# Jarvis73/PEMP

Measured on AMD Instinct MI355X. Metric: episodes/sec (PEMP stage-1 eval step, PASCAL-5i-shaped 1-shot, ResNet-50), higher is better.
Workload: dtype f32

## Files before the change

### include/pemp_hip.h

```cpp
#ifndef PEMP_HIP_H
#define PEMP_HIP_H

#include <stddef.h>
#include <stdint.h>

#ifdef __cplusplus
extern "C" {
#endif

#define PEMP_ABI_VERSION 2

#define PEMP_CONV_RELU 1u
#define PEMP_CONV_SHIFT_PER_IMAGE 2u
#define PEMP_CONV_STEM4 4u
#define PEMP_CONV_POOL3S2 8u
#define PEMP_CONV_OUT_SPLIT3 16u
#define PEMP_CONV_IN_SPLIT3 32u
#define PEMP_CONV_OUT_SPLIT3_ALSO 64u
#define PEMP_CONV_RES_S2 128u
#define PEMP_CONV_RES_HEVEN 512u
#define PEMP_CONV_RES_WEVEN 1024u

typedef struct pemp_conv_desc {
    int32_t N, H, W;
    int32_t Cin, ldx;
    int32_t Ho, Wo;
    int32_t Cout, ldy;
    int32_t KH, KW;
    int32_t stride, pad, dil;
    int32_t ldr;
    int32_t Kpad;
    uint32_t flags;
    int32_t tile;
} pemp_conv_desc;

const char* pemp_last_error(void);
int pemp_abi_version(void);

int pemp_conv2d_tile_shape(int id, int* bm, int* bn);

int pemp_conv2d_nhwc_f32(const pemp_conv_desc* d, const float* x, const float* w, float* y,
                         const float* scale, const float* shift, const float* residual,
                         void* stream);

int pemp_conv2d_padv_nhwc_f32(const pemp_conv_desc* d, const float* x, const float* w, float* y,
                              const float* scale, const float* shift, const float* residual,
                              const float* pad_value, void* stream);

int pemp_conv2d_hybrid_rows(const pemp_conv_desc* d);

int pemp_conv2d_group_nhwc_f32(int n, const pemp_conv_desc* d, const float* const* x, const float* const* w,
                               float* const* y, const float* const* scale, const float* const* shift,
                               const float* const* residual, const float* const* pad_value, void* stream);

int pemp_pack_split3_bf16(const float* w, void* out, int cout, int kpad, void* stream);

int pemp_conv2d_bf16_nhwc(const pemp_conv_desc* d, const void* x, const void* w, void* y, const float* scale,
                          const float* shift, const void* residual, const void* pad_value, int out_f32, void* stream);
int pemp_convert_f32_bf16(const float* x, void* y, long long n, void* stream);
int pemp_convert_bf16_f32(const void* x, float* y, long long n, void* stream);

int pemp_conv2d_dropblock_nhwc_f32(const pemp_conv_desc* d, const float* x, const float* w, float* y, const float* scale,
                                   const float* shift, const float* residual, const float* rowmask, const int* kept_count,
                                   void* ws, size_t ws_bytes, void* stream);
int pemp_bn_apply_dropblock_f32(const float* z, int ldz, const float* mean, const float* invstd, const float* gamma,
                                const float* beta, float* y, int ldy, int M, int C, const float* rowmask,
                                const int* kept_count, void* stream);

int pemp_pack_input_nhwc4_f32(const float* img, const float* prior, float* out,
                              int N, int H, int W, void* stream);

int pemp_maxpool2d_nhwc_f32(const float* x, float* y, int N, int H, int W, int C, int ldx,
                            int Ho, int Wo, int ldy, int k, int s, int p, void* stream);

int pemp_maxpool2d_idx_nhwc_f32(const float* x, float* y, uint8_t* idx, int N, int H, int W, int C,
                                int Ho, int Wo, int k, int s, int p, void* stream);
int pemp_maxpool2d_idx_bwd_nhwc_f32(const uint8_t* idx, const float* dy, float* dx, int N, int H, int W,
                                    int C, int Ho, int Wo, int k, int s, int p, void* stream);

int pemp_global_avgpool_nhwc_f32(const float* x, float* y, int N, int HW, int C, int ldx,
                                 void* stream);

int pemp_channel_affine_multi_f32(const float* x, int ldx, int M, int C, int nb,
                                  const float* const* scale, const float* const* shift,
                                  float* const* y, const int* ldy, void* stream);

size_t pemp_mpm_workspace_bytes(int B, int S, int n, int c, int p);
int pemp_mpm_protos_f32(const float* feat, int ldf, const float* mask, const float* ctr,
                        float* protos, void* ws, size_t ws_bytes,
                        int B, int S, int h, int w, int H, int W, int c, int p, void* stream);

size_t pemp_map_workspace_bytes(int B, int S, int n, int c);
int pemp_masked_avg_pool_f32(const float* feat, int ldf, const float* mask, float* protos,
                             void* ws, size_t ws_bytes, int B, int S, int h, int w, int H, int W,
                             int c, int full_res, void* stream);

int pemp_cosine_proto_max_f32(const float* qry, int ldf, const float* protos, float* pred,
                              uint8_t* resp, int B, int n, int c, int p, float dist_scalar,
                              void* stream);

int pemp_cosine_bank_max_f32(const float* qry, int ldf, const float* bank, const int32_t* index,
                             float* pred, uint8_t* resp, int N, int K, int n, int c, int p,
                             float dist_scalar, void* stream);

int pemp_argmax_masks_f32(const float* pred, float* masks, int B, int n, void* stream);

int pemp_upsample_bilinear_ac_f32(const float* pred, float* out, int B, int C, int h, int w,
                                  int Ho, int Wo, void* stream);

int pemp_upsample_nearest_u8_i64(const uint8_t* resp, int64_t* out, int B, int h, int w,
                                 int Ho, int Wo, void* stream);

size_t pemp_eval_tail_workspace_bytes(int B, int Ho, int Wo);
int pemp_eval_tail_f32(const float* pred, const int64_t* target, uint8_t* pred_out,
                       float* logits_out, double* stats, void* ws, size_t ws_bytes,
                       int B, int h, int w, int Ho, int Wo, void* stream);

size_t pemp_nway_tail_workspace_bytes(int N, int Ho, int Wo);
int pemp_nway_tail_f32(const float* pred, const int64_t* target, const int32_t* want, uint8_t* labels,
                       float* margin, double* stats, void* ws, size_t ws_bytes,
                       int N, int K, int h, int w, int Ho, int Wo, void* stream);

typedef struct pemp_tail_item {
    int32_t Ho, Wo;
    int32_t nblk;
    int32_t part_off;
    int64_t pix_off;
} pemp_tail_item;

size_t pemp_tail_ragged_workspace_bytes(pemp_tail_item* items_host, int n);
int pemp_eval_tail_ragged_f32(const float* pred, const int64_t* target, const pemp_tail_item* items_host,
                              const pemp_tail_item* items_dev, int B, int h, int w, uint8_t* pred_out,
                              double* stats, void* ws, size_t ws_bytes, void* stream);
int pemp_nway_tail_ragged_f32(const float* pred, const int64_t* target, const int32_t* want,
                              const pemp_tail_item* items_host, const pemp_tail_item* items_dev, int N, int K,
                              int h, int w, uint8_t* labels, float* margin, double* stats, void* ws,
                              size_t ws_bytes, void* stream);

int pemp_cm_reduce_f32(const float* x, int ldx, const float* mask_in, float* mask_out, float* stat,
                       int N, int Hm, int Wm, int Hx, int Wx, int C, int stride, void* stream);

int pemp_cm_linear_f32(const float* stat, const int32_t* group, const float* lin_w, const float* lin_b,
                       float* agg, float* feat, int N, int G, int C2, void* stream);
int pemp_cm_bias_f32(const float* feat, const int32_t* group, const float* wext, int ldw, const float* alpha,
                     const float* base, float* out, int N, int Cout, void* stream);
int pemp_cm_bias_bwd_f32(const float* colsum, const float* feat, const int32_t* group, const float* wext, int ldw,
                         float* dwext, int lddw, float* dfeat_img, int accumulate, int N, int Cout, void* stream);
int pemp_cm_linear_bwd_f32(const float* dfeat_img, const int32_t* group, const float* agg, const float* lin_w,
                           float* dlin_w, float* dlin_b, float* dstat, int N, int G, int C2, void* stream);

int pemp_cm_bwd_add_f32(const float* x, int ldx, const float* mask, const float* dstat, float* dx, int ldd,
                        int N, int HW, int C, void* stream);
int pemp_cm_reduce_arg_f32(const float* x, int ldx, const float* mask_in, float* mask_out, float* stat,
                           int32_t* argmax, int N, int Hm, int Wm, int Hx, int Wx, int C, int stride, void* stream);
int pemp_cm_bwd_add_arg_f32(const float* mask, const float* dstat, const int32_t* argmax, float* dx, int ldd,
                            int N, int HW, int C, void* stream);


size_t pemp_conv2d_splitk_workspace_bytes(const pemp_conv_desc* d);
int pemp_conv2d_splitk_nhwc_f32(const pemp_conv_desc* d, const float* x, const float* w, float* y, const float* scale,
                                const float* shift, const float* residual, void* ws, size_t ws_bytes, void* stream);
int pemp_conv2d_padv_splitk_nhwc_f32(const pemp_conv_desc* d, const float* x, const float* w, float* y, const float* scale,
                                     const float* shift, const float* residual, const float* pad_value, void* ws,
                                     size_t ws_bytes, void* stream);
void* pemp_uncached_alloc(size_t bytes);
int pemp_uncached_free(void* p);
int pemp_spin_us(int us, void* stream);
int pemp_splitk_reset(void* ws, void* stream);
int pemp_conv2d_stats_nhwc_f32(const pemp_conv_desc* d, const float* x, const float* w, float* y, float* stats,
                               void* ws, size_t ws_bytes, void* stream);
int pemp_conv2d_stats_rows(const pemp_conv_desc* d);
int pemp_split3_conv2d_stats_nhwc_f32(const pemp_conv_desc* d, const float* x, const void* w3, float* y, float* stats,
                                      void* stream);
int pemp_conv2d_stats_split3_rows(const pemp_conv_desc* d);
// ... 186 lines not shown
```

### pemp_amd/_lib.py

```python
import ctypes as C
import os

import torch

_HERE = os.path.dirname(os.path.abspath(__file__))
LIB_PATH = os.environ.get("PEMP_HIP_LIB", os.path.join(_HERE, "libpemp_hip.so"))

c_fp = C.c_void_p
c_int = C.c_int
c_size = C.c_size_t


class ConvDesc(C.Structure):
    _fields_ = [(n, C.c_int32) for n in
                ("N", "H", "W", "Cin", "ldx", "Ho", "Wo", "Cout", "ldy", "KH", "KW",
                 "stride", "pad", "dil", "ldr", "Kpad")] + [("flags", C.c_uint32), ("tile", C.c_int32)]


class SampleDesc(C.Structure):
    _fields_ = [("img_off", C.c_int64), ("msk_off", C.c_int64), ("img_out", C.c_int64), ("msk_out", C.c_int64)] + \
               [(n, C.c_int32) for n in ("hs", "ws", "sh", "sw", "oy", "ox", "flip", "jitter_order")] + \
               [("jitter", C.c_float * 3), ("mask_mode", C.c_int32), ("ksx", C.c_int32), ("ksy", C.c_int32),
                ("ws_off", C.c_int64)]


class TailItem(C.Structure):
    _fields_ = [(n, C.c_int32) for n in ("Ho", "Wo", "nblk", "part_off")] + [("pix_off", C.c_int64)]


CONV_RELU = 1
CONV_SHIFT_PER_IMAGE = 2
CONV_STEM4 = 4
CONV_POOL3S2 = 8
CONV_OUT_SPLIT3 = 16
CONV_IN_SPLIT3 = 32
CONV_OUT_SPLIT3_ALSO = 64
CONV_RES_S2 = 128
CONV_RES_HEVEN = 512
CONV_RES_WEVEN = 1024

SYMBOLS = {
    "pemp_last_error": (C.c_char_p, []),
    "pemp_abi_version": (c_int, []),
    "pemp_conv2d_hybrid_rows": (c_int, [C.POINTER(ConvDesc)]),
    "pemp_conv2d_tile_shape": (c_int, [c_int, C.POINTER(c_int), C.POINTER(c_int)]),
    "pemp_conv2d_nhwc_f32": (c_int, [C.POINTER(ConvDesc), c_fp, c_fp, c_fp, c_fp, c_fp, c_fp, c_fp]),
    "pemp_conv2d_padv_splitk_nhwc_f32": (c_int, [C.POINTER(ConvDesc), c_fp, c_fp, c_fp, c_fp, c_fp, c_fp, c_fp, c_fp, c_size, c_fp]),
    "pemp_conv2d_padv_nhwc_f32": (c_int, [C.POINTER(ConvDesc), c_fp, c_fp, c_fp, c_fp, c_fp, c_fp, c_fp, c_fp]),
    "pemp_conv2d_group_nhwc_f32": (c_int, [c_int, C.POINTER(ConvDesc)] + [C.POINTER(c_fp)] * 7 + [c_fp]),
    "pemp_conv2d_bf16_nhwc": (c_int, [C.POINTER(ConvDesc), c_fp, c_fp, c_fp, c_fp, c_fp, c_fp, c_fp, c_int, c_fp]),
    "pemp_pack_split3_bf16": (c_int, [c_fp, c_fp, c_int, c_int, c_fp]),
    "pemp_convert_f32_bf16": (c_int, [c_fp, c_fp, C.c_longlong, c_fp]),
    "pemp_convert_bf16_f32": (c_int, [c_fp, c_fp, C.c_longlong, c_fp]),
    "pemp_conv2d_dropblock_nhwc_f32": (c_int, [C.POINTER(ConvDesc), c_fp, c_fp, c_fp, c_fp, c_fp, c_fp, c_fp, c_fp, c_fp, c_size, c_fp]),
    "pemp_bn_apply_dropblock_f32": (c_int, [c_fp, c_int, c_fp, c_fp, c_fp, c_fp, c_fp, c_int, c_int, c_int, c_fp, c_fp, c_fp]),
    "pemp_pack_input_nhwc4_f32": (c_int, [c_fp, c_fp, c_fp, c_int, c_int, c_int, c_fp]),
    "pemp_maxpool2d_nhwc_f32": (c_int, [c_fp, c_fp] + [c_int] * 11 + [c_fp]),
    "pemp_global_avgpool_nhwc_f32": (c_int, [c_fp, c_fp, c_int, c_int, c_int, c_int, c_fp]),
    "pemp_channel_affine_multi_f32": (c_int, [c_fp, c_int, c_int, c_int, c_int,
                                              C.POINTER(c_fp), C.POINTER(c_fp), C.POINTER(c_fp),
                                              C.POINTER(c_int), c_fp]),
    "pemp_mpm_workspace_bytes": (c_size, [c_int] * 5),
    "pemp_mpm_protos_f32": (c_int, [c_fp, c_int, c_fp, c_fp, c_fp, c_fp, c_size] + [c_int] * 8 + [c_fp]),
    "pemp_map_workspace_bytes": (c_size, [c_int] * 4),
    "pemp_masked_avg_pool_f32": (c_int, [c_fp, c_int, c_fp, c_fp, c_fp, c_size] + [c_int] * 8 + [c_fp]),
    "pemp_cosine_proto_max_f32": (c_int, [c_fp, c_int, c_fp, c_fp, c_fp, c_int, c_int, c_int, c_int,
                                          C.c_float, c_fp]),
    "pemp_cosine_bank_max_f32": (c_int, [c_fp, c_int, c_fp, c_fp, c_fp, c_fp] + [c_int] * 5 + [C.c_float, c_fp]),
    "pemp_upsample_bilinear_ac_f32": (c_int, [c_fp, c_fp] + [c_int] * 6 + [c_fp]),
    "pemp_upsample_nearest_u8_i64": (c_int, [c_fp, c_fp] + [c_int] * 5 + [c_fp]),
    "pemp_eval_tail_workspace_bytes": (c_size, [c_int] * 3),
    "pemp_eval_tail_f32": (c_int, [c_fp, c_fp, c_fp, c_fp, c_fp, c_fp, c_size] + [c_int] * 5 + [c_fp]),
    "pemp_nway_tail_workspace_bytes": (c_size, [c_int] * 3),
    "pemp_nway_tail_f32": (c_int, [c_fp] * 7 + [c_size] + [c_int] * 6 + [c_fp]),
    "pemp_tail_ragged_workspace_bytes": (c_size, [C.POINTER(TailItem), c_int]),
    "pemp_eval_tail_ragged_f32": (c_int, [c_fp, c_fp, C.POINTER(TailItem), c_fp] + [c_int] * 3 + [c_fp, c_fp, c_fp, c_size, c_fp]),
    "pemp_nway_tail_ragged_f32": (c_int, [c_fp, c_fp, c_fp, C.POINTER(TailItem), c_fp] + [c_int] * 4 + [c_fp] * 4 + [c_size, c_fp]),
    "pemp_cm_reduce_f32": (c_int, [c_fp, c_int, c_fp, c_fp, c_fp] + [c_int] * 7 + [c_fp]),
    "pemp_argmax_masks_f32": (c_int, [c_fp, c_fp, c_int, c_int, c_fp]),
    "pemp_cm_reduce_arg_f32": (c_int, [c_fp, c_int, c_fp, c_fp, c_fp, c_fp] + [c_int] * 7 + [c_fp]),
    "pemp_cm_bwd_add_arg_f32": (c_int, [c_fp, c_fp, c_fp, c_fp] + [c_int] * 4 + [c_fp]),
    "pemp_cm_linear_f32": (c_int, [c_fp] * 6 + [c_int] * 3 + [c_fp]),
    "pemp_cm_bias_f32": (c_int, [c_fp, c_fp, c_fp, c_int, c_fp, c_fp, c_fp, c_int, c_int, c_fp]),
    "pemp_cm_bias_bwd_f32": (c_int, [c_fp, c_fp, c_fp, c_fp, c_int, c_fp, c_int, c_fp, c_int, c_int, c_int, c_fp]),
    "pemp_cm_linear_bwd_f32": (c_int, [c_fp] * 7 + [c_int] * 3 + [c_fp]),
    "pemp_episode_plan": (c_size, [C.POINTER(SampleDesc), c_int, c_int, c_int]),
    "pemp_episode_preprocess": (c_int, [c_fp, C.POINTER(SampleDesc), c_fp, c_int, c_int, c_int, C.POINTER(C.c_float),
                                        C.POINTER(C.c_float), c_fp, c_fp, c_fp, c_fp, c_size, c_fp]),
    "pemp_dropblock_mask_f32": (c_int, [c_fp, c_fp, c_fp, c_int, c_int, c_int, C.c_float, c_int, C.c_uint64, C.c_uint64, c_fp,
                                        c_fp]),
    "pemp_pixel_scale_f32": (c_int, [c_fp, c_int, c_fp, c_fp, c_fp, c_int, C.c_longlong, c_int, c_fp]),
    "pemp_dropout2d_mask_f32": (c_int, [c_fp, c_fp, c_int, c_int, C.c_float, C.c_uint64, C.c_uint64, c_fp, c_fp]),
    "pemp_channel_scale_f32": (c_int, [c_fp, c_int, c_fp, c_fp, c_int, c_int, c_int, c_int, c_fp]),
    "pemp_cm_bwd_add_f32": (c_int, [c_fp, c_int, c_fp, c_fp, c_fp, c_int, c_int, c_int, c_int, c_fp]),
    "pemp_conv2d_splitk_workspace_bytes": (c_size, [C.POINTER(ConvDesc)]),
    "pemp_conv2d_splitk_nhwc_f32": (c_int, [C.POINTER(ConvDesc), c_fp, c_fp, c_fp, c_fp, c_fp, c_fp, c_fp, c_size, c_fp]),
    "pemp_uncached_alloc": (c_fp, [c_size]),
    "pemp_uncached_free": (c_int, [c_fp]),
    "pemp_splitk_reset": (c_int, [c_fp, c_fp]),
    "pemp_spin_us": (c_int, [c_int, c_fp]),
    "pemp_conv2d_stats_nhwc_f32": (c_int, [C.POINTER(ConvDesc), c_fp, c_fp, c_fp, c_fp, c_fp, c_size, c_fp]),
    "pemp_conv2d_stats_rows": (c_int, [C.POINTER(ConvDesc)]),
    "pemp_split3_conv2d_stats_nhwc_f32": (c_int, [C.POINTER(ConvDesc), c_fp, c_fp, c_fp, c_fp, c_fp]),
    "pemp_conv2d_stats_split3_rows": (c_int, [C.POINTER(ConvDesc)]),
    "pemp_bn_stats_partials_f32": (c_int, [c_fp, c_int, c_int, c_int, C.c_float, C.c_float, c_fp, c_fp, c_fp, c_fp, c_fp]),
    "pemp_bn_fwd_partials_f32": (c_int, [c_fp, c_int, c_fp, c_int, c_int, c_int, C.c_float, C.c_float, c_fp, c_fp, c_fp, c_int,
                                         c_fp, c_int, c_int, c_fp, c_fp, c_fp, c_fp, c_fp, c_fp]),
    "pemp_conv2d_bnbwd_nhwc_f32": (c_int, [C.POINTER(ConvDesc), c_fp, c_fp, c_fp, c_fp, c_fp, c_fp, c_int, c_fp, c_fp, c_fp, c_fp,
                                           c_size, c_fp]),
    "pemp_bn_bwd_partials_f32": (c_int, [c_fp, c_int, c_fp, c_int, c_fp, c_fp, c_fp, c_fp, c_int, c_fp, c_int, c_fp, c_fp, c_int,
                                         c_int, c_fp]),
    "pemp_bn_apply_mask_f32": (c_int, [c_fp, c_int, c_fp, c_fp, c_fp, c_fp, c_fp, c_int, c_fp, c_int, c_int, c_int,
                                       c_int, c_fp, c_fp]),
    "pemp_conv2d_wgrad_workspace_bytes": (c_size, [C.POINTER(ConvDesc)]),
    "pemp_conv2d_wgrad_nhwc_f32": (c_int, [C.POINTER(ConvDesc), c_fp, c_fp, c_fp, c_int, c_fp, c_size, c_fp]),
    "pemp_colsum_workspace_bytes": (c_size, [c_int, c_int]),
    "pemp_bn_stats_f32": (c_int, [c_fp, c_int, c_int, c_int, C.c_float, C.c_float, c_fp, c_fp, c_fp, c_fp,
                                  c_fp, c_size, c_fp]),
    "pemp_bn_apply_f32": (c_int, [c_fp, c_int, c_fp, c_fp, c_fp, c_fp, c_fp, c_int, c_fp, c_int, c_int, c_int,
                                  c_int, c_fp]),
    "pemp_bn_bwd_f32": (c_int, [c_fp, c_int, c_fp, c_int, c_fp, c_int, c_fp, c_fp, c_fp, c_fp, c_int, c_fp, c_int,
                                c_fp, c_fp, c_int, c_int, c_int, c_fp, c_size, c_fp]),
    "pemp_bn_bwd_mask_f32": (c_int, [c_fp, c_int, c_fp, c_int, c_fp, c_fp, c_int, c_fp, c_fp, c_fp, c_fp, c_int, c_fp, c_int,
                                     c_fp, c_fp, c_int, c_int, c_int, c_fp, c_size, c_fp]),
    "pemp_relu_bias_bwd_f32": (c_int, [c_fp, c_int, c_fp, c_int, c_fp, c_int, c_fp, c_int, c_fp, c_int, c_int,
                                       c_int, c_fp, c_size, c_fp]),
    "pemp_maxpool2d_bwd_nhwc_f32": (c_int, [c_fp, c_fp, c_fp] + [c_int] * 9 + [c_fp]),
    "pemp_maxpool2d_idx_nhwc_f32": (c_int, [c_fp, c_fp, c_fp] + [c_int] * 9 + [c_fp]),
    "pemp_maxpool2d_idx_bwd_nhwc_f32": (c_int, [c_fp, c_fp, c_fp] + [c_int] * 9 + [c_fp]),
    "pemp_scatter_strided_nhwc_f32": (c_int, [c_fp, c_fp] + [c_int] * 7 + [c_fp]),
    "pemp_gap_bwd_add_nhwc_f32": (c_int, [c_fp, c_fp, c_int, c_int, c_int, c_int, c_fp]),
    "pemp_head_bwd_workspace_bytes": (c_size, [c_int] * 5),
    "pemp_head_bwd_f32": (c_int, [c_fp, c_fp, c_int, c_fp, c_fp, c_fp, c_fp, c_fp, c_fp, c_fp, c_fp, c_fp, c_fp, c_int,
                                  c_fp, c_fp, c_size] + [c_int] * 11 + [C.c_float, c_fp]),
    "pemp_head_bwd_dlogits_f32": (c_int, [c_fp, c_fp, c_int, c_fp, c_fp, c_fp, c_fp, c_fp, c_fp, c_fp, c_int,
                                          c_fp, c_fp, c_size] + [c_int] * 11 + [C.c_float, c_fp]),
    "pemp_eval_tail_weighted_f32": (c_int, [c_fp, c_fp, c_fp, c_fp, c_fp, c_fp, c_fp, c_size] + [c_int] * 5 + [c_fp]),
    "pemp_cedt_workspace_bytes": (c_size, [c_int] * 3),
    "pemp_cedt_weight_f32": (c_int, [c_fp, c_fp, c_fp, c_size, c_int, c_int, c_int, C.c_float, c_fp]),
    "pemp_sgd_workspace_bytes": (c_size, []),
    "pemp_sgd_clip_step_f32": (c_int, [c_fp, c_fp, c_fp, C.c_longlong, C.c_float, C.c_float, C.c_float,
                                       C.c_float, c_int, C.c_float, c_int, c_fp, c_fp, c_size, c_fp]),
    "pemp_dgrad_mirror_f32": (c_int, [c_fp, c_fp, c_fp, c_int, c_int, c_fp]),
    "pemp_adam_clip_step_f32": (c_int, [c_fp, c_fp, c_fp, c_fp, C.c_longlong, C.c_float] + [C.c_double] * 5 + [C.c_longlong, C.c_float, c_fp, c_fp,
                                                                                                  c_size, c_fp]),
    "pemp_prior_mask_workspace_bytes": (c_size, [c_int] * 3),
    "pemp_prior_mask_f32": (c_int, [c_fp, c_int, c_fp, c_int, c_fp, c_fp, c_fp, c_size] + [c_int] * 4 + [c_fp]),
    "pemp_prior_bank_pack_f32": (c_int, [c_fp, c_int, c_fp, c_fp, c_fp, c_fp] + [c_int] * 4 + [c_fp]),
    "pemp_prior_bank_workspace_bytes": (c_size, [c_int] * 3),
    "pemp_prior_bank_f32": (c_int, [c_fp, c_int, c_fp, c_fp, c_fp, c_fp, c_fp, c_fp, c_size] + [c_int] * 6 + [c_fp]),
    "pemp_bank_gather_rows_f32": (c_int, [c_fp, c_fp, c_fp, c_int, c_int, c_int, c_fp]),
    "pemp_adaptive_avgpool_nhwc_f32": (c_int, [c_fp, c_int, c_fp] + [c_int] * 7 + [c_fp]),
    "pemp_resize_bilinear_ac_nhwc_f32": (c_int, [c_fp, C.c_longlong, c_int, c_int, c_fp, C.c_longlong, c_int, c_int] + [c_int] * 7
                                         + [c_fp]),
    "pemp_weighted_gap_f32": (c_int, [c_fp, c_int, c_fp, c_fp] + [c_int] * 5 + [c_fp]),
    "pemp_scale_add_nhwc_f32": (c_int, [c_fp, c_int, c_fp, c_fp, c_int, c_fp, c_int, C.c_longlong, c_int, c_fp]),
    "pemp_canet_support_vector_f32": (c_int, [c_fp, c_int, c_fp, c_fp] + [c_int] * 7 + [c_fp]),
    "pemp_canet_zterm_f32": (c_int, [c_fp, c_fp, c_fp, c_fp] + [c_int] * 7 + [c_fp]),
    "pemp_canet_block_input_f32": (c_int, [c_fp, c_int, c_fp, c_fp, c_int, c_fp] + [c_int] * 5 + [c_fp]),
    "pemp_canet_history_update_f32": (c_int, [c_fp, c_fp, c_fp, c_int, c_fp, c_int, c_int, c_fp]),
    "pemp_canet_zterm_bwd_workspace_bytes": (c_size, [c_int] * 4),
    "pemp_canet_zterm_bwd_f32": (c_int, [c_fp, c_int, c_fp, c_int, c_fp, c_fp, c_fp, c_fp, c_fp, c_size] + [c_int] * 6 + [c_fp]),
    "pemp_canet_support_vector_bwd_f32": (c_int, [c_fp, c_fp, c_fp] + [c_int] * 8 + [c_fp]),
    "pemp_canet_cls_bwd_workspace_bytes": (c_size, [c_int] * 2),
    "pemp_canet_cls_bwd_f32": (c_int, [c_fp, c_fp, c_int, c_fp, c_fp, c_int, c_fp, c_fp, c_fp, c_size] + [c_int] * 3 + [c_fp]),
    "pemp_upsample_ce_bwd_f32": (c_int, [c_fp] * 6 + [c_int] * 5 + [c_fp]),
    "pemp_weighted_gap_bwd_f32": (c_int, [c_fp, c_fp, c_fp] + [c_int] * 6 + [c_fp]),
    "pemp_adaptive_avgpool_bwd_multi_nhwc_f32": (c_int, [c_int, C.POINTER(c_fp)] + [C.POINTER(c_int)] * 3 + [c_fp] + [c_int] * 5
                                                 + [c_fp]),
    "pemp_resize_bilinear_ac_bwd_nhwc_f32": (c_int, [c_fp, C.c_longlong, c_int, c_int] * 3 + [c_int] * 6 + [c_fp]),
    "pemp_pfenet_merge_support_bwd_workspace_bytes": (c_size, [c_int] * 3),
    "pemp_pfenet_merge_support_bwd_f32": (c_int, [c_int, C.POINTER(c_fp)] + [C.POINTER(c_int)] * 3 + [C.POINTER(c_fp)] * 2
                                          + [c_int, c_fp, c_fp, c_fp, c_size] + [c_int] * 3 + [c_fp]),
    "pemp_rpmms_em_f32": (c_int, [c_fp, c_int, c_fp, c_fp, c_fp, c_fp] + [c_int] * 5 + [c_fp]),
    "pemp_rpmms_prob_map_f32": (c_int, [c_fp, c_int, c_fp, c_fp, c_int, C.c_longlong, c_int, c_int, c_int, c_fp]),
    "pemp_rpmms_proto_sum_f32": (c_int, [c_fp, c_fp, c_fp, c_int, c_fp, c_fp, c_fp, c_int, C.c_longlong] + [c_int] * 5 + [c_fp]),
    "pemp_rpmms_proto_taps_f32": (c_int, [c_fp, c_fp, c_fp, c_int, c_int, c_fp]),
    "pemp_rpmms_bank_l56_f32": (c_int, [c_fp, c_int, c_fp, c_int, c_fp, c_fp, c_fp, c_fp, c_fp, c_int, C.c_longlong] + [c_int] * 6 + [c_fp]),
    "pemp_rpmms_proto_sum_train_f32": (c_int, [c_fp, c_fp, c_fp, c_int, c_fp, c_fp, c_fp, c_fp, c_int, C.c_longlong] + [c_int] * 5 + [c_fp]),
    "pemp_rpmms_proto_sum_bwd_work_floats": (c_size, [c_int] * 4),
    "pemp_rpmms_proto_sum_bwd_f32": (c_int, [c_fp, c_int, C.c_longlong, c_fp, c_int, c_fp, c_fp, c_fp, c_fp, c_fp, c_int, c_fp, c_fp, c_int,
                                             c_fp, c_fp, c_size] + [c_int] * 5 + [c_fp]),
    "pemp_rpmms_history_bwd_f32": (c_int, [c_fp, c_int, c_fp, c_fp, c_int, c_int, c_fp]),
}

ABI_VERSION = 2
_lib = None


class PempHipError(RuntimeError):
    pass

# ... 26 lines not shown
```

### pemp_amd/build.py

```python
import hashlib
import os
import subprocess
from concurrent.futures import ThreadPoolExecutor

HERE = os.path.dirname(os.path.abspath(__file__))
CSRC = os.path.join(HERE, "csrc")
OBJ = os.path.join(HERE, "_obj")
OUT = os.path.join(HERE, "libpemp_hip.so")
SOURCES = ("conv_igemm.hip", "conv_dma.hip", "conv_dma2.hip", "conv_panel.hip", "conv_row3.hip", "conv_ring.hip", "conv_stem_pool.hip", "conv_wgrad.hip", "train_ops.hip", "pool_misc.hip", "head.hip", "head_bwd.hip", "cedt.hip",
           "episode_io.hip", "dropout.hip", "cm_linear.hip", "pfenet.hip", "pfenet_bwd.hip", "canet.hip", "canet_bwd.hip", "rpmms.hip", "rpmms_bwd.hip")
FLAGS = ["-O3", "--offload-arch=gfx950", "-std=c++17", "-fPIC"]


def _headers():
    return [os.path.join(CSRC, f) for f in sorted(os.listdir(CSRC)) if f.endswith((".h", ".inc"))] + \
           [os.path.join(HERE, "..", "include", "pemp_hip.h")]


def csrc_digest():
    h = hashlib.sha1()
    for f in sorted(os.listdir(CSRC)):
        with open(os.path.join(CSRC, f), "rb") as fh:
            h.update(f.encode() + b"\0" + fh.read())
    with open(os.path.join(HERE, "..", "include", "pemp_hip.h"), "rb") as fh:
        h.update(fh.read())
    return h.hexdigest()[:12]


CONV_ENGINE = ("common.h", "conv_common.h", "conv_tiles.h", "conv_igemm.hip", "conv_dma.hip", "conv_dma2.hip", "conv_panel.hip", "conv_row3.hip", "conv_ring.hip", "conv_stem_pool.hip")


def conv_digest():
    h = hashlib.sha1()
    for f in CONV_ENGINE:
        with open(os.path.join(CSRC, f), "rb") as fh:
            h.update(f.encode() + b"\0" + fh.read())
    return h.hexdigest()[:12]


def needs_build():
    if not os.path.exists(OUT):
        return True
    t = os.path.getmtime(OUT)
    deps = [os.path.join(CSRC, f) for f in os.listdir(CSRC)] + [os.path.join(HERE, "..", "include", "pemp_hip.h")]
    return any(os.path.getmtime(d) > t for d in deps)


def _stamp(src, flags):
    h = hashlib.sha1(" ".join(flags).encode())
    for f in [src] + _headers():
        with open(f, "rb") as fh:
            h.update(fh.read())
    return h.hexdigest()


def _compile(hipcc, name, flags, force, verbose):
    src = os.path.join(CSRC, name)
    obj = os.path.join(OBJ, name.replace(".hip", ".o"))
    stamp_file = obj + ".stamp"
    stamp = _stamp(src, flags)
    if not force and os.path.exists(obj) and os.path.exists(stamp_file) and open(stamp_file).read() == stamp:
        return obj
    cmd = [hipcc] + flags + ["-c", src, "-o", obj]
    if verbose:
        print(" ".join(cmd), flush=True)
    subprocess.run(cmd, check=True)
    with open(stamp_file, "w") as f:
        f.write(stamp)
    return obj


def build(force=False, verbose=False, extra_flags=(), out=None):
    out = out or OUT
    if not force and out == OUT and not needs_build():
        return OUT
    hipcc = os.environ.get("HIPCC", "/opt/rocm/bin/hipcc")
    os.makedirs(OBJ, exist_ok=True)
    flags = FLAGS + list(extra_flags)
    jobs = max(1, min(len(SOURCES), int(os.environ.get("PEMP_BUILD_JOBS", str(min(os.cpu_count() or 1, 8))))))
    with ThreadPoolExecutor(jobs) as ex:
        objs = list(ex.map(lambda n: _compile(hipcc, n, flags, force, verbose), SOURCES))
    tmp = out + f".tmp{os.getpid()}"
    cmd = [hipcc, "--offload-arch=gfx950", "-shared", "-fPIC", "-o", tmp] + objs
    if verbose:
        print(" ".join(cmd), flush=True)
    subprocess.run(cmd, check=True)
    os.replace(tmp, out)
    return out


if __name__ == "__main__":
    print(build(force=True, verbose=True))
```

### pemp_amd/csrc/conv_common.h

```cpp
#pragma once
#include "common.h"

namespace pemp {

typedef __attribute__((ext_vector_type(16))) float f32x16;
typedef __attribute__((ext_vector_type(4))) float v4f;
typedef __attribute__((ext_vector_type(8))) __bf16 bf16x8;
typedef __attribute__((ext_vector_type(2))) unsigned int u32x2;

#define PEMP_CONV_BF16_IO 0x100u

__device__ __forceinline__ v4f load_quad(const float* base, size_t off, unsigned bf16) {
    if (!bf16) return *(const v4f*)(base + off);
    const u32x2 r = *(const u32x2*)((const unsigned short*)base + off);
    return v4f{__builtin_bit_cast(float, r.x << 16), __builtin_bit_cast(float, r.x & 0xFFFF0000u),
               __builtin_bit_cast(float, r.y << 16), __builtin_bit_cast(float, r.y & 0xFFFF0000u)};
}

__device__ __forceinline__ unsigned int bf16_bits(float f) {
    const unsigned int u = __builtin_bit_cast(unsigned int, f);
    if ((u & 0x7FFFFFFFu) > 0x7F800000u) return (u >> 16) | 0x40u;
    return (u + 0x7FFFu + ((u >> 16) & 1u)) >> 16;
}

// ... 217 lines not shown
                    if constexpr (DB) {
                        const float k = a.rowmask[m];
                        o.x = __fdiv_rn(__fmul_rn(__fmul_rn(o.x, k), db_numel), db_sum);
                        o.y = __fdiv_rn(__fmul_rn(__fmul_rn(o.y, k), db_numel), db_sum);
                        o.z = __fdiv_rn(__fmul_rn(__fmul_rn(o.z, k), db_numel), db_sum);
                        o.w = __fdiv_rn(__fmul_rn(__fmul_rn(o.w, k), db_numel), db_sum);
                    }
                    if constexpr (EPI == 2) {
                        const uint32_t b = mw[i] >> c4;
                        o.x = (b & 1u) ? o.x : 0.f;
                        o.y = (b & 2u) ? o.y : 0.f;
                        o.z = (b & 4u) ? o.z : 0.f;
                        o.w = (b & 8u) ? o.w : 0.f;
                    }
                    store_quad(a.y, (size_t)m * a.ldy + n, o, a.flags & PEMP_CONV_BF16_IO);
                    if constexpr (EPI == 1) {
                        s1 += o;
                        s2 += o * o;
                    }
                    if constexpr (EPI == 2) {
                        s1 += o;
                        s2 += o * ((zt[i] - bmu) * bis);
                    }
                }
            }
            if constexpr (EPI != 0) {
                t1 += s1;
                t2 += s2;
            }
            if constexpr (OS3 == 2) {
                static_assert(EPI == 0 && !DB && !PRE, "the second, pre-split output: plain epilogue");
                v4f sc8[2], sh8[2];
                conv_split3_affine(a, n_base + ni * 32 + (lane & 3) * 8, sc8, sh8);
                conv_store_split3_to(a, (unsigned short*)a.res, S, m_base + mi * 32, n_base + ni * 32, lane, sc8, sh8);
            }
            asm volatile("s_waitcnt lgkmcnt(0)" ::: "memory");
        }
        if constexpr (EPI != 0) {
            *(v4f*)(R + ((ni * 2 + 0) * 8 + rr) * 32 + c4) = t1;
            *(v4f*)(R + ((ni * 2 + 1) * 8 + rr) * 32 + c4) = t2;
        }
    }
}

template <int BN, int WGM, int NW, int TN>
__device__ __forceinline__ void conv_stats_store(const ConvArgs& a, const float* Rall, int bm, int n0, int tid) {
    constexpr int WGN = NW / WGM, WN = BN / WGN;
    if (tid < 2 * BN) {
        const int st = tid / BN, col = tid - st * BN;
        const int wni = col / WN, ni = (col - wni * WN) >> 5, c = col & 31;
        float s = 0.f;
#pragma unroll
        for (int wmi = 0; wmi < WGM; ++wmi)
#pragma unroll
            for (int g = 0; g < 8; ++g) s += Rall[((((wmi * WGN + wni) * TN + ni) * 2 + st) * 8 + g) * 32 + c];
        a.stats[((size_t)bm * 2 + st) * a.Cout + n0 + col] = s;
    }
}

template <int TM, int TN, bool DB = false, int OS3 = 0>
__device__ __forceinline__ void conv_epilogue_lds(const ConvArgs& a, f32x16 (&acc)[TM][TN], float* S, int m_base,
                                                  int n_base, int lane) {
    const v4f none[1] = {{0.f, 0.f, 0.f, 0.f}};
    static_assert(TM * TN * 4 != 1, "tile");
    conv_epilogue_lds_pre<TM, TN, 1, 0, DB, OS3>(a, acc, S, m_base, n_base, lane, none);
}

__device__ __forceinline__ void conv_patch_store_f32(const ConvArgs& a, const float* S, int m_base, int n32, int lane, const v4f& sc,
                                                     const v4f& sh, bool per_img, const v4f* res, unsigned bf16) {
    const bool relu = a.flags & PEMP_CONV_RELU;
    const int rr = lane >> 3, c4 = (lane & 7) * 4, n = n32 + c4;
#pragma unroll
    for (int i = 0; i < 4; ++i) {
        const int row = rr + 8 * i;
        const int m = m_base + row;
        const v4f v = *(const v4f*)(S + row * 32 + c4);
        if (m < a.M) {
            v4f add = sh;
            if (per_img) add += *(const v4f*)(a.shift + (size_t)(m / a.HoWo) * a.Cout + n);
            if (res && a.res) add += res[i];
            store_quad(a.y, (size_t)m * a.ldy + n, conv_affine_quad(v, sc, add, relu), bf16);
        }
    }
}

template <int TM, int TN, bool PLAIN = false>
__device__ __forceinline__ void conv_epilogue_s3p(const ConvArgs& a, f32x16 (&acc)[TM][TN], float* S, int m_base, int n_base,
                                                  int lane, const v4f* pre, const v4f (&scv)[TN], const v4f (&shv)[TN]) {
    const bool per_img = !PLAIN && (a.flags & PEMP_CONV_SHIFT_PER_IMAGE);
    const int lr = lane & 31, lh = lane >> 5;
#pragma unroll
    for (int ni = 0; ni < TN; ++ni) {
#pragma unroll
        for (int mi = 0; mi < TM; ++mi) {
            PEMP_CONV_PATCH_PUT(S, acc[mi][ni], lr, lh);
            asm volatile("s_waitcnt lgkmcnt(0)" ::: "memory");
            conv_patch_store_f32(a, S, m_base + mi * 32, n_base + ni * 32, lane, scv[ni], shv[ni], per_img,
                                 PLAIN ? nullptr : pre + (mi * TN + ni) * 4, PLAIN ? 0u : a.flags & PEMP_CONV_BF16_IO);
            asm volatile("s_waitcnt lgkmcnt(0)" ::: "memory");
        }
    }
}

template <int TN>
__device__ __forceinline__ void conv_epilogue_r16(const ConvArgs& a, v4f (&acc)[TN], float* S, int m_base, int n_base, int lane) {
    constexpr int WN = TN * 16, LD = WN + 4, QPR = WN / 4;
    static_assert(16 * LD * 4 <= 4096 && (16 * QPR) % 64 == 0, "R16 epilogue patch");
    const bool relu = a.flags & PEMP_CONV_RELU;
    const bool per_img = a.flags & PEMP_CONV_SHIFT_PER_IMAGE;
    const int r16 = lane & 15, g = lane >> 4;
#pragma unroll
    for (int ni = 0; ni < TN; ++ni)
#pragma unroll
        for (int e = 0; e < 4; ++e) S[(4 * g + e) * LD + ni * 16 + r16] = acc[ni][e];
    asm volatile("s_waitcnt lgkmcnt(0)" ::: "memory");
    const int c4 = (lane % QPR) * 4, n = n_base + c4;
    v4f sc = {1.f, 1.f, 1.f, 1.f}, sh = {0.f, 0.f, 0.f, 0.f};
    if (a.scale) sc = *(const v4f*)(a.scale + n);
    if (a.shift && !per_img) sh = *(const v4f*)(a.shift + n);
#pragma unroll
    for (int i = 0; i < 16 * QPR / 64; ++i) {
        const int row = (lane + 64 * i) / QPR;
        const int m = m_base + row;
        const v4f v = *(const v4f*)(S + row * LD + c4);
        if (m < a.M) {
            v4f add = sh;
            if (per_img) add += *(const v4f*)(a.shift + (size_t)(m / a.HoWo) * a.Cout + n);
            if (a.res) add += load_quad(a.res, (size_t)m * a.ldr + n, a.flags & PEMP_CONV_BF16_IO);
            store_quad(a.y, (size_t)m * a.ldy + n, conv_affine_quad(v, sc, add, relu), a.flags & PEMP_CONV_BF16_IO);
        }
    }
}

int launch_conv_dma(int shape, const ConvArgs& a, hipStream_t st);
bool conv_dma2_supported(const ConvArgs& a);
int launch_conv_dma2(int shape, const ConvArgs& a, hipStream_t st);
int launch_conv_dma2_group(int shape, ConvGroupArgs& g, hipStream_t st);
int launch_conv_dma2_hybrid(const ConvArgs& a, hipStream_t st);
int conv_dma2_hybrid_rows(int M, int Cout);
int launch_conv_dma2_bf16(int shape, const ConvArgs& a, hipStream_t st);
int launch_conv_dma2_db(int shape, ConvArgs a, void* ws, size_t ws_bytes, bool split, hipStream_t st);
struct SplitKPlan { int full, split, pieces; size_t ws_bytes; };
SplitKPlan conv_dma2_splitk_plan(int shape, const ConvArgs& a);
int launch_conv_dma2_splitk(int shape, ConvArgs a, void* ws, size_t ws_bytes, hipStream_t st);
int launch_conv_dma2_split3(int shape, ConvArgs a, void* ws, size_t ws_bytes, bool split, hipStream_t st);
int launch_conv_dma2_group_split3(int shape, ConvGroupArgs& g, hipStream_t st);
int launch_conv_dma2_split3_stats(int shape, const ConvArgs& a, hipStream_t st);
bool conv_dma2_split3_stats_shape(int shape);
int launch_conv_dma2_split3_persist(int shape, const ConvArgs& a, hipStream_t st);
bool conv_dma2_persist_out_split3(int shape);
int launch_conv_dma2_split3_pre(int shape, bool persistent, const ConvArgs& a, hipStream_t st);
bool conv_panel_supported(const ConvArgs& a);
int launch_conv_panel(int shape, const ConvArgs& a, hipStream_t st);
bool conv_row3_supported(const ConvArgs& a);
int launch_conv_row3(bool persistent, const ConvArgs& a, hipStream_t st);
bool conv_ring_supported(const ConvArgs& a);
int launch_conv_ring(const ConvArgs& a, hipStream_t st);
int conv_dma2_simds();
int pack_split3(const float* w, void* out, int cout, int kpad, hipStream_t st);
int launch_conv_stem_pool(const ConvArgs& a, hipStream_t st);
int conv_stem_pool_out(int i);

template <class Kern> int allow_lds(Kern kern, size_t lds);
template <class Kern>
int persistent_grid(Kern kern, int threads, size_t lds, long long tiles, int& occ_cache, const char* what, int& grid_out) {
    if (!occ_cache) {
        const int rc = allow_lds(kern, lds);
        if (rc) return rc;
        int v = 0;
        hipError_t e = hipOccupancyMaxActiveBlocksPerMultiprocessor(&v, (const void*)kern, threads, lds);
        if (e != hipSuccess || v <= 0) {
            set_error("%s: occupancy query failed (%s, %d blocks)", what, hipGetErrorString(e), v);
            return -1;
        }
        occ_cache = v;
    }
    long long grid = (long long)occ_cache * (conv_dma2_simds() / 4);
    if (grid < 8) grid = 8;
    if (grid > tiles) grid = tiles;
    grid_out = (int)grid;
    return 0;
}

}
```

### pemp_amd/csrc/conv_igemm.hip

```cpp
#include "conv_tiles.h"

namespace pemp {


template <int BM, int BN, int WGM, bool STEM>
__global__ __launch_bounds__(256) void conv_igemm_kernel(ConvArgs a) {
    constexpr int WGN = 4 / WGM;
    constexpr int WM = BM / WGM, WN = BN / WGN;
    constexpr int TM = WM / 32, TN = WN / 32;
    constexpr int AL = BM / 32, BL = BN / 32;
    static_assert(TM >= 1 && TN >= 1, "wave tile");

    extern __shared__ __attribute__((aligned(16))) v4f smem[];
    v4f* As = smem;
    v4f* Bs = smem + 2 * 8 * BM;

    const int tid = threadIdx.x;
    const int lane = tid & 63;
    const int wave = tid >> 6;
    const int wm0 = (wave / WGN) * WM;
    const int wn0 = (wave % WGN) * WN;
    const int lr = lane & 31, lh = lane >> 5;

    const int ntn = a.Cout / BN;
// ... 71 lines not shown
            _Pragma("unroll") for (int i = 0; i < AL; ++i) ra[i] = *(const v4f*)pa[i];              \
        }                                                                                            \
        _Pragma("unroll") for (int i = 0; i < BL; ++i) rb[i] = *(const v4f*)pb[i];                   \
    } while (0)

#define PEMP_ADVANCE()                                                                               \
    do {                                                                                             \
        if constexpr (STEM) {                                                                        \
            _Pragma("unroll") for (int i = 0; i < BL; ++i) pb[i] += 32;                              \
        } else if (a.ntaps > 1) {                                                                    \
                                   \
            if (++cur_tap == a.ntaps) {                                                              \
                cur_tap = 0;                                                                         \
                ++cur_cb;                                                                            \
            }                                                                                        \
            PEMP_SET_TAP(cur_tap, cur_cb);                                                           \
            const int koff = cur_tap * a.Cin + cur_cb * 32;                                          \
            _Pragma("unroll") for (int i = 0; i < BL; ++i) pb[i] = wrow[i] + koff;                   \
        } else {                                                                                     \
            _Pragma("unroll") for (int i = 0; i < BL; ++i) pb[i] += 32;                              \
            _Pragma("unroll") for (int i = 0; i < AL; ++i) pa[i] += 32;                              \
        }                                                                                            \
    } while (0)

#define PEMP_LSTORE(buf_)                                                                            \
    do {                                                                                             \
        v4f* Ab_ = As + (buf_) * 8 * BM + q * BM;                                                 \
        v4f* Bb_ = Bs + (buf_) * 8 * BN + q * BN;                                                 \
        _Pragma("unroll") for (int i = 0; i < AL; ++i) {                                             \
            v4f v = ra[i];                                                                        \
            if (!((okmask >> i) & 1u)) v = v4f{0.f, 0.f, 0.f, 0.f};                          \
            Ab_[(r + 32 * i) ^ q] = v;                                                               \
        }                                                                                            \
        _Pragma("unroll") for (int i = 0; i < BL; ++i) Bb_[(r + 32 * i) ^ q] = rb[i];                \
    } while (0)

    f32x16 acc[TM][TN];
#pragma unroll
    for (int mi = 0; mi < TM; ++mi)
#pragma unroll
        for (int ni = 0; ni < TN; ++ni)
#pragma unroll
            for (int e = 0; e < 16; ++e) acc[mi][ni][e] = 0.f;

    if constexpr (!STEM) PEMP_SET_TAP(0, 0);
    PEMP_GLOAD(0);
    PEMP_LSTORE(0);
    __syncthreads();

    const int arow = wm0 + lr, brow = wn0 + lr;
#ifndef PEMP_ABLATE
#define PEMP_ABLATE 0
#endif
    for (int kt = 0; kt < a.nk; ++kt) {
        const int buf = (PEMP_ABLATE >= 2) ? 0 : (kt & 1);
        if (PEMP_ABLATE < 1 && kt + 1 < a.nk) {
            PEMP_ADVANCE();
            PEMP_GLOAD(kt + 1);
        }
        __builtin_amdgcn_sched_barrier(0);

        const v4f* Ab = As + buf * 8 * BM;
        const v4f* Bb = Bs + buf * 8 * BN;
        v4f af[2][TM], bf[2][TN];
#pragma unroll
        for (int mi = 0; mi < TM; ++mi) af[0][mi] = Ab[lh * BM + ((arow + mi * 32) ^ lh)];
#pragma unroll
        for (int ni = 0; ni < TN; ++ni) bf[0][ni] = Bb[lh * BN + ((brow + ni * 32) ^ lh)];
#pragma unroll
        for (int j = 0; j < 4; ++j) {
            if (j < 3) {
                const int qq = 2 * (j + 1) + lh;
#pragma unroll
                for (int mi = 0; mi < TM; ++mi) af[(j + 1) & 1][mi] = Ab[qq * BM + ((arow + mi * 32) ^ qq)];
#pragma unroll
                for (int ni = 0; ni < TN; ++ni) bf[(j + 1) & 1][ni] = Bb[qq * BN + ((brow + ni * 32) ^ qq)];
            }
            __builtin_amdgcn_sched_barrier(0);
#pragma unroll
            for (int mi = 0; mi < TM; ++mi)
#pragma unroll
                for (int ni = 0; ni < TN; ++ni) {
                    const v4f av = af[j & 1][mi], bv = bf[j & 1][ni];
                    acc[mi][ni] = __builtin_amdgcn_mfma_f32_32x32x2f32(av.x, bv.x, acc[mi][ni], 0, 0, 0);
                    acc[mi][ni] = __builtin_amdgcn_mfma_f32_32x32x2f32(av.y, bv.y, acc[mi][ni], 0, 0, 0);
                    acc[mi][ni] = __builtin_amdgcn_mfma_f32_32x32x2f32(av.z, bv.z, acc[mi][ni], 0, 0, 0);
                    acc[mi][ni] = __builtin_amdgcn_mfma_f32_32x32x2f32(av.w, bv.w, acc[mi][ni], 0, 0, 0);
                }
        }
        __builtin_amdgcn_sched_barrier(0);
        if (PEMP_ABLATE < 2) {
            PEMP_LSTORE(buf ^ 1);
            __syncthreads();
        }
    }
#undef PEMP_GLOAD
#undef PEMP_ADVANCE
#undef PEMP_SET_TAP
#undef PEMP_LSTORE

    conv_epilogue_lds<TM, TN>(a, acc, (float*)smem + wave * 1024, m0 + wm0, n0 + wn0, lane);
}

static int launch_conv(int shape, const ConvArgs& a, hipStream_t st) {
    return with_tile<FamIgemm>(shape, [&](auto t) {
        using T = decltype(t);
        auto kern = (a.flags & PEMP_CONV_STEM4) ? conv_igemm_kernel<T::BM, T::BN, T::WGM, true> : conv_igemm_kernel<T::BM, T::BN, T::WGM, false>;
        return launch_with_lds(kern, tile_grid<T>(a), 256, tile_lds<T>(), st, a, "conv_igemm");
    });
}

}

using namespace pemp;

extern "C" int pemp_conv2d_nhwc_f32(const pemp_conv_desc* d, const float* x, const float* w, float* y,
                                    const float* scale, const float* shift, const float* residual,
                                    void* stream) {
    return pemp_conv2d_padv_nhwc_f32(d, x, w, y, scale, shift, residual, nullptr, stream);
}

static int conv2d_impl(const pemp_conv_desc* d, const float* x, const float* w, float* y, const float* scale, const float* shift,
                       const float* residual, const float* pad_value, void* ws, size_t ws_bytes, void* stream);

extern "C" int pemp_conv2d_padv_nhwc_f32(const pemp_conv_desc* d, const float* x, const float* w, float* y,
                                         const float* scale, const float* shift, const float* residual,
                                         const float* pad_value, void* stream) {
    PEMP_REQUIRE(!d || !decode_tile(d->tile).splitk,
                 "conv2d: the split-K tile ids 31..37 / 51..56 need pemp_conv2d_splitk_nhwc_f32 (workspace)");
    return conv2d_impl(d, x, w, y, scale, shift, residual, pad_value, nullptr, 0, stream);
}

extern "C" int pemp_conv2d_splitk_nhwc_f32(const pemp_conv_desc* d, const float* x, const float* w, float* y,
                                           const float* scale, const float* shift, const float* residual, void* ws,
                                           size_t ws_bytes, void* stream) {
    return conv2d_impl(d, x, w, y, scale, shift, residual, nullptr, ws, ws_bytes, stream);
}

extern "C" int pemp_conv2d_padv_splitk_nhwc_f32(const pemp_conv_desc* d, const float* x, const float* w, float* y,
                                                const float* scale, const float* shift, const float* residual,
                                                const float* pad_value, void* ws, size_t ws_bytes, void* stream) {
    PEMP_REQUIRE(pad_value, "conv2d_padv_splitk: pad_value is null");
    return conv2d_impl(d, x, w, y, scale, shift, residual, pad_value, ws, ws_bytes, stream);
}

static int conv_fill(const pemp_conv_desc* d, const float* x, const float* w, float* y, const float* scale, const float* shift,
                     const float* residual, const float* pad_value, ConvArgs& a, bool any_taps = false, bool pooled = false) {
    PEMP_REQUIRE(d && x && w && y, "conv2d: null pointer");
    PEMP_REQUIRE(pooled || !(d->flags & (PEMP_CONV_OUT_SPLIT3 | PEMP_CONV_IN_SPLIT3 | PEMP_CONV_OUT_SPLIT3_ALSO)),
                 "conv2d: pre-split activations belong to pemp_conv2d_nhwc_f32 / _padv_ (no grouped / dropblock / statistics / bf16 form)");
    PEMP_REQUIRE(pooled || !(d->flags & PEMP_CONV_POOL3S2), "conv2d: PEMP_CONV_POOL3S2 belongs to pemp_conv2d_nhwc_f32 (no grouped / dropblock / statistics / bf16 form)");
    PEMP_REQUIRE(pooled || !(d->flags & (PEMP_CONV_RES_S2 | PEMP_CONV_RES_HEVEN | PEMP_CONV_RES_WEVEN)),
                 "conv2d: PEMP_CONV_RES_S2 belongs to pemp_conv2d_nhwc_f32 (no grouped / dropblock / statistics / bf16 form)");
    PEMP_REQUIRE(!pad_value || (!(d->flags & PEMP_CONV_STEM4) && (any_taps || d->KH * d->KW > 1) && ((uintptr_t)pad_value & 15) == 0),
                 "conv2d: pad_value needs a multi-tap non-stem conv and a 16-byte aligned [Cin] vector");
    PEMP_REQUIRE(d->N > 0 && d->H > 0 && d->W > 0 && d->Cin > 0 && d->Cout > 0, "conv2d: bad dims");
    PEMP_REQUIRE(d->KH > 0 && d->KW > 0 && d->stride > 0 && d->dil > 0 && d->pad >= 0, "conv2d: bad kernel geometry");
    const int ho = (d->H + 2 * d->pad - d->dil * (d->KH - 1) - 1) / d->stride + 1;
    const int wo = (d->W + 2 * d->pad - d->dil * (d->KW - 1) - 1) / d->stride + 1;
    PEMP_REQUIRE(ho == d->Ho && wo == d->Wo, "conv2d: Ho/Wo (%d,%d) do not match geometry (%d,%d)", d->Ho, d->Wo, ho, wo);
    PEMP_REQUIRE(d->Cout % 64 == 0, "conv2d: Cout=%d must be a multiple of 64", d->Cout);
    PEMP_REQUIRE(d->ldy >= d->Cout && d->ldy % 4 == 0 && ((uintptr_t)y & 15) == 0, "conv2d: ldy must be >= Cout and a multiple of 4, y 16-byte aligned");
    PEMP_REQUIRE(!scale || ((uintptr_t)scale & 15) == 0, "conv2d: scale must be 16-byte aligned");
    PEMP_REQUIRE(!shift || ((uintptr_t)shift & 15) == 0, "conv2d: shift must be 16-byte aligned");
    PEMP_REQUIRE(((uintptr_t)x & 15) == 0 && ((uintptr_t)w & 15) == 0, "conv2d: x/w must be 16-byte aligned");
    const bool stem = d->flags & PEMP_CONV_STEM4;
    const int ntaps = d->KH * d->KW;
    if (stem) {
        PEMP_REQUIRE(d->Cin == 4 && d->ldx == 4, "conv2d: STEM4 needs NHWC4 input (Cin=ldx=4)");
        PEMP_REQUIRE(d->Kpad % 32 == 0 && d->Kpad >= ntaps * 4, "conv2d: STEM4 Kpad=%d too small / not x32", d->Kpad);
    } else {
        PEMP_REQUIRE(d->Cin % 32 == 0, "conv2d: Cin=%d must be a multiple of 32 (or use STEM4)", d->Cin);
        PEMP_REQUIRE(d->ldx >= d->Cin && d->ldx % 4 == 0, "conv2d: ldx=%d must be >= Cin and a multiple of 4", d->ldx);
        PEMP_REQUIRE(d->Kpad == ntaps * d->Cin, "conv2d: Kpad=%d must equal KH*KW*Cin=%d", d->Kpad, ntaps * d->Cin);
    }
    const long long in_elems = (long long)d->N * d->H * d->W * d->ldx;
    const long long out_elems = (long long)d->N * d->Ho * d->Wo * (long long)(d->ldy > d->ldr ? d->ldy : d->ldr);
    PEMP_REQUIRE(in_elems < (1ll << 31) && out_elems < (1ll << 31), "conv2d: tensor too large for 32-bit indexing");

    a.x = x; a.w = w; a.y = y; a.scale = scale; a.shift = shift; a.res = residual; a.padv = pad_value; a.stats = nullptr; a.bz = nullptr;
    a.bmask = nullptr; a.bmean = nullptr; a.binvstd = nullptr; a.ldbz = 0;
    a.rowmask = nullptr; a.rowcnt = nullptr;
    a.N = d->N; a.H = d->H; a.W = d->W; a.Cin = d->Cin; a.ldx = d->ldx; a.Ho = d->Ho; a.Wo = d->Wo;
    a.Cout = d->Cout; a.ldy = d->ldy; a.KH = d->KH; a.KW = d->KW; a.stride = d->stride; a.pad = d->pad;
    a.dil = d->dil; a.ldr = d->ldr; a.Kpad = d->Kpad; a.flags = d->flags;
    a.HoWo = d->Ho * d->Wo;
    a.M = d->N * a.HoWo;
    a.ntaps = ntaps;
    a.cin_steps = stem ? 1 : d->Cin / 32;
    a.nk = d->Kpad / 32;
    if (residual && !(d->flags & PEMP_CONV_OUT_SPLIT3_ALSO)) PEMP_REQUIRE(d->ldr >= d->Cout && d->ldr % 4 == 0 && ((uintptr_t)residual & 15) == 0, "conv2d: ldr must be >= Cout and x4, residual 16-byte aligned");
    a.sk_ws = nullptr; a.sk_cnt = nullptr; a.sk_full = 0; a.sk_S = 1;
    a.bm_first = 0;
    return 0;
}

static int conv2d_impl(const pemp_conv_desc* d, const float* x, const float* w, float* y, const float* scale, const float* shift,
                       const float* residual, const float* pad_value, void* ws, size_t ws_bytes, void* stream) {
    ConvArgs a;
    const int rc = conv_fill(d, x, w, y, scale, shift, residual, pad_value, a, false, true);
    if (rc) return rc;
    const bool stem = d->flags & PEMP_CONV_STEM4;
    int tile = d->tile;
    if (tile == 0) {
        tile = 3;
    }
    TileId t = decode_tile(tile);
    if (t.ring) {
        PEMP_REQUIRE(!ws && !pad_value && conv_ring_supported(a),
                     "conv2d: tile %d unsupported: needs a 1x1 conv without padding on fp32 activations with Kpad == Cin >= 128 and Cout %% 128 == 0, the "
                     "fp32 output or PEMP_CONV_OUT_SPLIT3 (ldy == Cout); no residual, PEMP_CONV_OUT_SPLIT3_ALSO, PEMP_CONV_IN_SPLIT3, PEMP_CONV_RES_S2, "
                     "padding value, stem, split-K or workspace; operands < 2 GiB", tile);
        return launch_conv_ring(a, (hipStream_t)stream);
    }
    const bool out_split3 = d->flags & PEMP_CONV_OUT_SPLIT3;
    if (out_split3)
        PEMP_REQUIRE(t.family == TILE_SPLIT3 && !t.splitk && !t.panel && !ws && !stem && !residual && a.Cout % 32 == 0 && a.ldy == a.Cout,
                     "conv2d: PEMP_CONV_OUT_SPLIT3 needs an unsplit split3 tile id (41..44, 46, 47, 49, 146, 149), ldy == Cout, no residual / workspace");
    const bool also_split3 = d->flags & PEMP_CONV_OUT_SPLIT3_ALSO;
    if (also_split3) {
        PEMP_REQUIRE(t.presplit && !out_split3 && !ws && !stem && a.Cout % 32 == 0,
                     "conv2d: PEMP_CONV_OUT_SPLIT3_ALSO needs tile id 146 / 149, no PEMP_CONV_OUT_SPLIT3 / split-K / workspace / stem");
        PEMP_REQUIRE(residual && ((uintptr_t)residual & 15) == 0,
                     "conv2d: PEMP_CONV_OUT_SPLIT3_ALSO takes the pre-split tensor (16-byte aligned) in the residual argument; a residual is never read");
        const char *y0 = (const char*)y, *y1 = y0 + ((size_t)(a.M - 1) * a.ldy + a.Cout) * 4;
        const char *s0 = (const char*)residual, *s1 = s0 + (size_t)a.M * a.Cout * 6;
        PEMP_REQUIRE(y1 <= s0 || s1 <= y0, "conv2d: PEMP_CONV_OUT_SPLIT3_ALSO: y and the pre-split tensor overlap");
    }
    const bool res_s2 = d->flags & PEMP_CONV_RES_S2;
    PEMP_REQUIRE(res_s2 || !(d->flags & (PEMP_CONV_RES_HEVEN | PEMP_CONV_RES_WEVEN)), "conv2d: PEMP_CONV_RES_HEVEN / _WEVEN come with PEMP_CONV_RES_S2");
    if (res_s2) {
        PEMP_REQUIRE(residual && !out_split3 && !also_split3 && !(d->flags & PEMP_CONV_IN_SPLIT3) && !ws && !stem && !pad_value,
                     "conv2d: PEMP_CONV_RES_S2 needs a residual, no pre-split operands / PEMP_CONV_OUT_SPLIT3_ALSO / split-K / workspace / stem / padding value");
        PEMP_REQUIRE(t.family == TILE_SPLIT3 && t.exists && !t.splitk && !t.persistent && !t.presplit &&
                         (t.panel ? (a.nk == 2 || (a.nk == 4 && t.shape == 2)) : t.shape == 3),
                     "conv2d: PEMP_CONV_RES_S2 needs tile id 43, 72 with Kpad 64 or 128, or 71 with Kpad 64 (tile %d, Kpad %d: the persistent, split-K, "
                     "pre-split and fp32-chain ids have no strided-residual form)", tile, a.Kpad);
        a.Hr = 2 * a.Ho - 1 + ((d->flags & PEMP_CONV_RES_HEVEN) ? 1 : 0);
        a.Wr = 2 * a.Wo - 1 + ((d->flags & PEMP_CONV_RES_WEVEN) ? 1 : 0);
        PEMP_REQUIRE((long long)a.N * a.Hr * a.Wr * a.ldr < (1ll << 31), "conv2d: PEMP_CONV_RES_S2: residual too large for 32-bit indexing");
    }
    if (d->flags & PEMP_CONV_POOL3S2) {
        PEMP_REQUIRE(stem && t.family == TILE_SPLIT3 && !t.splitk && !t.panel && !residual && !pad_value,
                     "conv2d: PEMP_CONV_POOL3S2 needs PEMP_CONV_STEM4 with split3 weights (a tile id 41..49), no residual, no padding value");
        return launch_conv_stem_pool(a, (hipStream_t)stream);
    }
    PEMP_REQUIRE(tile != 33 && tile != 53, "conv2d: no split-K variant of the 64 x 64 tile");
    PEMP_REQUIRE(tile != 45 && tile != 55, "conv2d: no split3 form of the 128 x 64 8-wave tile");
    PEMP_REQUIRE(tile != 48, "conv2d: no persistent split3 form of the 128 x 128 4-wave tile");
    PEMP_REQUIRE(t.exists, "conv2d: unknown tile id %d", tile);
    hipStream_t st = (hipStream_t)stream;
    PEMP_REQUIRE(t.presplit == ((d->flags & PEMP_CONV_IN_SPLIT3) != 0), "conv2d: tile ids 146 / 149 and PEMP_CONV_IN_SPLIT3 come together (tile %d)", tile);
    if (t.presplit) {
        PEMP_REQUIRE(!stem && !ws && a.ntaps > 1 && a.ntaps <= 16 && a.ldx == a.Cin && !(d->flags & PEMP_CONV_SHIFT_PER_IMAGE),
                     "conv2d: tile %d takes convs of 2..16 taps with ldx == Cin, no per-image shift, no workspace", tile);
        PEMP_REQUIRE(conv_dma2_supported(a) && (long long)a.Cout * a.Kpad * 6 < (1ll << 31),
                     "conv2d: tile %d needs <= 32 taps and operands < 2 GiB (a padding value behind the activations)", tile);
        PEMP_REQUIRE_COUT("conv2d", t.shape, a.Cout);
        if (t.row3) {
            PEMP_REQUIRE(conv_row3_supported(a),
                         "conv2d: tile %d unsupported: needs a 3x3 / stride 1 / pad == dil conv, the plain fp32 output without residual / padding value, "
                         "and a stage of at most 288 rows (256 + 2 d + d ceil((255 + 2 d) / W))", tile);
            return launch_conv_row3(t.persistent, a, st);
        }
        return launch_conv_dma2_split3_pre(t.shape, t.persistent, a, st);
    }
    if (t.family == TILE_SPLIT3) {
        PEMP_REQUIRE(!stem && conv_dma2_supported(a) && (long long)a.Cout * a.Kpad * 6 < (1ll << 31),
                     "conv2d: split3 tile %d needs a geometry of the buffer-addressed kernels (no stem, <= 32 taps, operands < 2 GiB)", tile);
        PEMP_REQUIRE_COUT("conv2d", t.shape, a.Cout);
        if (t.panel) {
            PEMP_REQUIRE(!ws && conv_panel_supported(a),
                         "conv2d: tile %d needs a 1x1 conv without padding, Kpad <= 256, no padding value / per-image shift / workspace, operands < 2 GiB", tile);
            return launch_conv_panel(t.shape, a, st);
        }
        if (t.persistent && (!out_split3 || conv_dma2_persist_out_split3(t.shape))) return launch_conv_dma2_split3_persist(t.shape, a, st);
        return launch_conv_dma2_split3(t.shape, a, ws, ws_bytes, t.splitk, st);
    }
    if (t.family == TILE_DMA2 && t.splitk) {
        if (conv_dma2_supported(a)) {
            PEMP_REQUIRE_COUT("conv2d", t.shape, a.Cout);
            return launch_conv_dma2_splitk(t.shape, a, ws, ws_bytes, st);
        }
        t.splitk = false;
    }
    if (t.family == TILE_DMA2 && t.shape == 9) {
        if (conv_dma2_supported(a)) {
            const int rc2 = launch_conv_dma2_hybrid(a, st);
            if (rc2 != -2) return rc2;
        }
        t.shape = 3;
    }
    if (t.family == TILE_DMA2) {
        if (conv_dma2_supported(a)) {
            PEMP_REQUIRE_COUT("conv2d", t.shape, a.Cout);
            return launch_conv_dma2(t.shape, a, st);
        }
        t.family = TILE_DMA;
        if (t.shape == 8) t.shape = 3;
    }
    if (t.family == TILE_DMA) {
        PEMP_REQUIRE_COUT("conv2d", t.shape, a.Cout);
        return launch_conv_dma(t.shape, a, st);
    }
    PEMP_REQUIRE(t.shape != 1 || a.Cout % 128 == 0, "conv2d: tile 128x128 needs Cout %% 128 == 0");
    return launch_conv(t.shape, a, st);
}


extern "C" int pemp_conv2d_group_nhwc_f32(int n, const pemp_conv_desc* d, const float* const* x, const float* const* w,
                                          float* const* y, const float* const* scale, const float* const* shift,
                                          const float* const* residual, const float* const* pad_value, void* stream) {
    PEMP_REQUIRE(n >= 1 && n <= CONV_GROUP_MAX && d && x && w && y, "conv2d_group: 1..%d member convs", CONV_GROUP_MAX);
    ConvGroupArgs g;
    g.n = n;
    const int tile = d[0].tile;
    const TileId t = decode_tile(tile);
    const bool s3 = t.family == TILE_SPLIT3 && t.exists && !t.splitk && !t.persistent && !t.panel && !t.presplit;
    PEMP_REQUIRE((t.family == TILE_DMA2 && !t.splitk && t.shape <= 8) || s3, "conv2d_group: tile must be one of the buffer-addressed variants 21..28 or 41..44, 46, got %d", tile);
    for (int i = 0; i < n; ++i) {
        PEMP_REQUIRE(d[i].tile == tile, "conv2d_group: every member must name the same tile variant");
        PEMP_REQUIRE(!pad_value || (pad_value[i] != nullptr) == (pad_value[0] != nullptr), "conv2d_group: pad_value for every member or for none");
        const int rc = conv_fill(&d[i], x[i], w[i], y[i], scale ? scale[i] : nullptr, shift ? shift[i] : nullptr,
                                 residual ? residual[i] : nullptr, pad_value ? pad_value[i] : nullptr, g.a[i], true);
        if (rc) return rc;
        PEMP_REQUIRE(conv_dma2_supported(g.a[i]), "conv2d_group: member %d lies outside the buffer-addressed kernels (stem / > 32 taps / 2 GiB operands / padding vector not behind the activations)", i);
        PEMP_REQUIRE_COUT("conv2d_group", t.shape, g.a[i].Cout);
        PEMP_REQUIRE(!s3 || (long long)g.a[i].Cout * g.a[i].Kpad * 6 < (1ll << 31), "conv2d_group: split3 weights of 2 GiB or more");
    }
    auto clash = [](const float* pa, long long rows_a, int ld_a, int c_a, const float* pb, long long rows_b, int ld_b, int c_b) {
        if (!pa || !pb) return false;
        const char *a0 = (const char*)pa, *a1 = a0 + ((rows_a - 1) * ld_a + c_a) * 4;
        const char *b0 = (const char*)pb, *b1 = b0 + ((rows_b - 1) * ld_b + c_b) * 4;
        if (a1 <= b0 || b1 <= a0) return false;
        if (ld_a != ld_b) return true;
        const long long delta = (b0 - a0) / 4, r = ((delta % ld_a) + ld_a) % ld_a;
        return !(r >= c_a && r + c_b <= ld_a);
    };
    for (int i = 0; i < n; ++i) {
        const long long Mi = (long long)g.a[i].N * g.a[i].Ho * g.a[i].Wo;
        for (int j = 0; j < n; ++j) {
            if (j == i) continue;
            const long long Mj = (long long)g.a[j].N * g.a[j].Ho * g.a[j].Wo, Pj = (long long)g.a[j].N * g.a[j].H * g.a[j].W;
            PEMP_REQUIRE(j > i || !clash(g.a[i].y, Mi, g.a[i].ldy, g.a[i].Cout, g.a[j].y, Mj, g.a[j].ldy, g.a[j].Cout),
                         "conv2d_group: members %d and %d write the same output", i, j);
            PEMP_REQUIRE(!clash(g.a[i].y, Mi, g.a[i].ldy, g.a[i].Cout, g.a[j].x, Pj, g.a[j].ldx, g.a[j].Cin),
                         "conv2d_group: member %d writes what member %d reads as its input", i, j);
            PEMP_REQUIRE(!clash(g.a[i].y, Mi, g.a[i].ldy, g.a[i].Cout, g.a[j].res, Mj, g.a[j].ldr, g.a[j].Cout),
                         "conv2d_group: member %d writes what member %d reads as its residual", i, j);
        }
    }
    for (int i = n; i < CONV_GROUP_MAX; ++i) g.a[i] = g.a[0];
    return s3 ? launch_conv_dma2_group_split3(t.shape, g, (hipStream_t)stream) : launch_conv_dma2_group(t.shape, g, (hipStream_t)stream);
}

extern "C" int pemp_pack_split3_bf16(const float* w, void* out, int cout, int kpad, void* stream) {
    PEMP_REQUIRE(w && out && cout > 0 && kpad > 0 && kpad % 32 == 0, "pack_split3: null pointer or Kpad not a multiple of 32");
    PEMP_REQUIRE((((uintptr_t)w | (uintptr_t)out) & 15) == 0, "pack_split3: pointers must be 16-byte aligned");
    return pack_split3(w, out, cout, kpad, (hipStream_t)stream);
}


extern "C" int pemp_conv2d_dropblock_nhwc_f32(const pemp_conv_desc* d, const float* x, const float* w, float* y, const float* scale,
                                              const float* shift, const float* residual, const float* rowmask, const int* kept_count,
                                              void* ws, size_t ws_bytes, void* stream) {
    PEMP_REQUIRE(rowmask && kept_count, "conv2d_dropblock: null mask / count");
    ConvArgs a;
    const int rc = conv_fill(d, x, w, y, scale, shift, residual, nullptr, a);
    if (rc) return rc;
    const TileId t = decode_tile(d->tile);
    PEMP_REQUIRE(t.family == TILE_DMA2 && t.exists && t.shape <= 7,
                 "conv2d_dropblock: tile must be 21..27 or 31..37 (no 33), got %d", d->tile);
    PEMP_REQUIRE(conv_dma2_supported(a), "conv2d_dropblock: geometry / operand size outside the buffer-addressed kernels");
    a.rowmask = rowmask;
    a.rowcnt = kept_count;
    PEMP_REQUIRE_COUT("conv2d_dropblock", t.shape, a.Cout);
    return launch_conv_dma2_db(t.shape, a, ws, ws_bytes, t.splitk, (hipStream_t)stream);
}


extern "C" int pemp_conv2d_bf16_nhwc(const pemp_conv_desc* d, const void* x, const void* w, void* y, const float* scale,
                                     const float* shift, const void* residual, const void* pad_value, int out_f32, void* stream) {
    PEMP_REQUIRE(d && x && w && y, "conv2d_bf16: null pointer");
    PEMP_REQUIRE(!(d->flags & (PEMP_CONV_STEM4 | PEMP_CONV_BF16_IO | PEMP_CONV_POOL3S2 | PEMP_CONV_OUT_SPLIT3_ALSO)), "conv2d_bf16: no stem variant; unknown flags");
    PEMP_REQUIRE(d->Cin % 64 == 0 && d->ldx % 8 == 0 && d->ldx >= d->Cin && d->Kpad == d->KH * d->KW * d->Cin,
                 "conv2d_bf16: Cin must be a multiple of 64, ldx of 8 (bf16 elements), Kpad = KH*KW*Cin");
    PEMP_REQUIRE(!residual || !out_f32, "conv2d_bf16: a residual comes with a bf16 output");
    const TileId t = decode_tile(d->tile == 0 ? 24 : d->tile);
    PEMP_REQUIRE(t.family == TILE_DMA2 && !t.splitk && t.shape <= 7, "conv2d_bf16: tile must be 0 or 21..27");
    pemp_conv_desc h = *d;
    h.Cin = d->Cin / 2;
    h.ldx = d->ldx / 2;
    h.Kpad = d->Kpad / 2;
    ConvArgs a;
    const int rc = conv_fill(&h, (const float*)x, (const float*)w, (float*)y, scale, shift, (const float*)residual,
                             (const float*)pad_value, a);
    if (rc) return rc;
    if (!out_f32) a.flags |= PEMP_CONV_BF16_IO;
    PEMP_REQUIRE(conv_dma2_supported(a), "conv2d_bf16: geometry / operand size outside the buffer-addressed kernels");
    PEMP_REQUIRE_COUT("conv2d_bf16", t.shape, a.Cout);
    return launch_conv_dma2_bf16(t.shape, a, (hipStream_t)stream);
}


static TileId stats_tile(const pemp_conv_desc* d) { return decode_tile(d->tile == 0 ? 23 : d->tile); }

static int conv_stats_fill(const char* what, const pemp_conv_desc* d, ConvArgs& a) {
    PEMP_REQUIRE(!(d->flags & (PEMP_CONV_STEM4 | PEMP_CONV_RELU | PEMP_CONV_SHIFT_PER_IMAGE | PEMP_CONV_POOL3S2 | PEMP_CONV_OUT_SPLIT3 | PEMP_CONV_IN_SPLIT3 | PEMP_CONV_OUT_SPLIT3_ALSO | PEMP_CONV_RES_S2 | PEMP_CONV_RES_HEVEN | PEMP_CONV_RES_WEVEN)), "%s: plain conv only (no stem / ReLU / per-image shift)", what);
    PEMP_REQUIRE(d->N > 0 && d->H > 0 && d->W > 0 && d->Cin > 0 && d->Cout > 0 && d->KH > 0 && d->KW > 0 && d->stride > 0 && d->dil > 0 && d->pad >= 0,
                 "%s: bad geometry", what);
    const int ho = (d->H + 2 * d->pad - d->dil * (d->KH - 1) - 1) / d->stride + 1;
    const int wo = (d->W + 2 * d->pad - d->dil * (d->KW - 1) - 1) / d->stride + 1;
    PEMP_REQUIRE(ho == d->Ho && wo == d->Wo, "%s: Ho/Wo do not match geometry", what);
    PEMP_REQUIRE(d->Cout % 64 == 0 && d->Cin % 32 == 0 && d->ldx >= d->Cin && d->ldx % 4 == 0 && d->ldy >= d->Cout && d->ldy % 4 == 0,
                 "%s: Cout %% 64, Cin %% 32, strides %% 4", what);
    PEMP_REQUIRE(d->Kpad == d->KH * d->KW * d->Cin, "%s: Kpad must equal KH*KW*Cin", what);
    a.scale = nullptr; a.shift = nullptr; a.padv = nullptr; a.rowmask = nullptr; a.rowcnt = nullptr;
    a.N = d->N; a.H = d->H; a.W = d->W; a.Cin = d->Cin; a.ldx = d->ldx; a.Ho = d->Ho; a.Wo = d->Wo;
    a.Cout = d->Cout; a.ldy = d->ldy; a.KH = d->KH; a.KW = d->KW; a.stride = d->stride; a.pad = d->pad;
    a.dil = d->dil; a.ldr = d->ldr; a.Kpad = d->Kpad; a.flags = d->flags;
    a.HoWo = d->Ho * d->Wo;
    a.M = d->N * a.HoWo;
    a.ntaps = d->KH * d->KW;
    a.cin_steps = d->Cin / 32;
    a.nk = d->Kpad / 32;
    a.sk_ws = nullptr; a.sk_cnt = nullptr; a.sk_full = 0; a.sk_S = 1;
    a.bm_first = 0;
    if (!conv_dma2_supported(a)) {
        set_error("%s: geometry / operand size outside the buffer-addressed kernels", what);
        return -2;
    }
    const TileId t = stats_tile(d);
    PEMP_REQUIRE(t.family == TILE_DMA2 && t.exists && t.shape <= 7, "%s: tile must be 0, 21..27 or 31..37 (no 33)", what);
    PEMP_REQUIRE_COUT(what, t.shape, a.Cout);
    return 0;
}

static int conv_stats_common(const char* what, const pemp_conv_desc* d, ConvArgs& a, void* ws, size_t ws_bytes, hipStream_t st) {
    const int rc = conv_stats_fill(what, d, a);
    if (rc) return rc;
    const TileId t = stats_tile(d);
    return t.splitk ? launch_conv_dma2_splitk(t.shape, a, ws, ws_bytes, st) : launch_conv_dma2(t.shape, a, st);
}

extern "C" int pemp_conv2d_hybrid_rows(const pemp_conv_desc* d) {
    if (!d || d->N <= 0 || d->Ho <= 0 || d->Wo <= 0 || d->Cout <= 0) return 0;
    return conv_dma2_hybrid_rows(d->N * d->Ho * d->Wo, d->Cout);
}

extern "C" int pemp_conv2d_tile_shape(int id, int* bm, int* bn) {
    const TileId t = decode_tile(id);
    if (!t.exists) return 0;
    if (bm) *bm = kTileShapes[t.shape].bm;
    if (bn) *bn = kTileShapes[t.shape].bn;
    return 1;
}

extern "C" int pemp_conv2d_stats_rows(const pemp_conv_desc* d) {
    if (!d || d->N <= 0 || d->Ho <= 0 || d->Wo <= 0) return 0;
    const TileId t = stats_tile(d);
    if (t.family != TILE_DMA2 || t.shape > 7) return 0;
    return cdiv(d->N * d->Ho * d->Wo, kTileShapes[t.shape].bm);
}

extern "C" size_t pemp_conv2d_splitk_workspace_bytes(const pemp_conv_desc* d) {
    const TileId t = decode_tile(d ? d->tile : 0);
    if (!t.splitk || !t.exists || d->N <= 0 || d->Ho <= 0 || d->Wo <= 0 || d->Cout <= 0 || d->Kpad < 32) return 0;
    ConvArgs a;
    a.M = d->N * d->Ho * d->Wo;
    a.Cout = d->Cout;
    a.nk = d->Kpad / 32;
    return conv_dma2_splitk_plan(t.shape, a).ws_bytes;
}

extern "C" int pemp_conv2d_stats_nhwc_f32(const pemp_conv_desc* d, const float* x, const float* w, float* y, float* stats,
                                          void* ws, size_t ws_bytes, void* stream) {
    PEMP_REQUIRE(d && x && w && y && stats, "conv2d_stats: null pointer");
    PEMP_REQUIRE((((uintptr_t)x | (uintptr_t)w | (uintptr_t)y | (uintptr_t)stats) & 15) == 0, "conv2d_stats: pointers must be 16-byte aligned");
    ConvArgs a;
    a.x = x; a.w = w; a.y = y; a.res = nullptr; a.stats = stats;
    a.bmask = nullptr; a.bz = nullptr; a.bmean = nullptr; a.binvstd = nullptr; a.ldbz = 0;
    return conv_stats_common("conv2d_stats", d, a, ws, ws_bytes, (hipStream_t)stream);
}

static int stats_split3_shape(const pemp_conv_desc* d) {
    const int id = d->tile == 0 ? 43 : d->tile;
    const TileId t = decode_tile(id);
    if (id < 41 || id > 46 || t.family != TILE_SPLIT3 || !t.exists || t.persistent || t.splitk || t.panel || t.presplit) return 0;
    return conv_dma2_split3_stats_shape(t.shape) ? t.shape : 0;
}

extern "C" int pemp_conv2d_stats_split3_rows(const pemp_conv_desc* d) {
    if (!d || d->N <= 0 || d->Ho <= 0 || d->Wo <= 0) return 0;
    const int shape = stats_split3_shape(d);
    return shape ? cdiv(d->N * d->Ho * d->Wo, kTileShapes[shape].bm) : 0;
}

extern "C" int pemp_split3_conv2d_stats_nhwc_f32(const pemp_conv_desc* d, const float* x, const void* w3, float* y, float* stats, void* stream) {
    PEMP_REQUIRE(d && x && w3 && y && stats, "conv2d_stats_split3: null pointer");
    PEMP_REQUIRE((((uintptr_t)x | (uintptr_t)w3 | (uintptr_t)y | (uintptr_t)stats) & 15) == 0, "conv2d_stats_split3: pointers must be 16-byte aligned");
    const int shape = stats_split3_shape(d);
    PEMP_REQUIRE(shape, "conv2d_stats_split3: tile %d has no split3 statistics form (0 or an unsplit id of 41..46 that pemp_conv2d_stats_split3_rows answers for)", d->tile);
    PEMP_REQUIRE(d->flags == 0, "conv2d_stats_split3: plain conv only (no flags: stem / ReLU / per-image shift / pre-split operands)");
    PEMP_REQUIRE(d->Cout > 0 && d->Cout >= kTileShapes[shape].bn, "conv2d_stats_split3: Cout=%d below the tile's %d columns", d->Cout, kTileShapes[shape].bn);
    ConvArgs a;
    a.x = x; a.w = (const float*)w3; a.y = y; a.res = nullptr; a.stats = stats;
    a.bmask = nullptr; a.bz = nullptr; a.bmean = nullptr; a.binvstd = nullptr; a.ldbz = 0;
    pemp_conv_desc f = *d;
    f.tile = 20 + shape;
    const int rc = conv_stats_fill("conv2d_stats_split3", &f, a);
    if (rc) return rc;
    if ((long long)a.Cout * a.Kpad * 6 >= (1ll << 31)) {
        set_error("conv2d_stats_split3: split3 weights of 2 GiB or more");
        return -2;
    }
    return launch_conv_dma2_split3_stats(shape, a, (hipStream_t)stream);
}

extern "C" int pemp_conv2d_bnbwd_nhwc_f32(const pemp_conv_desc* d, const float* x, const float* w, float* y, const float* residual,
                                          const uint32_t* mask, const float* z, int ldz, const float* mean, const float* invstd,
                                          float* stats, void* ws, size_t ws_bytes, void* stream) {
    PEMP_REQUIRE(d && x && w && y && z && mean && invstd && stats, "conv2d_bnbwd: null pointer");
    PEMP_REQUIRE((((uintptr_t)x | (uintptr_t)w | (uintptr_t)y | (uintptr_t)stats | (uintptr_t)z | (uintptr_t)residual | (uintptr_t)mean |
                   (uintptr_t)invstd) & 15) == 0 && ((uintptr_t)mask & 3) == 0, "conv2d_bnbwd: pointers must be 16-byte aligned");
    PEMP_REQUIRE(ldz >= d->Cout && ldz % 4 == 0 && (!residual || (d->ldr >= d->Cout && d->ldr % 4 == 0)), "conv2d_bnbwd: ldz / ldr");
    ConvArgs a;
    a.x = x; a.w = w; a.y = y; a.res = residual; a.stats = stats;
    a.bmask = mask; a.bz = z; a.bmean = mean; a.binvstd = invstd; a.ldbz = ldz;
    return conv_stats_common("conv2d_bnbwd", d, a, ws, ws_bytes, (hipStream_t)stream);
}
```

### pemp_amd/csrc/conv_panel.hip

```cpp
#include "conv_tiles.h"

namespace pemp {

typedef __attribute__((address_space(3))) void* lptr_t;
typedef __attribute__((ext_vector_type(4))) unsigned int v4u;

template <int NK> constexpr bool panel_early() { return NK >= 4; }
template <int NK, int BN> constexpr bool panel_two_blocks() { return BN == 64 && NK <= 4; }
template <int NK, int BN> constexpr int panel_stages() {
    if (!panel_early<NK>()) return 3;
    if (NK == 4) return 5;
    return BN == 64 ? 8 : 6;
}
template <int NK, int NS, int BL, int NST>
constexpr int panel_behind(int kt) {
    int c = 0;
    for (int u = kt + 1 - NS; u <= kt - 1; ++u) {
        const int ku = ((u % NK) + NK) % NK;
        if (u > kt + 1 - NS) c += BL;
        if (ku == NK - 1) c += NST;
    }
    return c;
}
template <int NK, int NS, int BL, int NST>
constexpr int panel_behind_max() {
    int m = 0;
    for (int kt = 0; kt < NK; ++kt) m = panel_behind<NK, NS, BL, NST>(kt) > m ? panel_behind<NK, NS, BL, NST>(kt) : m;
    return m;
}
template <int NK, int NS, int BL, int NST, int KT = 0>
__device__ __forceinline__ void panel_wait(int kt) {
    if constexpr (KT < NK) {
        if (kt == KT) asm volatile("s_waitcnt vmcnt(%0) lgkmcnt(0)" ::"n"(panel_behind<NK, NS, BL, NST>(KT)) : "memory");
        else panel_wait<NK, NS, BL, NST, KT + 1>(kt);
    }
}

template <int NK, int BN, int NW, bool RS2 = false>
__device__ __forceinline__ void conv_panel_body(const ConvArgs& a) {
#if defined(__HIP_DEVICE_COMPILE__)
    constexpr int TN = BN / 32;
    constexpr int SQ = BN * 12;
    static_assert(SQ % (NW * 64) == 0, "whole DMA rounds");
    constexpr int BL = SQ / (NW * 64);
    constexpr int NST = TN * 4;
    constexpr int NS = panel_stages<NK, BN>();
    constexpr bool EARLY = panel_early<NK>();
    static_assert(panel_behind_max<NK, NS, BL, NST>() <= 63, "vmcnt range");
    static_assert(NK >= 4 || (panel_behind<NK, NS, BL, NST>(0) == BL + (NK == 1 ? 2 : 1) * NST && panel_behind<NK, NS, BL, NST>(NK - 1) == BL + (NK == 1 ? 2 : NK == 2 ? 1 : 0) * NST),
                  "the short-K counts");

    extern __shared__ __attribute__((aligned(16))) v4f smem[];
    v4f* Bs = smem;
    const int tid = threadIdx.x;
    const int lane = tid & 63;
    const int wave = __builtin_amdgcn_readfirstlane(tid >> 6);
    float* patch = (float*)(smem + NS * SQ) + wave * 1024;
    const int lr = lane & 31, lh = lane >> 5;
    const int m_wave = ((int)blockIdx.x * NW + wave) * 32;
    const int ntn = a.Cout / BN;
    const int T = ntn * NK;

    const __amdgpu_buffer_rsrc_t rx = __builtin_amdgcn_make_buffer_rsrc((void*)a.x, 0, 0x80000000u, 0x00020000);
    const __amdgpu_buffer_rsrc_t rw = __builtin_amdgcn_make_buffer_rsrc((void*)a.w, 0, 0x80000000u, 0x00020000);
    const __amdgpu_buffer_rsrc_t ry = __builtin_amdgcn_make_buffer_rsrc((void*)a.y, 0, 0x80000000u, 0x00020000);
    const __amdgpu_buffer_rsrc_t rr = __builtin_amdgcn_make_buffer_rsrc((void*)(a.res ? a.res : a.y), 0, 0x80000000u, 0x00020000);

    unsigned b_voff[BL];
#pragma unroll
    for (int i = 0; i < BL; ++i) {
        const int q = i * NW * 64 + tid, row = q / 12, pos = q - row * 12;
        const int src = PEMP_SPLIT3_SWZ(row, pos);
        b_voff[i] = (unsigned)(row * a.Kpad * 6 + src * 16);
    }
    const int tile_bytes = BN * a.Kpad * 6;
#define PEMP_PANEL_DMA_SETUP(buf_, t_, n_, kt_)                                                                   \
    v4f* const Bd_ = Bs + (buf_) * SQ + wave * 64;                                                                \
    const int so_ = __builtin_amdgcn_readfirstlane((t_) < T ? (n_) * tile_bytes + (kt_) * 192 : 0);              \
    const bool in_ = (t_) < T
#define PEMP_PANEL_DMA_ONE(i_) \
    __builtin_amdgcn_raw_ptr_buffer_load_lds(rw, (lptr_t)(Bd_ + (i_) * NW * 64), 16, in_ ? b_voff[i_] : 0x80000000u, so_, 0, 0)
#define PEMP_PANEL_DMA(buf_, t_, n_, kt_)                                                                         \
    do {                                                                                                          \
        PEMP_PANEL_DMA_SETUP(buf_, t_, n_, kt_);                                                                  \
        _Pragma("unroll") for (int i = 0; i < BL; ++i) PEMP_PANEL_DMA_ONE(i);                                     \
    } while (0)

#pragma unroll
    for (int t = 0; t < NS; ++t) PEMP_PANEL_DMA(t, t, t / NK, t % NK);

    bf16x8 ah[2 * NK], am[2 * NK], al[2 * NK];
    {
        const int m = m_wave + lr;
        const bool ok = m < a.M;
        const int mm = ok ? m : 0;
        const int img = mm / a.HoWo;
        const int rem = mm - img * a.HoWo;
        const int ho = rem / a.Wo;
        const int wo = rem - ho * a.Wo;
        const unsigned off = ok ? (unsigned)(((img * a.H + ho * a.stride) * a.W + wo * a.stride) * a.ldx + 8 * lh) * 4u : 0x80000000u;
        v4f x0[2 * NK], x1[2 * NK];
#pragma unroll
        for (int s = 0; s < 2 * NK; ++s) {
            x0[s] = __builtin_bit_cast(v4f, __builtin_amdgcn_raw_buffer_load_b128(rx, off + s * 64, 0, 0));
            x1[s] = __builtin_bit_cast(v4f, __builtin_amdgcn_raw_buffer_load_b128(rx, off + s * 64 + 16, 0, 0));
        }
#pragma unroll
        for (int s = 0; s < 2 * NK; ++s) split3_bf16(x0[s], x1[s], ah[s], am[s], al[s]);
    }
    asm volatile("s_waitcnt vmcnt(0)" ::: "memory");
    __builtin_amdgcn_s_barrier();
    __builtin_amdgcn_sched_barrier(0);

    const int brow3 = lr * 12, bsw3 = (lr >> 2) & 3;
    v4f bfr[2][TN][3];
#define PEMP_PANEL_READ(dst_, buf_, j_)                                                                           \
    do {                                                                                                          \
        const v4f* Bb_ = Bs + (buf_) * SQ;                                                                        \
        const int pb_ = (2 * (j_) + lh) ^ bsw3;                                                                   \
        _Pragma("unroll") for (int ni = 0; ni < TN; ++ni)                                                         \
            _Pragma("unroll") for (int pl = 0; pl < 3; ++pl)                                                      \
                bfr[dst_][ni][pl] = Bb_[brow3 + ni * 32 * 12 + pl * 4 + pb_];                                     \
    } while (0)
#define PEMP_PANEL_MMA_HOOKED(src_, s_, HOOK_)                                                                    \
    do {                                                                                                          \
        _Pragma("unroll") for (int pr = 0; pr < 6; ++pr)                                                          \
            _Pragma("unroll") for (int ni = 0; ni < TN; ++ni) {                                                   \
                const bf16x8 av_ = pr == 0 ? al[s_] : (pr == 2 || pr == 3) ? am[s_] : ah[s_];                     \
                const bf16x8 bv_ = __builtin_bit_cast(bf16x8, bfr[src_][ni][pr == 1 ? 2 : (pr == 2 || pr == 4) ? 1 : 0]); \
                acc[ni] = __builtin_amdgcn_mfma_f32_32x32x16_bf16(av_, bv_, acc[ni], 0, 0, 0);                    \
                HOOK_(pr * TN + ni);                                                                              \
            }                                                                                                     \
    } while (0)
#define PEMP_PANEL_HOOK_NONE(j_)
#define PEMP_PANEL_MMA(src_, s_) PEMP_PANEL_MMA_HOOKED(src_, s_, PEMP_PANEL_HOOK_NONE)
#define PEMP_PANEL_HOOK_DMA(j_)                                                                                   \
    if ((j_) < BL) {                                                                                              \
        __builtin_amdgcn_sched_barrier(0);                                                                        \
        PEMP_PANEL_DMA_ONE((j_) < BL ? (j_) : 0);                                                                 \
        __builtin_amdgcn_sched_barrier(0);                                                                        \
    }
#define PEMP_PANEL_HOOK_DMA_RES(j_)                                                                               \
    PEMP_PANEL_HOOK_DMA(j_)                                                                                       \
    else if ((j_) - BL < NST && a.res) {                                                                          \
        const int k_ = (j_) - BL < NST ? (j_) - BL : 0;                                                           \
        __builtin_amdgcn_sched_barrier(0);                                                                        \
        rres[k_] = __builtin_bit_cast(v4f, __builtin_amdgcn_raw_buffer_load_b128(rr, r_off[k_ & 3] + (unsigned)(n * BN + (k_ >> 2) * 32) * 4u, 0, 0)); \
        __builtin_amdgcn_sched_barrier(0);                                                                        \
    }
    static_assert(BL + NST <= 6 * TN, "one instruction per MFMA of a slice");

    f32x16 acc[TN];
#pragma unroll
    for (int ni = 0; ni < TN; ++ni)
#pragma unroll
        for (int e = 0; e < 16; ++e) acc[ni][e] = 0.f;

    const bool relu = a.flags & PEMP_CONV_RELU;
    const int er = lane >> 3, c4 = (lane & 7) * 4;
    unsigned y_off[4], r_off[4];
#pragma unroll
    for (int i = 0; i < 4; ++i) {
        const int m = m_wave + er + 8 * i;
        y_off[i] = m < a.M ? (unsigned)(m * a.ldy + c4) * 4u : 0x80000000u;
        if constexpr (RS2) r_off[i] = m < a.M ? (unsigned)(conv_res_s2_pixel(a, m) * a.ldr + c4) * 4u : 0x80000000u;
        else r_off[i] = m < a.M ? (unsigned)(m * a.ldr + c4) * 4u : 0x80000000u;
    }

#define PEMP_PANEL_AFFINE(n_)                                                                                     \
    do {                                                                                                          \
        _Pragma("unroll") for (int ni = 0; ni < TN; ++ni) {                                                       \
            const int c = (n_) * BN + ni * 32 + c4;                                                               \
            scv[ni] = a.scale ? *(const v4f*)(a.scale + c) : v4f{1.f, 1.f, 1.f, 1.f};                             \
            shv[ni] = a.shift ? *(const v4f*)(a.shift + c) : v4f{0.f, 0.f, 0.f, 0.f};                             \
        }                                                                                                         \
    } while (0)

    int cur = 0;
    PEMP_PANEL_READ(0, 0, 0);
    for (int n = 0; n < ntn; ++n) {
        v4f rres[NST], scv[TN], shv[TN];
#pragma unroll
        for (int kt = 0; kt < NK; ++kt) {
            const int nxt = cur == NS - 1 ? 0 : cur + 1;
            PEMP_PANEL_READ(1, cur, 1);
            __builtin_amdgcn_sched_barrier(0);
            PEMP_PANEL_MMA(0, 2 * kt);
            __builtin_amdgcn_sched_barrier(0);
            panel_wait<NK, NS, BL, NST>(kt);
            __builtin_amdgcn_s_barrier();
            __builtin_amdgcn_sched_barrier(0);
            PEMP_PANEL_READ(0, nxt, 0);
            const int t3 = n * NK + kt + NS;
            const int n3 = n + (kt + NS) / NK, k3 = (kt + NS) % NK;
            if constexpr (!EARLY) {
                if (kt == NK - 1) {
                    PEMP_PANEL_AFFINE(n);
#pragma unroll
                    for (int i = 0; i < NST; ++i) rres[i] = v4f{0.f, 0.f, 0.f, 0.f};
                    if (a.res) {
#pragma unroll
                        for (int ni = 0; ni < TN; ++ni)
#pragma unroll
                            for (int i = 0; i < 4; ++i)
                                rres[ni * 4 + i] = __builtin_bit_cast(v4f, __builtin_amdgcn_raw_buffer_load_b128(rr, r_off[i] + (unsigned)(n * BN + ni * 32) * 4u, 0, 0));
                    }
                }
                __builtin_amdgcn_sched_barrier(0);
                PEMP_PANEL_DMA(cur, t3, n3, k3);
                __builtin_amdgcn_sched_barrier(0);
                PEMP_PANEL_MMA(1, 2 * kt + 1);
            } else {
                PEMP_PANEL_DMA_SETUP(cur, t3, n3, k3);
                if (kt == 0) PEMP_PANEL_AFFINE(n);
                __builtin_amdgcn_sched_barrier(0);
                if (kt == 0) PEMP_PANEL_MMA_HOOKED(1, 2 * kt + 1, PEMP_PANEL_HOOK_DMA_RES);
                else PEMP_PANEL_MMA_HOOKED(1, 2 * kt + 1, PEMP_PANEL_HOOK_DMA);
            }
            __builtin_amdgcn_sched_barrier(0);
            cur = nxt;
        }
#pragma unroll
        for (int ni = 0; ni < TN; ++ni) {
            PEMP_CONV_PATCH_PUT(patch, acc[ni], lr, lh);
            asm volatile("s_waitcnt lgkmcnt(0)" ::: "memory");
#pragma unroll
            for (int i = 0; i < 4; ++i) {
                const int row = er + 8 * i;
                const v4f v = *(const v4f*)(patch + row * 32 + c4);
                v4f add = shv[ni];
                if (a.res) add += rres[ni * 4 + i];
                const v4f o = conv_affine_quad(v, scv[ni], add, relu);
                __builtin_amdgcn_raw_buffer_store_b128(__builtin_bit_cast(v4u, o), ry, y_off[i] + (unsigned)(n * BN + ni * 32) * 4u, 0, 0);
            }
            asm volatile("s_waitcnt lgkmcnt(0)" ::: "memory");
#pragma unroll
            for (int e = 0; e < 16; ++e) acc[ni][e] = 0.f;
        }
        __builtin_amdgcn_sched_barrier(0);
    }
    asm volatile("s_waitcnt vmcnt(0)" ::: "memory");
#undef PEMP_PANEL_DMA_SETUP
#undef PEMP_PANEL_DMA_ONE
#undef PEMP_PANEL_DMA
#undef PEMP_PANEL_AFFINE
#undef PEMP_PANEL_READ
#undef PEMP_PANEL_MMA_HOOKED
#undef PEMP_PANEL_HOOK_NONE
#undef PEMP_PANEL_HOOK_DMA
#undef PEMP_PANEL_HOOK_DMA_RES
#undef PEMP_PANEL_MMA
#endif
}

template <int NK, int BN, int NW>
__global__ __launch_bounds__(NW * 64) __attribute__((amdgpu_waves_per_eu(panel_two_blocks<NK, BN>() ? 2 : 1))) void conv_panel_kernel(ConvArgs a) {
    conv_panel_body<NK, BN, NW>(a);
}

template <int NK, int BN, int NW>
__global__ __launch_bounds__(NW * 64) __attribute__((amdgpu_waves_per_eu(panel_two_blocks<NK, BN>() ? 2 : 1))) void conv_panel_rs2_kernel(ConvArgs a) {
    conv_panel_body<NK, BN, NW, true>(a);
}

constexpr int PANEL_NW = 4;
template <int NK, int BN> constexpr size_t panel_lds() { return (size_t)(panel_stages<NK, BN>() * BN * 12 + PANEL_NW * 256) * sizeof(v4f); }
static_assert(panel_lds<8, 128>() <= 160 * 1024 && 2 * panel_lds<4, 64>() <= 160 * 1024, "LDS of a CU");

template <int BN, int NK = 1>
static int launch_panel_nk(const ConvArgs& a, hipStream_t st) {
    if constexpr (NK > 8) {
        set_error("conv split3 panel: Kpad=%d above 256", a.Kpad);
        return -1;
    } else {
        if (a.nk == NK)
            return launch_with_lds(conv_panel_kernel<NK, BN, PANEL_NW>, cdiv(a.M, 32 * PANEL_NW), PANEL_NW * 64, panel_lds<NK, BN>(), st, a,
                                   "conv_panel");
        return launch_panel_nk<BN, NK + 1>(a, st);
    }
}

template <int BN, int NK>
static int launch_panel_rs2(const ConvArgs& a, hipStream_t st) {
    return launch_with_lds(conv_panel_rs2_kernel<NK, BN, PANEL_NW>, cdiv(a.M, 32 * PANEL_NW), PANEL_NW * 64, panel_lds<NK, BN>(), st, a,
                           "conv_panel/res_s2");
}

bool conv_panel_supported(const ConvArgs& a) {
    if (a.KH != 1 || a.KW != 1 || a.pad != 0 || a.nk < 1 || a.nk > 8 || a.Kpad != a.Cin || (a.flags & (PEMP_CONV_STEM4 | PEMP_CONV_SHIFT_PER_IMAGE | PEMP_CONV_BF16_IO)))
        return false;
    if (a.padv || a.stats || a.rowmask || a.sk_S > 1 || a.bm_first) return false;
    const bool rs2 = a.flags & PEMP_CONV_RES_S2;
    if (rs2 && (!a.res || a.Hr < 1 || a.Wr < 1 || (a.nk != 2 && a.nk != 4))) return false;
    const long long lim = 1ll << 31;
    const long long res_rows = rs2 ? (long long)a.N * a.Hr * a.Wr : a.M;
    return (long long)a.N * a.H * a.W * a.ldx * 4 < lim && (long long)a.M * a.ldy * 4 < lim && (!a.res || res_rows * a.ldr * 4 < lim) &&
           (long long)a.Cout * a.Kpad * 6 < lim;
}

int launch_conv_panel(int shape, const ConvArgs& a, hipStream_t st) {
    if (!conv_panel_supported(a)) {
        set_error("conv split3 panel: needs a 1x1 conv without padding, Kpad <= 256 (64 or 128 with PEMP_CONV_RES_S2), no padding value / per-image shift, operands < 2 GiB");
        return -1;
    }
    if (a.flags & PEMP_CONV_RES_S2) {
        if (kTileShapes[shape].bn == 128) {
            if (a.nk == 2) return launch_panel_rs2<128, 2>(a, st);
            set_error("conv split3 panel: PEMP_CONV_RES_S2 on tile 71 needs Kpad 64 (Kpad 128: tile 72 or 43)");
            return -1;
        }
        return a.nk == 2 ? launch_panel_rs2<64, 2>(a, st) : launch_panel_rs2<64, 4>(a, st);
    }
    return kTileShapes[shape].bn == 128 ? launch_panel_nk<128>(a, st) : launch_panel_nk<64>(a, st);
}

}
```

### pemp_amd/engine.py

```python
import copy
import os

import torch
import torch.nn as nn

from . import ops
from .ops import ConvParams

BN_EPS = 1e-5

SPLIT3 = os.environ.get("PEMP_SPLIT3", "1") != "0"


def split3_admits(cp):
    return (cp.w.dtype == torch.float32 and not cp.stem and cp.kh * cp.kw <= 32 and cp.cin % 32 == 0 and cp.cout % 64 == 0
            and cp.kpad == cp.kh * cp.kw * cp.cin)


def with_split3(cp):
    if not SPLIT3 or cp.w.dtype != torch.float32:
        return cp
    if cp.stem:
        if (cp.kh, cp.kw, cp.stride, cp.pad, cp.dil) == (7, 7, 2, 3, 1) and cp.kpad == 224 and cp.cout % 64 == 0:
            cp.w3pool = ops.pack_split3(cp.w)
    elif split3_admits(cp):
        cp.w3 = ops.pack_split3(cp.w)
    return cp


def bn_affine(bn):
    invstd = 1.0 / torch.sqrt(bn.running_var.detach().float() + bn.eps)
    alpha = bn.weight.detach().float() * invstd
    beta = bn.bias.detach().float() - bn.running_mean.detach().float() * alpha
    return alpha.contiguous(), beta.contiguous()


def conv_params(conv, bn=None, relu=False, stem4=False, in_slice=None, dtype=torch.float32):
    w = conv.weight.detach()
    if in_slice is not None:
        w = w[:, in_slice[0]:in_slice[1]]
    packed, kpad = ops.pack_conv_weight(w, stem4=stem4)
    cout, cin = w.shape[0], w.shape[1]
    scale = shift = None
    if bn is not None:
        scale, shift = bn_affine(bn)
        if conv.bias is not None:
            shift = shift + conv.bias.detach().float() * scale
    elif conv.bias is not None:
        shift = conv.bias.detach().float().contiguous()
    return with_split3(ConvParams(packed.contiguous().to(dtype), scale, shift, 4 if stem4 else cin, cout, conv.kernel_size[0],
                                  conv.kernel_size[1], conv.stride[0], conv.padding[0], conv.dilation[0], kpad, stem4, relu))


def pack_padded_in(conv, cin_pad, relu):
    w = conv.weight.detach().float()
    co, ci, kh, kw = w.shape
    wp = torch.zeros((co, kh, kw, cin_pad), dtype=torch.float32, device=w.device)
    wp[..., :ci] = w.permute(0, 2, 3, 1)
    return with_split3(ConvParams(wp.reshape(co, kh * kw * cin_pad).contiguous(), None, conv.bias.detach().float().contiguous(),
                                  cin_pad, co, kh, kw, 1, conv.padding[0], conv.dilation[0], kh * kw * cin_pad, False, relu))


def classifier2(conv):
    cin, dev = conv.weight.shape[1], conv.weight.device
    w = torch.zeros((64, cin), dtype=torch.float32, device=dev)
    w[:2] = conv.weight.detach().float()[:, :, 0, 0]
    b = torch.zeros(64, dtype=torch.float32, device=dev)
    b[:2] = conv.bias.detach().float()
    return with_split3(ConvParams(w.contiguous(), None, b.contiguous(), cin, 64, 1, 1, 1, 0, 1, cin, False, False))


def logits_nchw(c, pred):
    ops.resize_bilinear_ac(c[..., :2], tuple(c.shape[1:3]), out=pred.permute(0, 2, 3, 1))
    return pred


def pack_episode(arena, groups, priors=None):
    H, W = groups[0].shape[-2:]
    x4 = arena.get("x4", (sum(g.shape[0] for g in groups), H, W, 4), torch.float32)
    o = 0
    for i, g in enumerate(groups):
        ops.pack_input(g.contiguous(), None if priors is None else priors[i], out=x4[o:o + g.shape[0]])
        o += g.shape[0]
    return x4


GROUP_MAX_ROWS = int(os.environ.get("PEMP_EVAL_GROUP_ROWS", "12000"))


PRESPLIT_WIDTHS = (128, 256)
PRESPLIT_MIN_TILES = None


def presplit_pair(prod, cons, x, rows, enabled=True):
    if not (enabled and ops.SPLIT3_PRESPLIT and x.dtype == torch.float32 and x.is_cuda and prod.w3 is not None and cons.w3 is not None
            and not prod.stem and cons.kh * cons.kw > 1 and cons.cin % 32 == 0 and cons.cout % 128 == 0 and cons.cout in PRESPLIT_WIDTHS):
        return False
    least = torch.cuda.get_device_properties(x.device).multi_processor_count if PRESPLIT_MIN_TILES is None else PRESPLIT_MIN_TILES
    return -(-rows // 256) * (cons.cout // 128) >= least


PRESPLIT_ASPP = True


PRUNE_ROWS = os.environ.get("PEMP_PRUNE_ROWS", "1") != "0"


def restrided(cp, stride):
    return ConvParams(cp.w, cp.scale, cp.shift, cp.cin, cp.cout, cp.kh, cp.kw, stride, cp.pad, cp.dil, cp.kpad, cp.stem, cp.relu,
                      cp.w3, cp.w3pool)


def presplit_readers(prod, readers, x, rows, enabled=True):
    multi = [c for c in readers if c.kh * c.kw > 1]
    return bool(multi) and all(presplit_pair(prod, c, x, rows, enabled and PRESPLIT_ASPP) for c in multi)


class Arena:

    def __init__(self, device, dtype=torch.float32):
        self.device = device
        self.dtype = dtype
        self.bufs = {}
        self.ws = {}

    def get(self, name, shape, dtype=None, zero=False):
        dtype = self.dtype if dtype is None else dtype
        key = (name, tuple(shape), dtype)
        t = self.bufs.get(key)
        if t is None:
            t = (torch.zeros if zero else torch.empty)(shape, dtype=dtype, device=self.device)
            self.bufs[key] = t
        return t


class _BlockPlan:
    def __init__(self, blk, extra_in=0, dtype=torch.float32):
        sl = None
        if extra_in:
            sl = (0, blk.conv1.weight.shape[1] - extra_in)
        self.c1 = conv_params(blk.conv1, blk.bn1, relu=True, in_slice=sl, dtype=dtype)
        self.c2 = conv_params(blk.conv2, blk.bn2, relu=True, dtype=dtype)
        self.c3 = conv_params(blk.conv3, blk.bn3, relu=True, dtype=dtype)
        self.ds = conv_params(blk.downsample[0], blk.downsample[1], relu=False, in_slice=sl, dtype=dtype) \
            if blk.downsample is not None else None
        if extra_in:
            self.c1_extra = (blk.conv1.weight.detach()[:, sl[1]:, 0, 0].float() * self.c1.scale[:, None]).contiguous()
            self.ds_extra = (blk.downsample[0].weight.detach()[:, sl[1]:, 0, 0].float() * self.ds.scale[:, None]).contiguous()


class _BottleneckTrunk:
    GROUP_DS = True
    PRESPLIT = True

    def _block(self, x, bp, tag, c1_shift=None, ds_shift=None, out=None, prune=False):
        if prune:
            bp = self._pruned_plan(bp)
        a = self.arena
        n, h, w, _ = x.shape
        h1, w1 = (ops.conv_out_size(v, k, bp.c1.stride, bp.c1.pad, bp.c1.dil) for v, k in ((h, bp.c1.kh), (w, bp.c1.kw)))
        ho, wo = (ops.conv_out_size(v, k, bp.c2.stride, bp.c2.pad, bp.c2.dil) for v, k in ((h1, bp.c2.kh), (w1, bp.c2.kw)))
        if out is None:
            out = a.get(("blk", tag), (n, ho, wo, bp.c3.cout))
        res = a.get("res", (n, ho, wo, bp.ds.cout)) if bp.ds is not None else x
        grouped = self.GROUP_DS and bp.ds is not None and c1_shift is None and ds_shift is None \
            and 0 < n * ho * wo <= GROUP_MAX_ROWS and x.dtype == torch.float32
        pre = presplit_pair(bp.c1, bp.c2, x, n * ho * wo, self.PRESPLIT and not grouped)
        y1 = a.get("y1s", ops.split3_shape(n, h1, w1, bp.c1.cout), torch.bfloat16) if pre else a.get("y1", (n, h1, w1, bp.c1.cout))
        if grouped:
            ops.conv2d_group([x, x], [bp.c1, bp.ds], [y1, res])
        else:
            ops.conv2d(x, bp.c1, out=y1, shift_override=c1_shift, per_image_shift=c1_shift is not None, out_split3=pre)
        y2 = ops.conv2d(y1, bp.c2, out=a.get("y2", (n, ho, wo, bp.c2.cout)), x_split3=pre)
        if bp.ds is not None and not grouped:
            ops.conv2d(x, bp.ds, out=res, shift_override=ds_shift, per_image_shift=ds_shift is not None)
        return ops.conv2d(y2, bp.c3, out=out, residual=res, residual_stride=2 if prune else 1)

    def _plan_copy(self, bp, what, **convs):
        cache = self.__dict__.setdefault("_plan_copies", {})
        key = (id(bp), what)
        if key not in cache:
            q = copy.copy(bp)
            for name, cp in convs.items():
                setattr(q, name, cp)
            cache[key] = (bp, q)
        return cache[key][1]

    def _pruned_plan(self, bp):
        if bp.ds is not None:
            raise ValueError("row pruning: the block has a downsample conv of its own")
        return self._plan_copy(bp, "pruned", c2=restrided(bp.c2, 2 * bp.c2.stride))

    def _compact_plan(self, bp):
        return self._plan_copy(bp, "compact", c1=restrided(bp.c1, 1), ds=restrided(bp.ds, 1))

    def _stage(self, x, si, final_out=None, compact_in=False, prune=False):
        blocks = self.stages[si]
        for bi, bp in enumerate(blocks):
            last = bi == len(blocks) - 1
            if bi == 0 and compact_in:
                bp = self._compact_plan(bp)
            x = self._block(x, bp, (si, bi & 1), out=final_out if last else None, prune=prune and last)
        return x

    def _prunes(self, si, stage_outs=None):
        if not PRUNE_ROWS or self.arena.dtype != torch.float32 or si + 1 >= len(self.stages) or (stage_outs and si in stage_outs):
            return False
        last, nxt = self.stages[si][-1], self.stages[si + 1][0]
        if len(self.stages[si]) < 2 or last.ds is not None or nxt.ds is None:
            return False
        if any(c.w3 is None for c in (last.c1, last.c2, last.c3, nxt.c1, nxt.ds)):
            return False
        if any((c.kh, c.kw, c.pad, c.stride) != (1, 1, 0, 2) for c in (nxt.c1, nxt.ds)):
            return False
        return (last.c3.kh, last.c3.kw, last.c3.pad, last.c3.stride) == (1, 1, 0, 1) and bool(ops.res_s2_tiles(last.c3))


class ResNetEngine(_BottleneckTrunk):

    def __init__(self, prm, arena):
        self.arena = arena
        self.stem = conv_params(prm.conv1, prm.bn1, relu=True, stem4=True)
        self.stages = []
        for name in ("layer1", "layer2", "layer3"):
            self.stages.append([_BlockPlan(b, dtype=arena.dtype) for b in getattr(prm, name)])

    def stem_forward(self, x4):
        a = self.arena
        n, h, w, _ = x4.shape
        ho, wo = ops.conv_out_size(h, 7, 2, 3, 1), ops.conv_out_size(w, 7, 2, 3, 1)
        if a.dtype == torch.float32 and ops.stem_pool_supported(self.stem):
            hp, wp = ops._pool_out(ho, 3, 2, 1, True), ops._pool_out(wo, 3, 2, 1, True)
            return ops.stem_pool(x4, self.stem, out=a.get("pool", (n, hp, wp, 64), torch.float32))
        y = ops.conv2d(x4, self.stem, out=a.get("stem", (n, ho, wo, 64), torch.float32))
        hp, wp = ops._pool_out(ho, 3, 2, 1, True), ops._pool_out(wo, 3, 2, 1, True)
        x = ops.maxpool2d(y, 3, 2, 1, ceil_mode=True, out=a.get("pool", (n, hp, wp, 64), torch.float32))
        if a.dtype != torch.float32:
            x = ops.convert(x, a.get("pool16", (n, hp, wp, 64)))
        return x

    def forward(self, x4, stage_outs=None):
        x = self.stem_forward(x4)
        pruned = False
        for si in range(len(self.stages)):
            prune = self._prunes(si, stage_outs)
            x = self._stage(x, si, stage_outs.get(si) if stage_outs else None, compact_in=pruned, prune=prune)
            pruned = prune
        return x


class ResNetCMEngine(ResNetEngine):

    def __init__(self, prm, arena):
        self.arena = arena
        self.spq = prm.spq
        self.stem = conv_params(prm.conv1, prm.bn1, relu=True, stem4=True)
        self.stages = []
        for name in ("layer1", "layer2", "layer3"):
            blocks = list(getattr(prm, name))
            self.stages.append([_BlockPlan(blocks[0], extra_in=2)] + [_BlockPlan(b) for b in blocks[1:]])
        self.lin = [(l.weight.detach().float().contiguous(), l.bias.detach().float().contiguous())
                    for l in (prm.linear1, prm.linear2, prm.linear3)]
        self.group = None

    def _comm(self, x, mask, lin, stride):
        mask, stat = ops.cm_reduce(x, mask, stride)
        _, feat = ops.cm_linear(stat, self.group, lin[0], lin[1], self.n_groups)
        return feat, mask

    def forward(self, x4, prior):
        mask = ops.cm_reduce(None, prior, 2)[0]
        x = self.stem_forward(x4)
        strides = (2, 1, 2)
        for si, blocks in enumerate(self.stages):
            feat, mask = self._comm(x, mask, self.lin[si], strides[si])
            b0 = blocks[0]
            c1_shift = ops.cm_bias(feat, self.group, b0.c1_extra, base=b0.c1.shift)
            ds_shift = ops.cm_bias(feat, self.group, b0.ds_extra, base=b0.ds.shift)
            x = self._block(x, b0, (si, 0), c1_shift, ds_shift)
            for bi, bp in enumerate(blocks[1:], start=1):
                x = self._block(x, bp, (si, bi & 1))
        return x


class VGG16CMEngine:
    PADC = 32

    def __init__(self, prm, arena):
        from .networks.backbones import VGG_CM_LAYOUT
        self.arena, self.spq = arena, prm.spq
        self.stages = []
        first = True
        for si, (name, nconv, cout, d, pool) in enumerate(VGG_CM_LAYOUT):
            seq = getattr(prm, name)
            convs = []
            for k in range(nconv):
                conv = seq[2 * k]
                relu = not (pool is None and k == nconv - 1 and not prm.last_relu)
                if k == 0 and not first:
                    convs.append(pack_padded_in(conv, conv.weight.shape[1] - 2 + self.PADC, relu))
                else:
                    convs.append(conv_params(conv, None, relu=relu, stem4=first and k == 0))
            self.stages.append((convs, cout, pool))
            first = False
        self.lin = [(l.weight.detach().float().contiguous(), l.bias.detach().float().contiguous())
                    for l in (prm.linear1, prm.linear2, prm.linear3, prm.linear4)]
        self.group, self.n_groups = None, 0

    def forward(self, x4, prior):
        a = self.arena
        x, mask = x4, prior
        for si, (convs, cout, pool) in enumerate(self.stages):
            for k, cp in enumerate(convs):
                n, h, w, _ = x.shape
                x = ops.conv2d(x, cp, out=a.get(("vcm", si, k & 1), (n, h, w, cp.cout)))
            if pool is None:
                return x
            n, h, w, c = x.shape
            ho, wo = ops._pool_out(h, 3, pool, 1, False), ops._pool_out(w, 3, pool, 1, False)
            wide = a.get(("vcm_cat", si), (n, ho, wo, c + self.PADC), zero=True)
            xs = ops.maxpool2d(x, 3, pool, 1, out=wide[..., :c])
            mask, stat = ops.cm_reduce(xs, mask, pool)
            _, feat = ops.cm_linear(stat, self.group, self.lin[si][0], self.lin[si][1], self.n_groups)
            wide[..., c:c + 2] = feat.index_select(0, self.group.long()).view(n, 1, 1, 2)
            x = wide
        return x
# ... 169 lines not shown
```

### pemp_amd/ops.py

```python
import ctypes as C
import collections
import functools
import json
import os

import torch

from . import _lib
from ._lib import ConvDesc, CONV_RELU, CONV_SHIFT_PER_IMAGE, CONV_STEM4, CONV_POOL3S2, CONV_OUT_SPLIT3, CONV_IN_SPLIT3, CONV_OUT_SPLIT3_ALSO
from ._lib import CONV_RES_S2, CONV_RES_HEVEN, CONV_RES_WEVEN


def _stream():
    return C.c_void_p(torch.cuda.current_stream().cuda_stream)


def _p(t):
    return C.c_void_p(t.data_ptr()) if t is not None else C.c_void_p(0)


def _chk_dev(*ts):
    for t in ts:
        if t is not None and (not t.is_cuda):
            raise _lib.PempHipError("pemp_amd ops need device (cuda/HIP) tensors; there is no CPU path")


def _nhwc(t, name, dtype=torch.float32):
    if t.dim() != 4 or t.dtype != dtype or t.stride(3) != 1:
        raise ValueError(f"{name}: expected {dtype} NHWC view with unit channel stride, got {tuple(t.shape)} {t.dtype} {t.stride()}")
    n, h, w, c = t.shape
    if w > 1:
        ld = t.stride(2)
    elif h > 1:
        ld = t.stride(1)
    elif n > 1:
        ld = t.stride(0)
    else:
        ld = c
    if (w > 1 and h > 1 and t.stride(1) != w * ld) or (h * w > 1 and n > 1 and t.stride(0) != h * w * ld):
        raise ValueError(f"{name}: pixels must be densely packed with stride ld={ld}, got strides {t.stride()}")
    return ld


def conv_out_size(i, k, s, p, d):
    return (i + 2 * p - d * (k - 1) - 1) // s + 1


class ConvParams:
    __slots__ = ("w", "scale", "shift", "cin", "cout", "kh", "kw", "stride", "pad", "dil", "kpad", "stem", "relu", "w3", "w3pool")

    def __init__(self, w, scale, shift, cin, cout, kh, kw, stride, pad, dil, kpad, stem, relu, w3=None, w3pool=None):
        self.w, self.scale, self.shift, self.w3, self.w3pool = w, scale, shift, w3, w3pool
        self.cin, self.cout, self.kh, self.kw = cin, cout, kh, kw
        self.stride, self.pad, self.dil, self.kpad, self.stem, self.relu = stride, pad, dil, kpad, stem, relu


_SHAPES = {1: (128, 128), 2: (128, 64), 3: (64, 64), 4: (128, 128), 5: (128, 64), 6: (256, 128), 7: (256, 256),
           8: (32, 64),
           9: (64, 64)}
Tile = collections.namedtuple("Tile", "shape family splitk persistent_of")
SPLIT3_PERSISTENT = {47: 43, 49: 46}
TILES = {base + s: Tile(_SHAPES[s], family, base in (30, 50), None)
         for family, base, shapes in (("igemm", 0, (1, 2, 3)),
                                      ("dma", 10, range(1, 8)),
                                      ("dma2", 20, range(1, 10)),
                                      ("dma2", 30, (1, 2, 4, 5, 6, 7)),
                                      ("split3", 40, (1, 2, 3, 4, 6)),
                                      ("split3", 50, (1, 2, 4, 6)))
         for s in shapes}
TILES.update({t: TILES[of]._replace(persistent_of=of) for t, of in SPLIT3_PERSISTENT.items()})
TILES.update({70 + s: Tile(_SHAPES[s], "split3", False, None) for s in (1, 2)})
TILES.update({146: Tile(_SHAPES[6], "split3", False, None), 149: Tile(_SHAPES[6], "split3", False, 146)})
TILES.update({246: Tile(_SHAPES[6], "split3", False, None), 249: Tile(_SHAPES[6], "split3", False, 246)})
TILES.update({349: Tile(_SHAPES[6], "split3", False, 46)})
_NO_TILE = Tile(None, None, False, None)


def tile_shape(t):
    return TILES.get(t, _NO_TILE).shape


TILE_VARIANTS = {t: TILES[t].shape for t in (13, 14, 12, 11, 15, 3, 17, 16, 23, 24, 22, 21, 25, 27, 26, 28, 29)}
SPLIT3_TILES = (43, 42, 41, 44, 46, 47, 49)
SPLIT3_SPLITK_TILES = (51, 52, 54, 56)
SPLIT3_DEFAULT_TILE = 43
SPLIT3_PANEL_TILES = (71, 72)
SPLIT3_PANEL = os.environ.get("PEMP_SPLIT3_PANEL", "1") != "0"
SPLIT3_PRESPLIT_TILES = (146, 149)
SPLIT3_PRESPLIT = os.environ.get("PEMP_SPLIT3_PRESPLIT", "1") != "0"
SPLIT3_ROW3_TILES = (246, 249)
SPLIT3_ROW3 = os.environ.get("PEMP_SPLIT3_ROW3", "1") != "0"
ROW3_STAGE_ROWS = 288
SPLIT3_RING_TILES = (349,)
SPLIT3_RING = os.environ.get("PEMP_SPLIT3_RING", "1") != "0"
RING_MIN_K = 128
AUTOTUNE = True
PICK_HOOK = None
SPLITK = os.environ.get("PEMP_CONV_SPLITK", "1") != "0"
DEFAULT_TILE = 13
_TILE_CACHE = {}
_TILE_CACHE_FILE = os.environ.get("PEMP_TILE_CACHE")
WGRAD_PICKS = {}
if _TILE_CACHE_FILE and os.path.exists(_TILE_CACHE_FILE):
    with open(_TILE_CACHE_FILE) as _f:
        for _k, _v in json.load(_f).items():
            _key = json.loads(_k)
            if _key and _key[0] == "wgrad":
                WGRAD_PICKS[tuple(_key[1:])] = tuple(_v) if isinstance(_v, list) else int(_v)
            else:
                _TILE_CACHE[tuple(_key)] = int(_v)


def save_picks():
    if not _TILE_CACHE_FILE:
        return
    out = {json.dumps([int(v) for v in k]): t for k, t in _TILE_CACHE.items()}
    out.update({json.dumps(["wgrad"] + [int(v) for v in k]): (list(t) if isinstance(t, tuple) else t) for k, t in WGRAD_PICKS.items()})
    with open(_TILE_CACHE_FILE, "w") as f:
        json.dump(out, f)


def concurrent_stream(device, priority=0, tries=6, us=200):
    lib = _lib.load()
    cur = torch.cuda.current_stream(device)
    _lib.check(lib.pemp_spin_us(1, C.c_void_p(cur.cuda_stream)), "pemp_spin_us")
    cur.synchronize()
    keep = []
    for _ in range(tries):
        cand = torch.cuda.Stream(device=device, priority=priority)
        keep.append(cand)
        cand.wait_stream(cur)
        e0, e1 = torch.cuda.Event(enable_timing=True), torch.cuda.Event(enable_timing=True)
        e0.record(cur)
        _lib.check(lib.pemp_spin_us(us, C.c_void_p(cur.cuda_stream)), "pemp_spin_us")
        _lib.check(lib.pemp_spin_us(us, C.c_void_p(cand.cuda_stream)), "pemp_spin_us")
        cur.wait_stream(cand)
        e1.record(cur)
        e1.synchronize()
        if e0.elapsed_time(e1) * 1e3 < 1.6 * us:
            return cand
    return keep[-1]


def export_picks():
    return {"tiles": dict(_TILE_CACHE), "wgrad": dict(WGRAD_PICKS)}


def import_picks(picks):
    _TILE_CACHE.update(picks["tiles"])
    WGRAD_PICKS.update(picks["wgrad"])


def tuned_by_rank0(warm):
    import torch.distributed as dist
    if not (dist.is_available() and dist.is_initialized()) or dist.get_world_size() == 1:
        warm()
        return
    rank = dist.get_rank()
    if rank == 0:
        warm()
    box = [export_picks() if rank == 0 else None]
    dist.broadcast_object_list(box, src=0)
    if rank != 0:
# ... 154 lines not shown
        ldr = _nhwc(residual, "residual", dtype)
        if residual_stride == 2:
            rn, hr, wr, rc = residual.shape
            if (rn, rc) != (n, p.cout) or (hr - 1) // 2 + 1 != ho or (wr - 1) // 2 + 1 != wo:
                raise ValueError(f"{who}: a stride-2 residual of shape {tuple(residual.shape)} does not cover the output {tuple(out.shape)}")
        elif tuple(residual.shape) != tuple(out.shape):
            raise ValueError(f"{who}: residual shape mismatch")
    elif residual_stride != 1:
        raise ValueError(f"{who}: residual_stride without a residual")
    return n, h, w, cin, ldx, ho, wo, out, ldy, ldr


def conv2d(x, p, out=None, residual=None, shift_override=None, per_image_shift=False, relu=None, tile=0,
           pad_value=None, splitk=False, dropblock=None, out_split3=False, x_split3=False, also_split3=None, residual_stride=1):
    if out_split3 or x_split3:
        what = "a pre-split output" if out_split3 else "a pre-split input"
        if p.w3 is None or p.stem:
            raise ValueError(f"conv2d: {what} needs a split3 layer (ConvParams.w3), not the fp32 chain or a stem")
        if splitk or dropblock is not None:
            raise ValueError(f"conv2d: {what} has no split-K / DropBlock form")
        if out_split3 and tile and (tile not in SPLIT3_TILES + SPLIT3_PRESPLIT_TILES + SPLIT3_RING_TILES):
            raise ValueError(f"conv2d: a pre-split output needs an unsplit split3 tile id, got {tile}")
        if x_split3 and (p.kh * p.kw == 1 or per_image_shift or p.cin % 32 or p.cout % 128):
            raise ValueError("conv2d: a pre-split input needs a multi-tap conv with Cin % 32 == 0 and Cout % 128 == 0, no per-image shift")
    if also_split3 is not None and (not x_split3 or out_split3 or residual is not None):
        raise ValueError("conv2d: a second, pre-split output needs a pre-split input (x_split3), no out_split3, no residual")
    if (tile in SPLIT3_PRESPLIT_TILES + SPLIT3_ROW3_TILES) != bool(x_split3) and (tile or not x_split3):
        raise ValueError(f"conv2d: the tile ids {SPLIT3_PRESPLIT_TILES + SPLIT3_ROW3_TILES} and x_split3 come together (tile {tile})")
    res_s2 = residual_stride == 2
    if residual_stride not in (1, 2):
        raise ValueError(f"conv2d: residual_stride must be 1 or 2, got {residual_stride}")
    if res_s2:
        if p.w3 is None or p.stem or x.dtype != torch.float32:
            raise ValueError("conv2d: a stride-2 residual needs a split3 layer (ConvParams.w3) on fp32 activations")
        if residual is None or out_split3 or x_split3 or also_split3 is not None or pad_value is not None or splitk or dropblock is not None:
            raise ValueError("conv2d: a stride-2 residual comes with a residual and without pre-split operands, padding value, split-K or DropBlock")
        if tile and tile not in res_s2_tiles(p):
            raise ValueError(f"conv2d: a stride-2 residual needs one of the tile ids {res_s2_tiles(p)} for this layer, got {tile}")
    if x.dtype == torch.bfloat16 and not x_split3:
        return _conv2d_bf16(x, p, out, residual, shift_override, per_image_shift, relu, tile, pad_value)
    n, h, w, cin, ldx, ho, wo, out, ldy, ldr = _conv_geom("conv2d", x, p, out, residual, x_split3=x_split3, out_split3=out_split3,
                                                          residual_stride=residual_stride)
    if also_split3 is not None and _split3_dims(also_split3, "also_split3") != (n, ho, wo, p.cout):
        raise ValueError(f"conv2d: also_split3 shape {tuple(also_split3.shape)} != {split3_shape(n, ho, wo, p.cout)}")
    lib = _lib.load()
    _chk_dev(x, p.w, out, residual, also_split3)
    if also_split3 is not None:
        residual = also_split3
    shift = p.shift if shift_override is None else shift_override
    if pad_value is not None:
        _chk_dev(pad_value)
        if x_split3:
            if tuple(pad_value.shape) != (cin // 32, 3, 32) or pad_value.dtype != torch.bfloat16 or not pad_value.is_contiguous():
                raise ValueError(f"conv2d: with x_split3, pad_value must be a contiguous bf16 [{cin // 32}, 3, 32] split vector")
        elif pad_value.numel() != cin or pad_value.dtype != torch.float32 or not pad_value.is_contiguous():
            raise ValueError(f"conv2d: pad_value must be a contiguous fp32 [{cin}] vector")
    flags = (CONV_OUT_SPLIT3 if out_split3 else 0) | (CONV_IN_SPLIT3 if x_split3 else 0) | (CONV_OUT_SPLIT3_ALSO if also_split3 is not None else 0)
    if (p.relu if relu is None else relu):
        flags |= CONV_RELU
    if per_image_shift:
        flags |= CONV_SHIFT_PER_IMAGE
    if p.stem:
        flags |= CONV_STEM4
    if res_s2:
        flags |= CONV_RES_S2 | (CONV_RES_HEVEN if residual.shape[1] % 2 == 0 else 0) | (CONV_RES_WEVEN if residual.shape[2] % 2 == 0 else 0)
    splitk = ((splitk and SPLITK) or (EVAL_SPLITK and n * ho * wo <= EVAL_SPLITK_MAX_ROWS)) and not p.stem \
        and not out_split3 and not x_split3 and not res_s2
    if x_split3:
        s3 = _presplit_ok(x, p, pad_value)
    else:
        s3 = p.w3 is not None and dropblock is None and dma2_supported(x, p) and _group_member_ok(x, p, pad_value)
    if (out_split3 or x_split3) and not s3:
        raise ValueError("conv2d: pre-split activations need a geometry of the buffer-addressed kernels (<= 32 taps, operands < 2 GiB, "
                         "a padding value behind the activations)")
    if res_s2 and not (s3 and residual.numel() // p.cout * ldr < 1 << 31):
        raise ValueError("conv2d: a stride-2 residual needs a geometry of the buffer-addressed kernels and a residual below 2^31 elements")

    if dropblock is not None:
        dmask, dcnt = dropblock
        _chk_dev(dmask, dcnt)
        if (pad_value is not None or p.stem or dmask.dtype != torch.float32 or not dmask.is_contiguous() or dmask.numel() != n * ho * wo
                or dcnt.dtype != torch.int32 or not dma2_supported(x, p)):
            from . import train_ops
            y = conv2d(x, p, out=out, residual=residual, shift_override=shift_override, per_image_shift=per_image_shift, relu=relu,
                       tile=tile, pad_value=pad_value, splitk=splitk)
            return train_ops.pixel_scale(y, dmask, dcnt, out=y)

    def launch(t):
        d = ConvDesc(n, h, w, cin, ldx, ho, wo, p.cout, ldy, p.kh, p.kw, p.stride, p.pad, p.dil, ldr, p.kpad, flags, t)
        tl = TILES.get(t, _NO_TILE)
        pw, sk = p.w3 if tl.family == "split3" else p.w, tl.splitk
        if dropblock is not None:
            ws, ws_bytes = _splitk_ws(lib, d, x.device) if sk else (None, 0)
            _check_sk(lib, lib.pemp_conv2d_dropblock_nhwc_f32(C.byref(d), _p(x), _p(pw), _p(out), _p(p.scale), _p(shift), _p(residual),
                                                              _p(dropblock[0]), _p(dropblock[1]), C.c_void_p(ws), ws_bytes, _stream()),
                      ws, "pemp_conv2d_dropblock_nhwc_f32")
            return
        if sk and pad_value is not None:
            ws, ws_bytes = _splitk_ws(lib, d, x.device)
            _check_sk(lib, lib.pemp_conv2d_padv_splitk_nhwc_f32(C.byref(d), _p(x), _p(pw), _p(out), _p(p.scale), _p(shift), _p(residual),
                                                                _p(pad_value), C.c_void_p(ws), ws_bytes, _stream()), ws,
                      "pemp_conv2d_padv_splitk_nhwc_f32")
        elif sk:
            ws, ws_bytes = _splitk_ws(lib, d, x.device)
            _check_sk(lib, lib.pemp_conv2d_splitk_nhwc_f32(C.byref(d), _p(x), _p(pw), _p(out), _p(p.scale), _p(shift), _p(residual),
                                                           C.c_void_p(ws), ws_bytes, _stream()), ws, "pemp_conv2d_splitk_nhwc_f32")
        elif pad_value is None:
            _lib.check(lib.pemp_conv2d_nhwc_f32(C.byref(d), _p(x), _p(pw), _p(out), _p(p.scale), _p(shift),
                                                _p(residual), _stream()), "pemp_conv2d_nhwc_f32")
        else:
            _lib.check(lib.pemp_conv2d_padv_nhwc_f32(C.byref(d), _p(x), _p(pw), _p(out), _p(p.scale), _p(shift),
                                                     _p(residual), _p(pad_value), _stream()), "pemp_conv2d_padv_nhwc_f32")

    if tile == 0:
        key = (p.cin, p.cout, p.kh, p.kw, p.stride, p.pad, p.dil, (6 if dropblock is not None else 4) if splitk else int(p.stem) + (7 if dropblock is not None else 0),
               n, h, w, int(residual is not None and also_split3 is None), int(pad_value is not None)) + ((3,) if s3 else ())
        if x_split3 or out_split3:
            key += (146,) * int(x_split3) + (17,) * int(out_split3) + (64,) * int(also_split3 is not None)
            row3 = bool(x_split3) and _row3_ok(p, w, residual, pad_value, out_split3, also_split3, per_image_shift)
            if row3:
                key += (246,)
            ring = _ring_ok(p, x_split3, residual, pad_value, also_split3, splitk)
            if ring:
                key += (349,)
            cands = lambda: _fits(list(SPLIT3_PRESPLIT_TILES if x_split3 else SPLIT3_TILES) +
                                  (list(SPLIT3_ROW3_TILES) if row3 and PICK_HOOK is None else []) +
                                  (list(SPLIT3_RING_TILES) if ring else []), p.cout)
        elif res_s2:
            panel = _panel_ok(p, n, ho, wo, ldx, ldy, ldr, h, w, pad_value, splitk, per_image_shift) \
                and residual.numel() // p.cout * ldr * 4 < 1 << 31
            key += (128,) + ((71,) if panel else ())
            cands = lambda: _fits([t for t in res_s2_tiles(p) if panel or t not in SPLIT3_PANEL_TILES], p.cout)
        elif s3:
            panel = _panel_ok(p, n, ho, wo, ldx, ldy, ldr, h, w, pad_value, splitk, per_image_shift)
            ring = _ring_ok(p, x_split3, residual, pad_value, also_split3, splitk)
            if ring:
                key += (349,)
            if panel:
                key += (71,)
            cands = lambda: _fits(list(SPLIT3_TILES) + (list(SPLIT3_SPLITK_TILES) if splitk else []) +
                                  (list(SPLIT3_RING_TILES) if ring else []) + (list(SPLIT3_PANEL_TILES) if panel else []), p.cout)
        else:
            def cands():
                ids = list(GROUP_TILES if dropblock is not None else TILE_VARIANTS) + (list(SPLITK_TILES) if splitk else [])
                if 29 in ids and not (hybrid_rows(n, ho, wo, p.cout) and dma2_supported(x, p)):
                    ids.remove(29)
                return _fits(ids, p.cout)
        tile = _choose_tile(key, n * ho * wo, launch, cands,
                            SPLIT3_PRESPLIT_TILES[0] if x_split3 else SPLIT3_DEFAULT_TILE if s3 else DEFAULT_TILE + (10 if dropblock is not None else 0))
    launch(tile)
    return out


def stem_pool_supported(p):
    return (p.stem and p.w3pool is not None and (p.kh, p.kw, p.stride, p.pad, p.dil) == (7, 7, 2, 3, 1) and p.kpad == 224
            and p.cout % 64 == 0)


def stem_pool(x, p, out=None):
    lib = _lib.load()
    if not stem_pool_supported(p):
        raise ValueError("stem_pool: a 7x7 / stride 2 / pad 3 NHWC4 stem with split weights (ConvParams.w3pool)")
    _chk_dev(x, p.w3pool, out)
    ldx = _nhwc(x, "x")
    n, h, w, cin = x.shape
    if cin != p.cin or x.dtype != torch.float32:
        raise ValueError(f"stem_pool: fp32 NHWC4 input expected, got {cin} channels of {x.dtype}")
    ho, wo = conv_out_size(h, 7, 2, 3, 1), conv_out_size(w, 7, 2, 3, 1)
    hp, wp = _pool_out(ho, 3, 2, 1, True), _pool_out(wo, 3, 2, 1, True)
    if out is None:
        out = torch.empty((n, hp, wp, p.cout), dtype=torch.float32, device=x.device)
    ldy = _nhwc(out, "out")
    if tuple(out.shape) != (n, hp, wp, p.cout) or out.dtype != torch.float32:
        raise ValueError(f"stem_pool: out shape {tuple(out.shape)} != {(n, hp, wp, p.cout)} (fp32)")
    flags = CONV_STEM4 | CONV_POOL3S2 | (CONV_RELU if p.relu else 0)
    d = ConvDesc(n, h, w, cin, ldx, ho, wo, p.cout, ldy, 7, 7, 2, 3, 1, 0, p.kpad, flags, SPLIT3_DEFAULT_TILE)
    _lib.check(lib.pemp_conv2d_nhwc_f32(C.byref(d), _p(x), _p(p.w3pool), _p(out), _p(p.scale), _p(p.shift), None, _stream()),
               "pemp_conv2d_nhwc_f32")
    return out


def _conv2d_bf16(x, p, out, residual, shift_override, per_image_shift, relu, tile, pad_value):
    lib = _lib.load()
    _chk_dev(x, p.w, out, residual, pad_value)
    if p.w.dtype != torch.bfloat16 or p.stem:
        raise ValueError("conv2d (bf16 input): the layer's weights must be packed as bf16 (engine precision 'bf16'); no stem")
    n, h, w, cin, ldx, ho, wo, out, ldy, ldr = _conv_geom("conv2d", x, p, out, residual, torch.bfloat16,
                                                          None if out is None else out.dtype)
    out_f32 = out.dtype == torch.float32
    if pad_value is not None and (pad_value.numel() != cin or pad_value.dtype != torch.bfloat16 or not pad_value.is_contiguous()):
        raise ValueError(f"conv2d: pad_value must be a contiguous bf16 [{cin}] vector")
    shift = p.shift if shift_override is None else shift_override
    flags = (CONV_RELU if (p.relu if relu is None else relu) else 0) | (CONV_SHIFT_PER_IMAGE if per_image_shift else 0)

    def launch(t):
        d = ConvDesc(n, h, w, cin, ldx, ho, wo, p.cout, ldy, p.kh, p.kw, p.stride, p.pad, p.dil, ldr, p.kpad, flags, t)
        _lib.check(lib.pemp_conv2d_bf16_nhwc(C.byref(d), _p(x), _p(p.w), _p(out), _p(p.scale), _p(shift), _p(residual), _p(pad_value),
                                             1 if out_f32 else 0, _stream()), "pemp_conv2d_bf16_nhwc")

    if tile == 0:
        key = (p.cin, p.cout, p.kh, p.kw, p.stride, p.pad, p.dil, 5, n, h, w, int(residual is not None), int(pad_value is not None))
        tile = _choose_tile(key, n * ho * wo, launch, lambda: _fits(GROUP_TILES, p.cout), 24 if p.cout % 128 == 0 else 23)
    launch(tile)
    return out


def convert(x, out):
    lib = _lib.load()
    _chk_dev(x, out)
    if not x.is_contiguous() or not out.is_contiguous() or x.numel() != out.numel() or x.numel() % 4:
        raise ValueError("convert: contiguous tensors of the same size (a multiple of 4 elements)")
    if x.dtype == torch.float32 and out.dtype == torch.bfloat16:
        _lib.check(lib.pemp_convert_f32_bf16(_p(x), _p(out), x.numel(), _stream()), "convert_f32_bf16")
    elif x.dtype == torch.bfloat16 and out.dtype == torch.float32:
        _lib.check(lib.pemp_convert_bf16_f32(_p(x), _p(out), x.numel(), _stream()), "convert_bf16_f32")
    else:
        raise ValueError(f"convert: {x.dtype} -> {out.dtype} is not one of fp32 <-> bf16")
    return out


GROUP_TILES = (23, 22, 25, 21, 24, 26, 27)
GROUP_MAX = 4


def _group_member_ok(x, p, pad_value):
    n, h, w, _ = x.shape
    ldx = _nhwc(x, "x")
    taps = p.kh * p.kw
    tapmax = (p.dil * (p.kh - 1) * w + p.dil * (p.kw - 1)) * ldx * 4
    xbytes = (n * h * w + p.pad * w + p.pad) * ldx * 4 + tapmax
    if p.stem or taps > 32 or xbytes >= 2 ** 31 or p.w.numel() * 4 >= 2 ** 31:
        return False
    if pad_value is not None:
        off = pad_value.data_ptr() - x.data_ptr()
        d = off + (p.pad * w + p.pad) * ldx * 4
        if off < n * h * w * ldx * 4 or d < tapmax or d + p.cin * 4 >= 2 ** 31:
            return False
    return True


def _presplit_ok(x, p, pad_value):
    n, h, w = x.shape[:3]
    row = p.cin * 6
    tapmax = (p.dil * (p.kh - 1) * w + p.dil * (p.kw - 1)) * row
    if p.kh * p.kw > 32 or (n * h * w + p.pad * w + p.pad) * row + tapmax >= 2 ** 31 or p.w3.numel() * 2 >= 2 ** 31:
        return False
    if pad_value is not None:
        off = pad_value.data_ptr() - x.data_ptr()
        d = off + (p.pad * w + p.pad) * row
        if off < n * h * w * row or d < tapmax or d + row >= 2 ** 31:
            return False
    return True


def conv2d_group(xs, ps, outs, pad_values=None, residuals=None, tile=0):
    lib = _lib.load()
    n = len(ps)
    if not 1 <= n <= GROUP_MAX or len(xs) != n or len(outs) != n:
        raise ValueError(f"conv2d_group: 1..{GROUP_MAX} members with one input and one output each")
    pad_values = list(pad_values) if pad_values is not None else [None] * n
    residuals = list(residuals) if residuals is not None else [None] * n
    descs, keys = [], []
    for x, p, out, pv, res in zip(xs, ps, outs, pad_values, residuals):
        _chk_dev(x, p.w, out, pv, res)
        if p.stem:
            raise ValueError("conv2d_group: no stem convs")
        if out is None:
            raise ValueError("conv2d_group: every member needs its output")
        nb, h, w, cin, ldx, ho, wo, out, ldy, ldr = _conv_geom("conv2d_group", x, p, out, res)
        descs.append((nb, h, w, cin, ldx, ho, wo, p.cout, ldy, p.kh, p.kw, p.stride, p.pad, p.dil, ldr, p.kpad, CONV_RELU if p.relu else 0))
        keys += [p.cin, p.cout, p.kh, p.stride, p.pad, p.dil, nb, h, w, int(res is not None), int(pv is not None)]
    s3 = all(p.w3 is not None for p in ps)
    if not all(_group_member_ok(x, p, pv) for x, p, pv in zip(xs, ps, pad_values)) or (not s3 and any(p.w3 is not None for p in ps)):
        for x, p, out, pv, res in zip(xs, ps, outs, pad_values, residuals):
            conv2d(x, p, out=out, residual=res, pad_value=pv if p.kh * p.kw > 1 else None)
        return outs
    arr = lambda ts: (C.c_void_p * n)(*[(t.data_ptr() if t is not None else None) for t in ts])
    xa, wa, ya = arr(xs), arr([p.w3 if s3 else p.w for p in ps]), arr(outs)
    sa, ha, ra, pa = arr([p.scale for p in ps]), arr([p.shift for p in ps]), arr(residuals), arr(pad_values)
    ptr = lambda a: C.cast(a, C.POINTER(C.c_void_p))

    def launch(t):
        da = (ConvDesc * n)(*[ConvDesc(*d, t) for d in descs])
        _lib.check(lib.pemp_conv2d_group_nhwc_f32(n, da, ptr(xa), ptr(wa), ptr(ya), ptr(sa), ptr(ha), ptr(ra), ptr(pa), _stream()),
                   "pemp_conv2d_group_nhwc_f32")

    if tile == 0:
        key = (-8 if s3 else -7,) + tuple(keys)
        couts = [p.cout for p in ps]
        if s3:
            cands = lambda: _fits([t for t in SPLIT3_TILES if t not in SPLIT3_PERSISTENT], *couts)
        else:
            cands = lambda: _fits(GROUP_TILES + (28,), *couts)
        tile = _choose_tile(key, max(d[0] * d[5] * d[6] for d in descs), launch, cands, SPLIT3_DEFAULT_TILE if s3 else DEFAULT_TILE + 10)
    launch(tile)
    return outs


SPLITK_TILES = (31, 32, 34, 35, 36, 37)
EVAL_SPLITK = os.environ.get("PEMP_EVAL_SPLITK", "0") == "1"
EVAL_SPLITK_MAX_ROWS = int(os.environ.get("PEMP_EVAL_SPLITK_MAX_ROWS", "12000"))
_SK_WS = {}
SK_SCOPE = 0
_SK_WS_BYTES = 72 << 20


# ... 1065 lines not shown
```

### scratch/s3_layers_bench.py

```python
import argparse
import hashlib
import os
import sys

import torch

sys.path.insert(0, os.path.dirname(os.path.dirname(os.path.abspath(__file__))))
from pemp_amd import ops

UNSPLIT = (43, 42, 41, 44, 46, 47, 49)
SPLIT = (52, 51, 54, 56)
PANEL = ops.SPLIT3_PANEL_TILES
PRESPLIT = ops.SPLIT3_PRESPLIT_TILES
RING = getattr(ops, "SPLIT3_RING_TILES", ())
ROW3 = ops.SPLIT3_ROW3_TILES
LAYERS = ((256, 1024, 1, 1, True, False), (512, 1024, 1, 1, False, False), (1024, 256, 1, 1, False, False),
          (256, 256, 3, 2, False, False), (128, 512, 1, 1, True, False), (1024, 512, 1, 1, False, False),
          (256, 256, 3, 2, False, True),
          (64, 256, 1, 1, True, False, 1, 101), (64, 256, 1, 1, False, False, 1, 101), (256, 512, 1, 1, False, False, 2, 101),
          (128, 128, 3, 1, False, False), (128, 128, 3, 1, False, False, 2, 101), (64, 64, 3, 1, False, False, 1, 101),
          (512, 128, 1, 1, False, False),
          (512, 256, 1, 1, False, False), (256, 256, 1, 1, False, False),
          (64, 256, 1, 1, True, False, 1, 51, 101),
          (64, 64, 3, 1, False, False, 2, 101),
          (256, 256, 3, 12, False, True))


def timed(fn, reps, n=5):
    for _ in range(2):
        fn()
    e0, e1 = torch.cuda.Event(enable_timing=True), torch.cuda.Event(enable_timing=True)
    best, worst = 1e9, 0.0
    for _ in range(reps):
        e0.record()
        for _ in range(n):
            fn()
        e1.record()
        e1.synchronize()
        us = e0.elapsed_time(e1) / n * 1e3
        best, worst = min(best, us), max(worst, us)
    return best, worst


def presplit(x):
    h = x.to(torch.bfloat16)
    r = x - h.float()
    m = r.to(torch.bfloat16)
    lo = (r - m.float()).to(torch.bfloat16)
    return torch.stack([p.reshape(*x.shape[:-1], x.shape[-1] // 32, 32) for p in (h, m, lo)], dim=-2).contiguous()


def digest(t):
    return hashlib.sha1(t.cpu().numpy().tobytes()).hexdigest()[:16]


def rs2_row(dev, N, HW, HR, cin, cout, name, keep, reps):
    g = torch.Generator().manual_seed(cin * 7 + cout * 3 + 1001)
    x = torch.randn(N * HW * HW, cin, generator=g).to(dev).view(N, HW, HW, cin)
    w = (torch.randn(cout, cin, 1, 1, generator=g) * (1.0 / cin ** 0.5)).to(dev)
    packed, kpad = ops.pack_conv_weight(w)
    packed = packed.contiguous()
    prm = ops.ConvParams(packed, None, torch.randn(cout, generator=g).to(dev), cin, cout, 1, 1, 1, 0, 1, kpad, False, True, ops.pack_split3(packed))
    res = torch.randn(N, HR, HR, cout, generator=g).to(dev)
    ref = ops.conv2d(x, prm, residual=res[:, ::2, ::2, :].contiguous(), tile=43).clone()
    out = torch.empty_like(ref)
    fl = 2.0 * N * HW * HW * cout * cin
    cells = []
    for tile in keep(ops.res_s2_tiles(prm)):
        run = lambda: ops.conv2d(x, prm, residual=res, residual_stride=2, out=out, tile=tile)
        out.zero_()
        run()
        same = torch.equal(out, ref)
        us, worst = timed(run, reps)
        cells.append(f"{tile}: {us:7.1f}..{worst:6.1f}us {fl / us / 1e6:5.1f}TF{'' if same else ' !'}")
    print(f"{name:>16} k1 d1 res1 | " + " | ".join(cells), flush=True)
    print(f"{'':>16} hash 43={digest(ref)}", flush=True)


def main():
    ap = argparse.ArgumentParser()
    ap.add_argument("--only", default="", help="cin-cout-kK[-padv]: one layer")
    ap.add_argument("--reps", type=int, default=3)
    ap.add_argument("--ids", default="", help="comma-separated tile ids: only these are timed (a counter run of one kernel)")
    ap.add_argument("--producers", action="store_true", help="with --ids: time the selected ids as producers of a pre-split output too")
    ap.add_argument("--res", type=int, choices=(0, 1), default=None, help="run the selected layers without / with a residual, whatever their row says")
    args = ap.parse_args()
    dev = torch.device("cuda:0")
    N = 50
    keep = lambda ids: tuple(t for t in ids if not args.ids or str(t) in args.ids.split(","))
    for layer in LAYERS:
        cin, cout, k, dil, has_res, padv = layer[:6]
        stride, HW = layer[6:8] if len(layer) > 6 else (1, 51)
        RS2 = layer[8] if len(layer) > 8 else 0
        has_res = has_res if args.res is None or RS2 else bool(args.res)
        M = N * HW * HW
        HO = (HW - 1) // stride + 1
        name = f"{cin}-{cout}-k{k}" + (f"-d{dil}" if k == 3 and dil > 2 else "") + ("-padv" if padv else "") + (f"-s{stride}" if stride > 1 else "") + (f"-hw{HW}-res{int(has_res)}" if HW != 51 else "") + ("-rs2" if RS2 else "")
        if args.only and name not in args.only.split(","):
            continue
        if RS2:
            rs2_row(dev, N, HW, RS2, cin, cout, name, keep, args.reps)
            continue
        g = torch.Generator().manual_seed(cin * 7 + cout * 3 + k)
        buf = torch.empty(M + 4, cin, device=dev)
        buf[:M] = torch.randn(M, cin, generator=g).to(dev)
        buf[M:] = torch.randn(cin, generator=g).to(dev)
        x, pv = buf[:M].view(N, HW, HW, cin), buf[M]
        w = (torch.randn(cout, cin, k, k, generator=g) * (1.0 / (cin * k * k) ** 0.5)).to(dev)
        packed, kpad = ops.pack_conv_weight(w)
        packed = packed.contiguous()
        prm = ops.ConvParams(packed, None, torch.randn(cout, generator=g).to(dev), cin, cout, k, k, stride, dil if k == 3 else 0, dil, kpad,
                             False, True, ops.pack_split3(packed))
        res = torch.randn(N, HO, HO, cout, generator=g).to(dev) if has_res else None
        pad_value = pv if padv else None
        out = torch.empty(N, HO, HO, cout, device=dev)
        fl = 2.0 * N * HO * HO * cout * k * k * cin
        ref = ops.conv2d(x, prm, residual=res, pad_value=pad_value, tile=43).clone()
        cells, hashes = [], [f"43={digest(ref)}"]
        panel = PANEL if k == 1 and kpad <= 256 and not padv else ()
        ring = RING if k == 1 and kpad >= 128 and not has_res and not padv and cout % 128 == 0 else ()
        for tile in keep(UNSPLIT + ring + panel + SPLIT):
            if cout % ops._tile_bn(tile):
                continue
            run = lambda: ops.conv2d(x, prm, residual=res, pad_value=pad_value, out=out, tile=tile)
            run()
            same = torch.equal(out, ref)
            if tile in SPLIT:
                hashes.append(f"{tile}=" + ("43" if same else digest(out)))
            us, worst = timed(run, args.reps)
            mark = "" if same else (" ~" if tile in SPLIT else " !")
            cells.append(f"{tile}: {us:7.1f}..{worst:6.1f}us {fl / us / 1e6:5.1f}TF{mark}")
            if tile not in SPLIT and not same:
                hashes.append(f"{tile}=MISMATCH:{digest(out)}")
        if k > 1 and cout % 128 == 0:
            sbuf = torch.zeros((M + 4) * cin * 3, dtype=torch.bfloat16, device=dev)
            sbuf[:(M + 1) * cin * 3] = presplit(buf[:M + 1]).reshape(-1)
            xs, pvs = sbuf[:M * cin * 3].view(N, HW, HW, cin // 32, 3, 32), sbuf[M * cin * 3:(M + 1) * cin * 3].view(cin // 32, 3, 32)
            row3 = ROW3 if k == 3 and stride == 1 and not has_res and not padv and ops.row3_stage_rows(HW, dil) <= ops.ROW3_STAGE_ROWS else ()
            for tile in keep(PRESPLIT + row3):
                run = lambda: ops.conv2d(xs, prm, residual=res, pad_value=pvs if padv else None, out=out, tile=tile, x_split3=True)
                out.zero_()
                run()
                same = torch.equal(out, ref)
                us, worst = timed(run, args.reps)
                cells.append(f"{tile}: {us:7.1f}..{worst:6.1f}us {fl / us / 1e6:5.1f}TF{'' if same else ' !'}")
            if not has_res:
                want = presplit(ref)
                outs = torch.empty_like(want)
                for tile in keep(PRESPLIT):
                    run = lambda: ops.conv2d(xs, prm, pad_value=pvs if padv else None, out=out, tile=tile, x_split3=True, also_split3=outs)
                    out.zero_()
                    run()
                    same = torch.equal(out, ref) and torch.equal(outs.view(torch.int16), want.view(torch.int16))
                    us, worst = timed(run, args.reps)
                    cells.append(f"{tile}+s: {us:7.1f}..{worst:6.1f}us{'' if same else ' !'}")
                del want, outs
            del sbuf, xs, pvs
        if k == 1 and not has_res:
            want = presplit(ref)
            outs = torch.empty_like(want)
            for tile in keep((43, 42, 41, 44, 46, 47, 49) + ring if not args.ids or args.producers else ()):
                if cout % ops._tile_bn(tile):
                    continue
                run = lambda: ops.conv2d(x, prm, out=outs, tile=tile, out_split3=True)
                run()
                same = torch.equal(outs.view(torch.int16), want.view(torch.int16))
                us, worst = timed(run, args.reps)
                cells.append(f"{tile}s: {us:7.1f}..{worst:6.1f}us{'' if same else ' !'}")
            del want, outs
        print(f"{name:>16} k{k} d{dil} res{int(has_res)} | " + " | ".join(cells), flush=True)
        print(f"{'':>16} hash " + " ".join(hashes), flush=True)
    print("(146 / 149 / 246 / 249: on the pre-split input; NNs: id NN writing a pre-split output, ! = not the split of id 43's;")
    print(" NNN+s: id NNN writing fp32 and the pre-split copy, ! = either differs)")
    print("(! = an unsplit id differs from id 43; ~ = a split-K id differs from id 43, expected where it splits)")


if __name__ == "__main__":
    main()
```

Before: 1559.

## Fuse bottleneck downsample shortcut conv into c3 conv as one K-concatenated panel kernel

Adds a panel kernel that computes the 1x1 downsample shortcut and the c3 1x1 conv together by concatenating their K dimensions (64+64). Each output tile applies the shortcut and main scale/shift separately and adds them in registers. This is meant to remove the separate shortcut conv launch and the write and re-read of the residual tensor in the first layer1 block. The model wires it in when the shapes match. It adds a new kernel, a cached per-layer concatenated weight pack, and a shared scheduling header split out of conv_panel.hip.

Result: no change. 1569, median of 6 (+0.7%).

```diff
diff --git a/include/pemp_hip.h b/include/pemp_hip.h
--- a/include/pemp_hip.h
+++ b/include/pemp_hip.h
@@ -20,6 +20,7 @@
 #define PEMP_CONV_RES_S2 128u
 #define PEMP_CONV_RES_HEVEN 512u
 #define PEMP_CONV_RES_WEVEN 1024u
+#define PEMP_CONV_SHORTCUT 2048u
 
 typedef struct pemp_conv_desc {
     int32_t N, H, W;
diff --git a/pemp_amd/_lib.py b/pemp_amd/_lib.py
--- a/pemp_amd/_lib.py
+++ b/pemp_amd/_lib.py
@@ -38,6 +38,7 @@
 CONV_RES_S2 = 128
 CONV_RES_HEVEN = 512
 CONV_RES_WEVEN = 1024
+CONV_SHORTCUT = 2048
 
 SYMBOLS = {
     "pemp_last_error": (C.c_char_p, []),
diff --git a/pemp_amd/build.py b/pemp_amd/build.py
--- a/pemp_amd/build.py
+++ b/pemp_amd/build.py
@@ -7,7 +7,7 @@
 CSRC = os.path.join(HERE, "csrc")
 OBJ = os.path.join(HERE, "_obj")
 OUT = os.path.join(HERE, "libpemp_hip.so")
-SOURCES = ("conv_igemm.hip", "conv_dma.hip", "conv_dma2.hip", "conv_panel.hip", "conv_row3.hip", "conv_ring.hip", "conv_stem_pool.hip", "conv_wgrad.hip", "train_ops.hip", "pool_misc.hip", "head.hip", "head_bwd.hip", "cedt.hip",
+SOURCES = ("conv_igemm.hip", "conv_dma.hip", "conv_dma2.hip", "conv_panel.hip", "conv_panel_sc.hip", "conv_row3.hip", "conv_ring.hip", "conv_stem_pool.hip", "conv_wgrad.hip", "train_ops.hip", "pool_misc.hip", "head.hip", "head_bwd.hip", "cedt.hip",
            "episode_io.hip", "dropout.hip", "cm_linear.hip", "pfenet.hip", "pfenet_bwd.hip", "canet.hip", "canet_bwd.hip", "rpmms.hip", "rpmms_bwd.hip")
 FLAGS = ["-O3", "--offload-arch=gfx950", "-std=c++17", "-fPIC"]
 
@@ -27,7 +27,7 @@
     return h.hexdigest()[:12]
 
 
-CONV_ENGINE = ("common.h", "conv_common.h", "conv_tiles.h", "conv_igemm.hip", "conv_dma.hip", "conv_dma2.hip", "conv_panel.hip", "conv_row3.hip", "conv_ring.hip", "conv_stem_pool.hip")
+CONV_ENGINE = ("common.h", "conv_common.h", "conv_tiles.h", "conv_panel_sched.h", "conv_igemm.hip", "conv_dma.hip", "conv_dma2.hip", "conv_panel.hip", "conv_panel_sc.hip", "conv_row3.hip", "conv_ring.hip", "conv_stem_pool.hip")
 
 
 def conv_digest():
diff --git a/pemp_amd/csrc/conv_common.h b/pemp_amd/csrc/conv_common.h
--- a/pemp_amd/csrc/conv_common.h
+++ b/pemp_amd/csrc/conv_common.h
@@ -393,6 +393,8 @@
 int launch_conv_dma2_split3_pre(int shape, bool persistent, const ConvArgs& a, hipStream_t st);
 bool conv_panel_supported(const ConvArgs& a);
 int launch_conv_panel(int shape, const ConvArgs& a, hipStream_t st);
+bool conv_panel_sc_supported(const ConvArgs& a);
+int launch_conv_panel_sc(const ConvArgs& a, hipStream_t st);
 bool conv_row3_supported(const ConvArgs& a);
 int launch_conv_row3(bool persistent, const ConvArgs& a, hipStream_t st);
 bool conv_ring_supported(const ConvArgs& a);
diff --git a/pemp_amd/csrc/conv_igemm.hip b/pemp_amd/csrc/conv_igemm.hip
--- a/pemp_amd/csrc/conv_igemm.hip
+++ b/pemp_amd/csrc/conv_igemm.hip
@@ -247,6 +247,8 @@
     PEMP_REQUIRE(pooled || !(d->flags & PEMP_CONV_POOL3S2), "conv2d: PEMP_CONV_POOL3S2 belongs to pemp_conv2d_nhwc_f32 (no grouped / dropblock / statistics / bf16 form)");
     PEMP_REQUIRE(pooled || !(d->flags & (PEMP_CONV_RES_S2 | PEMP_CONV_RES_HEVEN | PEMP_CONV_RES_WEVEN)),
                  "conv2d: PEMP_CONV_RES_S2 belongs to pemp_conv2d_nhwc_f32 (no grouped / dropblock / statistics / bf16 form)");
+    PEMP_REQUIRE(pooled || !(d->flags & PEMP_CONV_SHORTCUT),
+                 "conv2d: PEMP_CONV_SHORTCUT belongs to pemp_conv2d_nhwc_f32 (no grouped / dropblock / statistics / bf16 form)");
     PEMP_REQUIRE(!pad_value || (!(d->flags & PEMP_CONV_STEM4) && (any_taps || d->KH * d->KW > 1) && ((uintptr_t)pad_value & 15) == 0),
                  "conv2d: pad_value needs a multi-tap non-stem conv and a 16-byte aligned [Cin] vector");
     PEMP_REQUIRE(d->N > 0 && d->H > 0 && d->W > 0 && d->Cin > 0 && d->Cout > 0, "conv2d: bad dims");
@@ -266,7 +268,7 @@
         PEMP_REQUIRE(d->Kpad % 32 == 0 && d->Kpad >= ntaps * 4, "conv2d: STEM4 Kpad=%d too small / not x32", d->Kpad);
     } else {
         PEMP_REQUIRE(d->Cin % 32 == 0, "conv2d: Cin=%d must be a multiple of 32 (or use STEM4)", d->Cin);
-        PEMP_REQUIRE(d->ldx >= d->Cin && d->ldx % 4 == 0, "conv2d: ldx=%d must be >= Cin and a multiple of 4", d->ldx);
+        PEMP_REQUIRE(d->ldx >= ((d->flags & PEMP_CONV_SHORTCUT) ? d->Cin / 2 : d->Cin) && d->ldx % 4 == 0, "conv2d: ldx=%d must be >= Cin and a multiple of 4", d->ldx);
         PEMP_REQUIRE(d->Kpad == ntaps * d->Cin, "conv2d: Kpad=%d must equal KH*KW*Cin=%d", d->Kpad, ntaps * d->Cin);
     }
     const long long in_elems = (long long)d->N * d->H * d->W * d->ldx;
@@ -284,7 +286,10 @@
     a.ntaps = ntaps;
     a.cin_steps = stem ? 1 : d->Cin / 32;
     a.nk = d->Kpad / 32;
-    if (residual && !(d->flags & PEMP_CONV_OUT_SPLIT3_ALSO)) PEMP_REQUIRE(d->ldr >= d->Cout && d->ldr % 4 == 0 && ((uintptr_t)residual & 15) == 0, "conv2d: ldr must be >= Cout and x4, residual 16-byte aligned");
+    if (residual && (d->flags & PEMP_CONV_SHORTCUT))
+        PEMP_REQUIRE(d->ldr >= d->Cin / 2 && d->ldr % 4 == 0 && ((uintptr_t)residual & 15) == 0,
+                     "conv2d: PEMP_CONV_SHORTCUT: ldr must be >= Cin / 2 and x4, the shortcut's input 16-byte aligned");
+    else if (residual && !(d->flags & PEMP_CONV_OUT_SPLIT3_ALSO)) PEMP_REQUIRE(d->ldr >= d->Cout && d->ldr % 4 == 0 && ((uintptr_t)residual & 15) == 0, "conv2d: ldr must be >= Cout and x4, residual 16-byte aligned");
     a.sk_ws = nullptr; a.sk_cnt = nullptr; a.sk_full = 0; a.sk_S = 1;
     a.bm_first = 0;
     return 0;
@@ -301,6 +306,22 @@
         tile = 3;
     }
     TileId t = decode_tile(tile);
+    if (d->flags & PEMP_CONV_SHORTCUT) {
+        PEMP_REQUIRE(d->tile == 72, "conv2d: PEMP_CONV_SHORTCUT needs tile id 72 (tile %d: no other id has the fused form)", d->tile);
+        PEMP_REQUIRE(residual, "conv2d: PEMP_CONV_SHORTCUT takes the shortcut's input in the residual argument");
+        PEMP_REQUIRE(!(d->flags & (PEMP_CONV_OUT_SPLIT3 | PEMP_CONV_IN_SPLIT3 | PEMP_CONV_OUT_SPLIT3_ALSO)), "conv2d: PEMP_CONV_SHORTCUT: no pre-split operands");
+        PEMP_REQUIRE(!(d->flags & (PEMP_CONV_RES_S2 | PEMP_CONV_RES_HEVEN | PEMP_CONV_RES_WEVEN)), "conv2d: PEMP_CONV_SHORTCUT: not with PEMP_CONV_RES_S2");
+        PEMP_REQUIRE(!(d->flags & PEMP_CONV_SHIFT_PER_IMAGE), "conv2d: PEMP_CONV_SHORTCUT: no per-image shift");
+        PEMP_REQUIRE(!(d->flags & (PEMP_CONV_STEM4 | PEMP_CONV_POOL3S2 | PEMP_CONV_BF16_IO)), "conv2d: PEMP_CONV_SHORTCUT: no stem form");
+        PEMP_REQUIRE(!ws, "conv2d: PEMP_CONV_SHORTCUT: no split-K / workspace");
+        PEMP_REQUIRE(!pad_value, "conv2d: PEMP_CONV_SHORTCUT: no padding value");
+        PEMP_REQUIRE(a.KH == 1 && a.KW == 1 && a.pad == 0 && a.stride == 1 && a.H == a.Ho && a.W == a.Wo,
+                     "conv2d: PEMP_CONV_SHORTCUT needs a 1x1 conv at stride 1 without padding: both inputs lie on the output's grid");
+        PEMP_REQUIRE(a.Kpad == 128, "conv2d: PEMP_CONV_SHORTCUT needs Cin = Kpad = 128 (shortcut K 64 + main K 64), got Kpad %d", a.Kpad);
+        PEMP_REQUIRE(scale && shift, "conv2d: PEMP_CONV_SHORTCUT needs the [2][Cout] scale and shift");
+        PEMP_REQUIRE(conv_panel_sc_supported(a), "conv2d: PEMP_CONV_SHORTCUT needs operands < 2 GiB");
+        return launch_conv_panel_sc(a, (hipStream_t)stream);
+    }
     if (t.ring) {
         PEMP_REQUIRE(!ws && !pad_value && conv_ring_supported(a),
                      "conv2d: tile %d unsupported: needs a 1x1 conv without padding on fp32 activations with Kpad == Cin >= 128 and Cout %% 128 == 0, the "
@@ -501,7 +522,7 @@
 static TileId stats_tile(const pemp_conv_desc* d) { return decode_tile(d->tile == 0 ? 23 : d->tile); }
 
 static int conv_stats_fill(const char* what, const pemp_conv_desc* d, ConvArgs& a) {
-    PEMP_REQUIRE(!(d->flags & (PEMP_CONV_STEM4 | PEMP_CONV_RELU | PEMP_CONV_SHIFT_PER_IMAGE | PEMP_CONV_POOL3S2 | PEMP_CONV_OUT_SPLIT3 | PEMP_CONV_IN_SPLIT3 | PEMP_CONV_OUT_SPLIT3_ALSO | PEMP_CONV_RES_S2 | PEMP_CONV_RES_HEVEN | PEMP_CONV_RES_WEVEN)), "%s: plain conv only (no stem / ReLU / per-image shift)", what);
+    PEMP_REQUIRE(!(d->flags & (PEMP_CONV_STEM4 | PEMP_CONV_RELU | PEMP_CONV_SHIFT_PER_IMAGE | PEMP_CONV_POOL3S2 | PEMP_CONV_OUT_SPLIT3 | PEMP_CONV_IN_SPLIT3 | PEMP_CONV_OUT_SPLIT3_ALSO | PEMP_CONV_RES_S2 | PEMP_CONV_RES_HEVEN | PEMP_CONV_RES_WEVEN | PEMP_CONV_SHORTCUT)), "%s: plain conv only (no stem / ReLU / per-image shift)", what);
     PEMP_REQUIRE(d->N > 0 && d->H > 0 && d->W > 0 && d->Cin > 0 && d->Cout > 0 && d->KH > 0 && d->KW > 0 && d->stride > 0 && d->dil > 0 && d->pad >= 0,
                  "%s: bad geometry", what);
     const int ho = (d->H + 2 * d->pad - d->dil * (d->KH - 1) - 1) / d->stride + 1;
diff --git a/pemp_amd/csrc/conv_panel.hip b/pemp_amd/csrc/conv_panel.hip
--- a/pemp_amd/csrc/conv_panel.hip
+++ b/pemp_amd/csrc/conv_panel.hip
@@ -1,40 +1,6 @@
-#include "conv_tiles.h"
+#include "conv_panel_sched.h"
 
 namespace pemp {
-
-typedef __attribute__((address_space(3))) void* lptr_t;
-typedef __attribute__((ext_vector_type(4))) unsigned int v4u;
-
-template <int NK> constexpr bool panel_early() { return NK >= 4; }
-template <int NK, int BN> constexpr bool panel_two_blocks() { return BN == 64 && NK <= 4; }
-template <int NK, int BN> constexpr int panel_stages() {
-    if (!panel_early<NK>()) return 3;
-    if (NK == 4) return 5;
-    return BN == 64 ? 8 : 6;
-}
-template <int NK, int NS, int BL, int NST>
-constexpr int panel_behind(int kt) {
-    int c = 0;
-    for (int u = kt + 1 - NS; u <= kt - 1; ++u) {
-        const int ku = ((u % NK) + NK) % NK;
-        if (u > kt + 1 - NS) c += BL;
-        if (ku == NK - 1) c += NST;
-    }
-    return c;
-}
-template <int NK, int NS, int BL, int NST>
-constexpr int panel_behind_max() {
-    int m = 0;
-    for (int kt = 0; kt < NK; ++kt) m = panel_behind<NK, NS, BL, NST>(kt) > m ? panel_behind<NK, NS, BL, NST>(kt) : m;
-    return m;
-}
-template <int NK, int NS, int BL, int NST, int KT = 0>
-__device__ __forceinline__ void panel_wait(int kt) {
-    if constexpr (KT < NK) {
-        if (kt == KT) asm volatile("s_waitcnt vmcnt(%0) lgkmcnt(0)" ::"n"(panel_behind<NK, NS, BL, NST>(KT)) : "memory");
-        else panel_wait<NK, NS, BL, NST, KT + 1>(kt);
-    }
-}
 
 template <int NK, int BN, int NW, bool RS2 = false>
 __device__ __forceinline__ void conv_panel_body(const ConvArgs& a) {
@@ -263,8 +229,6 @@
     conv_panel_body<NK, BN, NW, true>(a);
 }
 
-constexpr int PANEL_NW = 4;
-template <int NK, int BN> constexpr size_t panel_lds() { return (size_t)(panel_stages<NK, BN>() * BN * 12 + PANEL_NW * 256) * sizeof(v4f); }
 static_assert(panel_lds<8, 128>() <= 160 * 1024 && 2 * panel_lds<4, 64>() <= 160 * 1024, "LDS of a CU");
 
 template <int BN, int NK = 1>
diff --git a/pemp_amd/csrc/conv_panel_sc.hip b/pemp_amd/csrc/conv_panel_sc.hip
--- /dev/null
+++ b/pemp_amd/csrc/conv_panel_sc.hip
@@ -0,0 +1,236 @@
+#include "conv_panel_sched.h"
+
+namespace pemp {
+
+template <int NKS, int NKM, int BN, int NW>
+__device__ __forceinline__ void conv_panel_sc_body(const ConvArgs& a) {
+#if defined(__HIP_DEVICE_COMPILE__)
+    constexpr int NK = NKS + NKM;
+    constexpr int TN = BN / 32;
+    using Stream = PanelStream<NK, BN, NW>;
+    constexpr int SQ = Stream::SQ;
+    constexpr int BL = Stream::BL;
+    constexpr int NST = Stream::NST;
+    constexpr int NS = Stream::NS;
+    static_assert(panel_early<NK>() && panel_two_blocks<NK, BN>(), "the long-K schedule at two blocks per CU");
+    static_assert(Stream::behind_max() <= 63, "vmcnt range");
+    static_assert(BL <= 6 * TN, "one instruction per MFMA of a slice");
+
+    extern __shared__ __attribute__((aligned(16))) v4f smem[];
+    v4f* Bs = smem;
+    const int tid = threadIdx.x;
+    const int lane = tid & 63;
+    const int wave = __builtin_amdgcn_readfirstlane(tid >> 6);
+    float* patch = (float*)(smem + NS * SQ) + wave * 1024;
+    const int lr = lane & 31, lh = lane >> 5;
+    const int m_wave = ((int)blockIdx.x * NW + wave) * 32;
+    const int ntn = a.Cout / BN;
+    const int T = ntn * NK;
+
+    const __amdgpu_buffer_rsrc_t rx = __builtin_amdgcn_make_buffer_rsrc((void*)a.x, 0, 0x80000000u, 0x00020000);
+    const __amdgpu_buffer_rsrc_t rs = __builtin_amdgcn_make_buffer_rsrc((void*)a.res, 0, 0x80000000u, 0x00020000);
+    const __amdgpu_buffer_rsrc_t rw = __builtin_amdgcn_make_buffer_rsrc((void*)a.w, 0, 0x80000000u, 0x00020000);
+    const __amdgpu_buffer_rsrc_t ry = __builtin_amdgcn_make_buffer_rsrc((void*)a.y, 0, 0x80000000u, 0x00020000);
+
+    unsigned b_voff[BL];
+#pragma unroll
+    for (int i = 0; i < BL; ++i) {
+        const int q = i * NW * 64 + tid, row = q / 12, pos = q - row * 12;
+        const int src = PEMP_SPLIT3_SWZ(row, pos);
+        b_voff[i] = (unsigned)(row * a.Kpad * 6 + src * 16);
+    }
+    const int tile_bytes = BN * a.Kpad * 6;
+#define PEMP_PANEL_DMA_SETUP(buf_, t_, n_, kt_)                                                                   \
+    v4f* const Bd_ = Bs + (buf_) * SQ + wave * 64;                                                                \
+    const int so_ = __builtin_amdgcn_readfirstlane((t_) < T ? (n_) * tile_bytes + (kt_) * 192 : 0);              \
+    const bool in_ = (t_) < T
+#define PEMP_PANEL_DMA_ONE(i_) \
+    __builtin_amdgcn_raw_ptr_buffer_load_lds(rw, (lptr_t)(Bd_ + (i_) * NW * 64), 16, in_ ? b_voff[i_] : 0x80000000u, so_, 0, 0)
+
+#pragma unroll
+    for (int t = 0; t < NS; ++t) {
+        PEMP_PANEL_DMA_SETUP(t, t, t / NK, t % NK);
+#pragma unroll
+        for (int i = 0; i < BL; ++i) PEMP_PANEL_DMA_ONE(i);
+    }
+
+    bf16x8 ah[2 * NK], am[2 * NK], al[2 * NK];
+    {
+        const int m = m_wave + lr;
+        const bool ok = m < a.M;
+        const unsigned off_s = ok ? (unsigned)(m * a.ldr + 8 * lh) * 4u : 0x80000000u;
+        const unsigned off_x = ok ? (unsigned)(m * a.ldx + 8 * lh) * 4u : 0x80000000u;
+        v4f x0[2 * NK], x1[2 * NK];
+#pragma unroll
+        for (int s = 0; s < 2 * NKS; ++s) {
+            x0[s] = __builtin_bit_cast(v4f, __builtin_amdgcn_raw_buffer_load_b128(rs, off_s + s * 64, 0, 0));
+            x1[s] = __builtin_bit_cast(v4f, __builtin_amdgcn_raw_buffer_load_b128(rs, off_s + s * 64 + 16, 0, 0));
+        }
+#pragma unroll
+        for (int s = 0; s < 2 * NKM; ++s) {
+            x0[2 * NKS + s] = __builtin_bit_cast(v4f, __builtin_amdgcn_raw_buffer_load_b128(rx, off_x + s * 64, 0, 0));
+            x1[2 * NKS + s] = __builtin_bit_cast(v4f, __builtin_amdgcn_raw_buffer_load_b128(rx, off_x + s * 64 + 16, 0, 0));
+        }
+#pragma unroll
+        for (int s = 0; s < 2 * NK; ++s) split3_bf16(x0[s], x1[s], ah[s], am[s], al[s]);
+    }
+    asm volatile("s_waitcnt vmcnt(0)" ::: "memory");
+    __builtin_amdgcn_s_barrier();
+    __builtin_amdgcn_sched_barrier(0);
+
+    const int brow3 = lr * 12, bsw3 = (lr >> 2) & 3;
+    v4f bfr[2][TN][3];
+#define PEMP_PANEL_READ(dst_, buf_, j_)                                                                           \
+    do {                                                                                                          \
+        const v4f* Bb_ = Bs + (buf_) * SQ;                                                                        \
+        const int pb_ = (2 * (j_) + lh) ^ bsw3;                                                                   \
+        _Pragma("unroll") for (int ni = 0; ni < TN; ++ni)                                                         \
+            _Pragma("unroll") for (int pl = 0; pl < 3; ++pl)                                                      \
+                bfr[dst_][ni][pl] = Bb_[brow3 + ni * 32 * 12 + pl * 4 + pb_];                                     \
+    } while (0)
+#define PEMP_PANEL_MMA_HOOKED(src_, s_, HOOK_)                                                                    \
+    do {                                                                                                          \
+        _Pragma("unroll") for (int pr = 0; pr < 6; ++pr)                                                          \
+            _Pragma("unroll") for (int ni = 0; ni < TN; ++ni) {                                                   \
+                const bf16x8 av_ = pr == 0 ? al[s_] : (pr == 2 || pr == 3) ? am[s_] : ah[s_];                     \
+                const bf16x8 bv_ = __builtin_bit_cast(bf16x8, bfr[src_][ni][pr == 1 ? 2 : (pr == 2 || pr == 4) ? 1 : 0]); \
+                acc[ni] = __builtin_amdgcn_mfma_f32_32x32x16_bf16(av_, bv_, acc[ni], 0, 0, 0);                    \
+                HOOK_(pr * TN + ni);                                                                              \
+            }                                                                                                     \
+    } while (0)
+#define PEMP_PANEL_HOOK_NONE(j_)
+#define PEMP_PANEL_HOOK_DMA(j_)                                                                                   \
+    if ((j_) < BL) {                                                                                              \
+        __builtin_amdgcn_sched_barrier(0);                                                                        \
+        PEMP_PANEL_DMA_ONE((j_) < BL ? (j_) : 0);                                                                 \
+        __builtin_amdgcn_sched_barrier(0);                                                                        \
+    }
+
+    f32x16 acc[TN];
+#pragma unroll
+    for (int ni = 0; ni < TN; ++ni)
+#pragma unroll
+        for (int e = 0; e < 16; ++e) acc[ni][e] = 0.f;
+
+    const bool relu = a.flags & PEMP_CONV_RELU;
+    const int er = lane >> 3, c4 = (lane & 7) * 4;
+    unsigned y_off[4];
+#pragma unroll
+    for (int i = 0; i < 4; ++i) {
+        const int m = m_wave + er + 8 * i;
+        y_off[i] = m < a.M ? (unsigned)(m * a.ldy + c4) * 4u : 0x80000000u;
+    }
+    const float* const scale_m = a.scale + a.Cout;
+    const float* const shift_m = a.shift + a.Cout;
+
+    int cur = 0;
+    PEMP_PANEL_READ(0, 0, 0);
+    for (int n = 0; n < ntn; ++n) {
+        v4f rres[NST], scv[TN], shv[TN], scs[TN], shs[TN];
+#pragma unroll
+        for (int kt = 0; kt < NK; ++kt) {
+            const int nxt = cur == NS - 1 ? 0 : cur + 1;
+            PEMP_PANEL_READ(1, cur, 1);
+            __builtin_amdgcn_sched_barrier(0);
+            PEMP_PANEL_MMA_HOOKED(0, 2 * kt, PEMP_PANEL_HOOK_NONE);
+            __builtin_amdgcn_sched_barrier(0);
+            panel_wait<NK, NS, BL, NST>(kt);
+            __builtin_amdgcn_s_barrier();
+            __builtin_amdgcn_sched_barrier(0);
+            PEMP_PANEL_READ(0, nxt, 0);
+            const int t3 = n * NK + kt + NS;
+            const int n3 = n + (kt + NS) / NK, k3 = (kt + NS) % NK;
+            PEMP_PANEL_DMA_SETUP(cur, t3, n3, k3);
+            if (kt == 0) {
+#pragma unroll
+                for (int ni = 0; ni < TN; ++ni) {
+                    const int c = n * BN + ni * 32 + c4;
+                    scs[ni] = *(const v4f*)(a.scale + c);
+                    shs[ni] = *(const v4f*)(a.shift + c);
+                }
+            }
+            if (kt == NKS) {
+#pragma unroll
+                for (int ni = 0; ni < TN; ++ni) {
+                    const int c = n * BN + ni * 32 + c4;
+                    scv[ni] = *(const v4f*)(scale_m + c);
+                    shv[ni] = *(const v4f*)(shift_m + c);
+                }
+            }
+            __builtin_amdgcn_sched_barrier(0);
+            PEMP_PANEL_MMA_HOOKED(1, 2 * kt + 1, PEMP_PANEL_HOOK_DMA);
+            __builtin_amdgcn_sched_barrier(0);
+            cur = nxt;
+            if (kt == NKS - 1) {
+#pragma unroll
+                for (int ni = 0; ni < TN; ++ni) {
+                    PEMP_CONV_PATCH_PUT(patch, acc[ni], lr, lh);
+                    asm volatile("s_waitcnt lgkmcnt(0)" ::: "memory");
+#pragma unroll
+                    for (int i = 0; i < 4; ++i) {
+                        const v4f v = *(const v4f*)(patch + (er + 8 * i) * 32 + c4);
+                        rres[ni * 4 + i] = conv_affine_quad(v, scs[ni], shs[ni], false);
+                        asm volatile("" : "+v"(rres[ni * 4 + i]));
+                    }
+                    asm volatile("s_waitcnt lgkmcnt(0)" ::: "memory");
+#pragma unroll
+                    for (int e = 0; e < 16; ++e) acc[ni][e] = 0.f;
+                }
+                __builtin_amdgcn_sched_barrier(0);
+            }
+        }
+#pragma unroll
+        for (int ni = 0; ni < TN; ++ni) {
+            PEMP_CONV_PATCH_PUT(patch, acc[ni], lr, lh);
+            asm volatile("s_waitcnt lgkmcnt(0)" ::: "memory");
+#pragma unroll
+            for (int i = 0; i < 4; ++i) {
+                const int row = er + 8 * i;
+                const v4f v = *(const v4f*)(patch + row * 32 + c4);
+                v4f add = shv[ni];
+                add += rres[ni * 4 + i];
+                const v4f o = conv_affine_quad(v, scv[ni], add, relu);
+                __builtin_amdgcn_raw_buffer_store_b128(__builtin_bit_cast(v4u, o), ry, y_off[i] + (unsigned)(n * BN + ni * 32) * 4u, 0, 0);
+            }
+            asm volatile("s_waitcnt lgkmcnt(0)" ::: "memory");
+#pragma unroll
+            for (int e = 0; e < 16; ++e) acc[ni][e] = 0.f;
+        }
+        __builtin_amdgcn_sched_barrier(0);
+    }
+    asm volatile("s_waitcnt vmcnt(0)" ::: "memory");
+#undef PEMP_PANEL_DMA_SETUP
+#undef PEMP_PANEL_DMA_ONE
+#undef PEMP_PANEL_READ
+#undef PEMP_PANEL_MMA_HOOKED
+#undef PEMP_PANEL_HOOK_NONE
+#undef PEMP_PANEL_HOOK_DMA
+#endif
+}
+
+template <int NKS, int NKM, int BN, int NW>
+__global__ __launch_bounds__(NW * 64) __attribute__((amdgpu_waves_per_eu(2))) void conv_panel_sc_kernel(ConvArgs a) {
+    conv_panel_sc_body<NKS, NKM, BN, NW>(a);
+}
+
+static_assert(2 * panel_lds<4, 64>() <= 160 * 1024 && panel_lds<4, 64>() <= 80 * 1024, "two blocks per CU");
+
+bool conv_panel_sc_supported(const ConvArgs& a) {
+    if (a.KH != 1 || a.KW != 1 || a.pad != 0 || a.stride != 1 || a.H != a.Ho || a.W != a.Wo || a.nk != 4 || a.Kpad != a.Cin) return false;
+    if (!a.res || !a.scale || !a.shift || a.padv || a.stats || a.rowmask || a.sk_S > 1 || a.bm_first || a.Hr || a.Wr) return false;
+    if (a.flags & ~(PEMP_CONV_RELU | PEMP_CONV_SHORTCUT)) return false;
+    const long long lim = 1ll << 31;
+    return (long long)a.M * a.ldx * 4 < lim && (long long)a.M * a.ldr * 4 < lim && (long long)a.M * a.ldy * 4 < lim &&
+           (long long)a.Cout * a.Kpad * 6 < lim;
+}
+
+int launch_conv_panel_sc(const ConvArgs& a, hipStream_t st) {
+    if (!conv_panel_sc_supported(a)) {
+        set_error("conv split3 panel: PEMP_CONV_SHORTCUT needs a 1x1 / stride 1 conv without padding, Kpad 64 + 64, scale and shift, operands < 2 GiB");
+        return -1;
+    }
+    return launch_with_lds(conv_panel_sc_kernel<2, 2, 64, PANEL_NW>, cdiv(a.M, 32 * PANEL_NW), PANEL_NW * 64, panel_lds<4, 64>(), st, a,
+                           "conv_panel/shortcut");
+}
+
+}
diff --git a/pemp_amd/csrc/conv_panel_sched.h b/pemp_amd/csrc/conv_panel_sched.h
--- /dev/null
+++ b/pemp_amd/csrc/conv_panel_sched.h
@@ -0,0 +1,54 @@
+#pragma once
+#include "conv_tiles.h"
+
+namespace pemp {
+
+typedef __attribute__((address_space(3))) void* lptr_t;
+typedef __attribute__((ext_vector_type(4))) unsigned int v4u;
+
+template <int NK> constexpr bool panel_early() { return NK >= 4; }
+template <int NK, int BN> constexpr bool panel_two_blocks() { return BN == 64 && NK <= 4; }
+template <int NK, int BN> constexpr int panel_stages() {
+    if (!panel_early<NK>()) return 3;
+    if (NK == 4) return 5;
+    return BN == 64 ? 8 : 6;
+}
+template <int NK, int NS, int BL, int NST>
+constexpr int panel_behind(int kt) {
+    int c = 0;
+    for (int u = kt + 1 - NS; u <= kt - 1; ++u) {
+        const int ku = ((u % NK) + NK) % NK;
+        if (u > kt + 1 - NS) c += BL;
+        if (ku == NK - 1) c += NST;
+    }
+    return c;
+}
+template <int NK, int NS, int BL, int NST>
+constexpr int panel_behind_max() {
+    int m = 0;
+    for (int kt = 0; kt < NK; ++kt) m = panel_behind<NK, NS, BL, NST>(kt) > m ? panel_behind<NK, NS, BL, NST>(kt) : m;
+    return m;
+}
+template <int NK, int NS, int BL, int NST, int KT = 0>
+__device__ __forceinline__ void panel_wait(int kt) {
+    if constexpr (KT < NK) {
+        if (kt == KT) asm volatile("s_waitcnt vmcnt(%0) lgkmcnt(0)" ::"n"(panel_behind<NK, NS, BL, NST>(KT)) : "memory");
+        else panel_wait<NK, NS, BL, NST, KT + 1>(kt);
+    }
+}
+
+template <int NK, int BN, int NW>
+struct PanelStream {
+    static constexpr int SQ = BN * 12;
+    static_assert(SQ % (NW * 64) == 0, "whole DMA rounds");
+    static constexpr int BL = SQ / (NW * 64);
+    static constexpr int NST = (BN / 32) * 4;
+    static constexpr int NS = panel_stages<NK, BN>();
+    static constexpr int behind(int kt) { return panel_behind<NK, NS, BL, NST>(kt); }
+    static constexpr int behind_max() { return panel_behind_max<NK, NS, BL, NST>(); }
+};
+
+constexpr int PANEL_NW = 4;
+template <int NK, int BN> constexpr size_t panel_lds() { return (size_t)(panel_stages<NK, BN>() * BN * 12 + PANEL_NW * 256) * sizeof(v4f); }
+
+}
diff --git a/pemp_amd/engine.py b/pemp_amd/engine.py
--- a/pemp_amd/engine.py
+++ b/pemp_amd/engine.py
@@ -106,6 +106,17 @@
 PRUNE_ROWS = os.environ.get("PEMP_PRUNE_ROWS", "1") != "0"
 
 
+FUSE_SHORTCUT = os.environ.get("PEMP_FUSE_SHORTCUT", "1") != "0"
+FUSE_SHORTCUT_MIN_ROWS = None
+
+
+def fuses_shortcut(x, c3, ds, rows):
+    if not (FUSE_SHORTCUT and x.dtype == torch.float32 and x.is_cuda and ops.PICK_HOOK is None and ops.shortcut_tiles(c3, ds)):
+        return False
+    least = 256 * torch.cuda.get_device_properties(x.device).multi_processor_count if FUSE_SHORTCUT_MIN_ROWS is None else FUSE_SHORTCUT_MIN_ROWS
+    return rows >= least
+
+
 def restrided(cp, stride):
     return ConvParams(cp.w, cp.scale, cp.shift, cp.cin, cp.cout, cp.kh, cp.kw, stride, cp.pad, cp.dil, cp.kpad, cp.stem, cp.relu,
                       cp.w3, cp.w3pool)
@@ -162,9 +173,11 @@
         ho, wo = (ops.conv_out_size(v, k, bp.c2.stride, bp.c2.pad, bp.c2.dil) for v, k in ((h1, bp.c2.kh), (w1, bp.c2.kw)))
         if out is None:
             out = a.get(("blk", tag), (n, ho, wo, bp.c3.cout))
-        res = a.get("res", (n, ho, wo, bp.ds.cout)) if bp.ds is not None else x
         grouped = self.GROUP_DS and bp.ds is not None and c1_shift is None and ds_shift is None \
             and 0 < n * ho * wo <= GROUP_MAX_ROWS and x.dtype == torch.float32
+        fused = bp.ds is not None and not grouped and ds_shift is None and a.dtype == torch.float32 and (h, w) == (ho, wo) \
+            and fuses_shortcut(x, bp.c3, bp.ds, n * ho * wo)
+        res = x if bp.ds is None else None if fused else a.get("res", (n, ho, wo, bp.ds.cout))
         pre = presplit_pair(bp.c1, bp.c2, x, n * ho * wo, self.PRESPLIT and not grouped)
         y1 = a.get("y1s", ops.split3_shape(n, h1, w1, bp.c1.cout), torch.bfloat16) if pre else a.get("y1", (n, h1, w1, bp.c1.cout))
         if grouped:
@@ -172,6 +185,8 @@
         else:
             ops.conv2d(x, bp.c1, out=y1, shift_override=c1_shift, per_image_shift=c1_shift is not None, out_split3=pre)
         y2 = ops.conv2d(y1, bp.c2, out=a.get("y2", (n, ho, wo, bp.c2.cout)), x_split3=pre)
+        if fused:
+            return ops.conv2d_shortcut(y2, bp.c3, x, bp.ds, out=out)
         if bp.ds is not None and not grouped:
             ops.conv2d(x, bp.ds, out=res, shift_override=ds_shift, per_image_shift=ds_shift is not None)
         return ops.conv2d(y2, bp.c3, out=out, residual=res, residual_stride=2 if prune else 1)
diff --git a/pemp_amd/ops.py b/pemp_amd/ops.py
--- a/pemp_amd/ops.py
+++ b/pemp_amd/ops.py
@@ -8,7 +8,7 @@
 
 from . import _lib
 from ._lib import ConvDesc, CONV_RELU, CONV_SHIFT_PER_IMAGE, CONV_STEM4, CONV_POOL3S2, CONV_OUT_SPLIT3, CONV_IN_SPLIT3, CONV_OUT_SPLIT3_ALSO
-from ._lib import CONV_RES_S2, CONV_RES_HEVEN, CONV_RES_WEVEN
+from ._lib import CONV_RES_S2, CONV_RES_HEVEN, CONV_RES_WEVEN, CONV_SHORTCUT
 
 
 def _stream():
@@ -469,6 +469,62 @@
     return out
 
 
+SHORTCUT_TILES = (72,)
+SHORTCUT_K = 64
+_SHORTCUT_PACKS = {}
+
+
+def shortcut_tiles(p, p_sc):
+    for q in (p, p_sc):
+        if q.w3 is None or q.stem or (q.kh, q.kw, q.stride, q.pad) != (1, 1, 1, 0) or q.cin != SHORTCUT_K or q.kpad != SHORTCUT_K:
+            return ()
+    if p.cout != p_sc.cout or p_sc.relu or not SPLIT3_PANEL:
+        return ()
+    return tuple(t for t in SHORTCUT_TILES if p.cout % _tile_bn(t) == 0)
+
+
+def _shortcut_pack(p, p_sc):
+    ent = _SHORTCUT_PACKS.get((id(p), id(p_sc)))
+    if ent is None:
+        one = lambda q: torch.ones(q.cout, device=q.w.device) if q.scale is None else q.scale.float()
+        zero = lambda q: torch.zeros(q.cout, device=q.w.device) if q.shift is None else q.shift.float()
+        w3 = pack_split3(torch.cat([p_sc.w[:, :p_sc.kpad], p.w[:, :p.kpad]], dim=1).contiguous())
+        ent = (p, p_sc, w3, torch.stack([one(p_sc), one(p)]).contiguous(), torch.stack([zero(p_sc), zero(p)]).contiguous())
+        _SHORTCUT_PACKS[(id(p), id(p_sc))] = ent
+    return ent[2:]
+
+
+def conv2d_shortcut(x, p, x_sc, p_sc, out=None, relu=None, tile=0):
+    tiles = shortcut_tiles(p, p_sc)
+    if not tiles:
+        raise ValueError("conv2d_shortcut: needs two split3 1x1 / stride 1 / pad 0 layers with Cin = 64 and one Cout, the shortcut without a ReLU")
+    if tile and tile not in tiles:
+        raise ValueError(f"conv2d_shortcut: the computed shortcut needs one of the tile ids {tiles}, got {tile}")
+    n, h, w, cin, ldx, ho, wo, out, ldy, _ = _conv_geom("conv2d_shortcut", x, p, out, None)
+    if tuple(x_sc.shape) != (n, ho, wo, p_sc.cin):
+        raise ValueError(f"conv2d_shortcut: the shortcut's input {tuple(x_sc.shape)} does not lie on the output's grid {(n, ho, wo, p_sc.cin)}")
+    lds = _nhwc(x_sc, "x_sc")
+    lim = 1 << 31
+    if not (n * h * w * ldx * 4 < lim and n * h * w * lds * 4 < lim and n * ho * wo * ldy * 4 < lim):
+        raise ValueError("conv2d_shortcut: operands of 2 GiB or more")
+    _chk_dev(x, x_sc, out, p.w, p_sc.w)
+    w3, scale2, shift2 = _shortcut_pack(p, p_sc)
+    flags = CONV_SHORTCUT | (CONV_RELU if (p.relu if relu is None else relu) else 0)
+    lib = _lib.load()
+    kcat = p_sc.kpad + p.kpad
+
+    def launch(t):
+        d = ConvDesc(n, h, w, kcat, ldx, ho, wo, p.cout, ldy, 1, 1, 1, 0, 1, lds, kcat, flags, t)
+        _lib.check(lib.pemp_conv2d_nhwc_f32(C.byref(d), _p(x), _p(w3), _p(out), _p(scale2), _p(shift2), _p(x_sc), _stream()),
+                   "pemp_conv2d_nhwc_f32")
+
+    if tile == 0:
+        key = (kcat, p.cout, 1, 1, 1, 0, 1, 0, n, h, w, 1, 0, 3, 2048)
+        tile = _choose_tile(key, n * ho * wo, launch, lambda: list(tiles), tiles[0])
+    launch(tile)
+    return out
+
+
 def stem_pool_supported(p):
     return (p.stem and p.w3pool is not None and (p.kh, p.kw, p.stride, p.pad, p.dil) == (7, 7, 2, 3, 1) and p.kpad == 224
             and p.cout % 64 == 0)
diff --git a/scratch/s3_layers_bench.py b/scratch/s3_layers_bench.py
--- a/scratch/s3_layers_bench.py
+++ b/scratch/s3_layers_bench.py
@@ -23,7 +23,8 @@
           (512, 256, 1, 1, False, False), (256, 256, 1, 1, False, False),
           (64, 256, 1, 1, True, False, 1, 51, 101),
           (64, 64, 3, 1, False, False, 2, 101),
-          (256, 256, 3, 12, False, True))
+          (256, 256, 3, 12, False, True),
+          (64, 256, 1, 1, True, False, 1, 101, 0, "shortcut"))
 
 
 def timed(fn, reps, n=5):
@@ -77,6 +78,47 @@
     print(f"{'':>16} hash 43={digest(ref)}", flush=True)
 
 
+def shortcut_row(dev, N, HW, cin, cout, name, reps):
+    if not hasattr(ops, "conv2d_shortcut"):
+        print(f"{name:>16} (no ops.conv2d_shortcut on this tree)", flush=True)
+        return
+    g = torch.Generator().manual_seed(cin * 7 + cout * 3 + 2048)
+    M = N * HW * HW
+    y2 = torch.randn(M, cin, generator=g).to(dev).view(N, HW, HW, cin)
+    x = torch.randn(M, cin, generator=g).to(dev).view(N, HW, HW, cin)
+
+    def layer(relu):
+        w = (torch.randn(cout, cin, 1, 1, generator=g) * (1.0 / cin ** 0.5)).to(dev)
+        packed, kpad = ops.pack_conv_weight(w)
+        packed = packed.contiguous()
+        return ops.ConvParams(packed, (torch.rand(cout, generator=g) + 0.5).to(dev), torch.randn(cout, generator=g).to(dev), cin, cout, 1, 1, 1, 0, 1,
+                              kpad, False, relu, ops.pack_split3(packed))
+    c3, ds = layer(True), layer(False)
+    res, out = torch.empty(N, HW, HW, cout, device=dev), torch.empty(N, HW, HW, cout, device=dev)
+    ref = ops.conv2d(y2, c3, residual=ops.conv2d(x, ds, tile=43), tile=43).clone()
+    fl = 2.0 * M * cout * 2 * cin
+    cells = []
+    for tile in (43, 72):
+        two = lambda: (ops.conv2d(x, ds, out=res, tile=tile), ops.conv2d(y2, c3, residual=res, out=out, tile=tile))
+        out.zero_()
+        two()
+        same = torch.equal(out, ref)
+        us, worst = timed(two, reps)
+        a, _ = timed(lambda: ops.conv2d(x, ds, out=res, tile=tile), reps)
+        b, _ = timed(lambda: ops.conv2d(y2, c3, residual=res, out=out, tile=tile), reps)
+        cells.append(f"{tile}+{tile}: {us:7.1f}..{worst:6.1f}us ({a:.1f} + {b:.1f}) {fl / us / 1e6:5.1f}TF{'' if same else ' !'}")
+    for tile in ops.shortcut_tiles(c3, ds):
+        one = lambda: ops.conv2d_shortcut(y2, c3, x, ds, out=out, tile=tile)
+        out.zero_()
+        one()
+        same = torch.equal(out, ref)
+        us, worst = timed(one, reps)
+        cells.append(f"{tile} fused: {us:7.1f}..{worst:6.1f}us {fl / us / 1e6:5.1f}TF{'' if same else ' !'}")
+        fused_hash = digest(out)
+    print(f"{name:>16} k1 d1 | " + " | ".join(cells), flush=True)
+    print(f"{'':>16} hash 43+43={digest(ref)} fused={fused_hash}", flush=True)
+
+
 def main():
     ap = argparse.ArgumentParser()
     ap.add_argument("--only", default="", help="cin-cout-kK[-padv]: one layer")
@@ -96,6 +138,11 @@
         M = N * HW * HW
         HO = (HW - 1) // stride + 1
         name = f"{cin}-{cout}-k{k}" + (f"-d{dil}" if k == 3 and dil > 2 else "") + ("-padv" if padv else "") + (f"-s{stride}" if stride > 1 else "") + (f"-hw{HW}-res{int(has_res)}" if HW != 51 else "") + ("-rs2" if RS2 else "")
+        if len(layer) > 9:
+            name = f"{cin}+{cin}-{cout}-hw{HW}-shortcut"
+            if not args.only or name in args.only.split(","):
+                shortcut_row(dev, N, HW, cin, cout, name, args.reps)
+            continue
         if args.only and name not in args.only.split(","):
             continue
         if RS2:
```
